# jzlianglu/pykaldi2

Measured on AMD Instinct MI355X. Metric: iRTF (hrs audio/hr) 3x512 BLSTM LF-MMI, LibriSpeech-shaped synthetic utterances, higher is better.
Workload: dtype f32 (GEMMs: bf16x3 split, f32 accumulate)

## Files before the change

pykaldi2_amd/_lib.py:

```python
import ctypes as C
import os

import torch

_HERE = os.path.dirname(os.path.abspath(__file__))
LIB_PATH = os.environ.get("PK2_LIB") or os.path.join(_HERE, "libpk2hip.so")


class Pk2Error(RuntimeError):
    pass


class NumBatch(C.Structure):
    _fields_ = [("arc_src", C.c_void_p), ("arc_dst", C.c_void_p), ("arc_pdf", C.c_void_p),
                ("arc_weight", C.c_void_p), ("frame_off", C.c_void_p), ("state_off", C.c_void_p),
                ("final_state", C.c_void_p), ("final_weight", C.c_void_p), ("final_off", C.c_void_p),
                ("total_arcs", C.c_int64), ("max_seq_arcs", C.c_int64)]


class DecoderOpts(C.Structure):
    _fields_ = [("beam", C.c_float), ("lattice_beam", C.c_float), ("beam_delta", C.c_float),
                ("acoustic_scale", C.c_float), ("max_active", C.c_int32), ("min_active", C.c_int32),
                ("tokens_per_frame", C.c_int32), ("links_per_frame", C.c_int32)]


class SimRirJob(C.Structure):
    _fields_ = [("wav", C.c_void_p), ("rir", C.c_void_p), ("out", C.c_void_p), ("early", C.c_void_p),
                ("delay_dev", C.c_void_p), ("n", C.c_int64), ("k", C.c_int32), ("delay", C.c_int32)]


class SimSeg(C.Structure):
    _fields_ = [("x", C.c_void_p), ("count", C.c_int64)]


class SimMixSrc(C.Structure):
    _fields_ = [("sig", C.c_void_p), ("sig2", C.c_void_p), ("pos", C.c_void_p), ("pos2", C.c_void_p),
                ("n", C.c_int64), ("start", C.c_int64), ("spr_db", C.c_double)]


class ResampleJob(C.Structure):
    _fields_ = [("plan", C.c_void_p), ("inp", C.c_void_p), ("n_in", C.c_int64), ("out", C.c_void_p), ("n_out", C.c_int64),
                ("gain", C.c_float)]


SIM_MAX_SEGS = 16
RESAMPLE_MAX_JOBS = 32
SPEC_MAX_FREQ_MASKS = 4
SPEC_MAX_TIME_MASKS = 16
SPEC_PLAN_STRIDE = 2 + 2 * SPEC_MAX_FREQ_MASKS + 2 * SPEC_MAX_TIME_MASKS
BF_MAX_CHANNELS = 8
BF_MAX_MASKS = 4
BF_FRAMES_PER_PART = 32
BF_REF_SNR = -1
WPE_MAX_CHANNELS = 8
WPE_MAX_ORDER = 80
WPE_MAX_DELAY = 8
WPE_MAX_ITERS = 8
WPE_FRAMES_PER_PART = 1024

_vp, _i32, _i64, _f32, _sz = C.c_void_p, C.c_int32, C.c_int64, C.c_float, C.c_size_t

SIGNATURES = {
    "pk2_last_error": (C.c_char_p, []),
    "pk2_version": (C.c_int, []),
    "pk2_den_graph_create": (C.c_int, [_i32, _i32, _i64, _vp, _vp, _vp, _vp, _i32, C.POINTER(_vp)]),
    "pk2_den_graph_from_openfst": (C.c_int, [C.c_char_p, _i32, C.POINTER(_vp)]),
    "pk2_den_graph_destroy": (C.c_int, [_vp]),
    "pk2_den_graph_info": (C.c_int, [_vp, C.POINTER(_i32), C.POINTER(_i32), C.POINTER(_i64)]),
    "pk2_den_graph_initial_probs": (C.c_int, [_vp, _vp]),
    "pk2_den_graph_arcs_per_lane": (_i32, []),
    "pk2_den_graph_path": (_i32, [_vp, _i32]),
    "pk2_den_graph_persist_form": (_i32, [_vp, _i32]),
    "pk2_den_graph_plan": (C.c_int, [_vp, _i32, _i32, _vp]),
    "pk2_den_graph_debug_ordering": (C.c_int, [_vp, C.c_int, C.POINTER(_i64), C.POINTER(_i32), _vp, _vp,
                                               _vp, _vp, _vp, _vp]),
    "pk2_den_graph_debug_virtual": (C.c_int, [_vp, C.c_int, C.POINTER(_i32), _vp, _vp, _vp, _vp, _vp,
                                              C.POINTER(_i64), _vp, _vp, _vp, C.POINTER(_i32), _vp, _vp]),
    "pk2_den_graph_debug_persist2": (C.c_int, [_vp, C.c_int] + [_vp] * 18),
    "pk2_chain_workspace_bytes": (_sz, [_vp, _i32, _i32, _i64]),
    "pk2_chain_objf_and_deriv": (C.c_int, [_vp, _vp, _i64, _i64, _vp, _i32, C.POINTER(NumBatch), _f32,
                                           _f32, _f32, _f32, _vp, _i64, _i64, _vp, _vp, _sz, _vp]),
    "pk2_chain_objf_and_deriv_op": (C.c_int, [_vp, _vp, _i64, _i64, _vp, _i32, C.POINTER(NumBatch), _f32,
                                              _f32, _f32, _f32, _vp, _i64, _i64, _vp, _vp, _sz, _f32, _vp, _vp]),
    "pk2_chain_den_fwd_bwd": (C.c_int, [_vp, _vp, _i64, _i64, _vp, _i32, _f32, _vp, _vp, _i64, _i64,
                                        _vp, _sz, _vp]),
    "pk2_chain_debug_flags": (C.c_int, [_vp, _vp, _vp, _vp, _i32, _f32, _vp, _vp, _vp]),
    "pk2_chain_debug_num_route": (C.c_int, [_vp]),
    "pk2_split_to_phones": (C.c_int, [_vp, _vp, _vp, _i32, _vp, _i32, _vp, _vp, C.POINTER(_i32), C.POINTER(_i32)]),
    "pk2_sup_model_create": (_vp, [_i32, _vp, _i32, _vp, _vp, _vp, _vp, _vp, _i32, _vp, _i32, _i32, _i32, _vp, _vp,
                                   _vp, _vp, _i32, _vp]),
    "pk2_sup_model_destroy": (None, [_vp]),
    "pk2_sup_model_pdf": (C.c_int, [_vp, _vp, _i32, C.POINTER(_i32)]),
    "pk2_supervision_create": (_vp, [_vp, _vp, _vp, _i32, _i32, _i32, _i32]),
    "pk2_supervision_destroy": (None, [_vp]),
    "pk2_supervision_sizes": (None, [_vp, C.POINTER(_i32), C.POINTER(_i32), C.POINTER(_i32), C.POINTER(_i32),
                                     C.POINTER(_i32)]),
    "pk2_supervision_copy": (C.c_int, [_vp, _vp, _vp, _vp, _vp, _vp, _vp, _vp, _vp, _vp, _vp]),
    "pk2_lexicon_create": (_vp, [_i32, _i32, _i64, _vp, _vp, _vp, _vp, _vp, _vp, _vp, _i32]),
    "pk2_lexicon_from_openfst": (_vp, [C.c_char_p, _vp, _i32]),
    "pk2_lexicon_destroy": (None, [_vp]),
    "pk2_align_model_create": (_vp, [_vp, _i32, _vp, _i32, _vp, C.c_double, C.c_double]),
    "pk2_align_model_destroy": (None, [_vp]),
    "pk2_align_compile": (_vp, [_vp, _vp, _i32, _vp, _vp, _vp]),
    "pk2_align_graphs_destroy": (None, [_vp]),
    "pk2_align_graphs_info": (C.c_int, [_vp, _i32, C.POINTER(_i32), C.POINTER(_i32), C.POINTER(_i32)]),
    "pk2_align_graphs_error": (C.c_char_p, [_vp, _i32]),
    "pk2_align_graphs_copy": (C.c_int, [_vp, _i32, _vp, _vp, _vp, _vp, _vp, _vp]),
    "pk2_align_graphs_packed_words": (_i64, [_vp]),
    "pk2_align_graphs_pack": (C.c_int, [_vp, _vp]),
    "pk2_align_workspace_bytes": (_sz, [_vp]),
    "pk2_align_use_lds": (C.c_int, [_vp]),
    "pk2_align_viterbi": (C.c_int, [_vp, _vp, _vp, _i64, _i64, _i32, _i32, _f32, _f32, _vp, _vp, _vp, _vp, _sz, _vp]),
    "pk2_num_graph_workspace_bytes": (_sz, [_vp]),
    "pk2_num_graph_use_lds": (C.c_int, [_vp]),
    "pk2_num_graph_fwd_bwd": (C.c_int, [_vp, _vp, _vp, _i64, _i64, _i32, _i32, _f32, _vp, _i64, _i64, _vp, _vp, _vp, _sz, _vp]),
    "pk2_chain_graph_workspace_bytes": (_sz, [_vp, _vp]),
    "pk2_chain_objf_and_deriv_graph": (C.c_int, [_vp, _vp, _i64, _i64, _vp, _vp, _f32, _f32, _f32, _f32, _vp, _i64, _i64, _vp,
                                                 _vp, _sz, _vp]),
    "pk2_chain_objf_and_deriv_graph_op": (C.c_int, [_vp, _vp, _i64, _i64, _vp, _vp, _f32, _f32, _f32, _f32, _vp, _i64, _i64,
                                                    _vp, _vp, _sz, _f32, _vp, _vp]),
    "pk2_decode_graph_create": (C.c_int, [_i32, _i32, _i64, _vp, _vp, _vp, _vp, _vp, C.POINTER(_vp)]),
    "pk2_decode_graph_create_words": (C.c_int, [_i32, _i32, _i64, _vp, _vp, _vp, _vp, _vp, _vp, C.POINTER(_vp)]),
    "pk2_decode_graph_link_words": (C.c_int, [_vp, _i64, _vp, _vp, _vp, _vp, _vp]),
    "pk2_decode_graph_from_openfst": (C.c_int, [C.c_char_p, C.POINTER(_vp)]),
    "pk2_decode_graph_destroy": (C.c_int, [_vp]),
    "pk2_decode_graph_info": (C.c_int, [_vp, C.POINTER(_i32), C.POINTER(_i64), C.POINTER(_i32)]),
    "pk2_lattice_batch_create": (C.c_int, [_vp, _vp, _i32, C.POINTER(DecoderOpts), C.POINTER(_vp)]),
    "pk2_lattice_batch_bytes": (_sz, [_vp]),
    "pk2_lattice_batch_destroy": (C.c_int, [_vp]),
    "pk2_lattice_decode": (C.c_int, [_vp, _vp, _i64, _i64, _i32, _vp, _i32, _vp, _vp]),
    "pk2_lattice_summary": (C.c_int, [_vp, _vp, _vp, _vp, _vp, _vp, _vp]),
    "pk2_lattice_persist_status": (C.c_int, [C.POINTER(C.c_int32), C.POINTER(C.c_uint32)]),
    "pk2_lattice_mmi": (C.c_int, [_vp, _vp, _vp, _i64, _vp, C.c_double, C.c_double, _i32, _vp, _i64, _i64, _vp, _vp]),
    "pk2_lattice_mpe": (C.c_int, [_vp, _vp, _vp, _i64, _vp, _vp, _vp, _i32, _i32, C.c_double, C.c_double, _vp, _i64, _i64,
                                  _vp, _vp]),
    "pk2_lattice_nbest_bytes": (_sz, [_vp, _i32, _i64, _i64, _i32, _i32]),
    "pk2_lattice_nbest": (C.c_int, [_vp, _vp, _vp, _i64, _i64, _i32, _i32, _i32, _vp, _i32, C.c_double, C.c_double, _i32,
                                    _vp, _vp, _vp, _vp, _vp, _vp, _vp]),
    "pk2_lattice_mwe": (C.c_int, [_vp, _vp, _vp, _i64, _i64, _i32, _i32, _i32, _vp, _i32, C.c_double, C.c_double, _i32, _i32,
                                  _vp, _i64, _vp, _vp, _i32, _vp, _i64, _i64, _vp, _vp]),
    "pk2_lattice_rescore": (C.c_int, [_vp, _vp, _vp, _i64, _i64, _i32, _vp, _i32, _f32, _vp]),
    "pk2_lattice_fb_rerun": (C.c_int, [_vp, _vp, _vp, _vp]),
    "pk2_lattice_posteriors": (C.c_int, [_vp, _vp, _vp, C.c_double, C.c_double, _f32, _vp, _i64, _i64, _vp, _vp]),
    "pk2_lattice_ts": (C.c_int, [_vp, _vp, _vp, _i64, _i64, _i32, _vp, _i32, _f32, C.c_double, C.c_double, _vp, _i64, _i64,
                                 _vp, _vp, _vp, _vp]),
    "pk2_lattice_export": (C.c_int, [_vp, _vp, _i32, C.POINTER(_i32), C.POINTER(_i32), _vp, _vp, _vp, _vp, _vp,
                                     _vp, _vp, _vp, _vp, _vp]),
    "pk2_comm_unique_id_bytes": (_i32, []),
    "pk2_comm_unique_id": (C.c_int, [_vp]),
    "pk2_comm_init": (C.c_int, [_i32, _i32, _vp, C.POINTER(_vp)]),
    "pk2_allreduce_bucket": (C.c_int, [_vp, _vp, _i64, _vp]),
    "pk2_allreduce_guarded": (C.c_int, [_vp, _vp, _i64, _vp, _vp]),
    "pk2_comm_info": (C.c_int, [_vp, C.POINTER(_i32), C.POINTER(_i32), C.c_char_p, _i32]),
    "pk2_comm_destroy": (C.c_int, [_vp]),
    "pk2_sim_apply_rir": (C.c_int, [_vp, _i64, _vp, _i32, _i32, _vp, _vp]),
    "pk2_sim_apply_rir_dev": (C.c_int, [_vp, _i64, _vp, _i32, _vp, _vp, _vp]),
    "pk2_sim_power": (C.c_int, [_vp, _i64, _vp, _vp]),
    "pk2_rirgen_segment_samples": (_i32, []),
    "pk2_rirgen": (C.c_int, [_vp, _vp, _vp, _vp, _i32, _vp, _i32, _i64, _vp, _vp, _vp, _vp]),
    "pk2_sim_add_noise": (C.c_int, [_vp, _i64, _vp, _i64, _i64, _f32, _vp, _vp, _vp]),
    "pk2_sim_gain_norm": (C.c_int, [_vp, _i64, _vp, _vp]),
    "pk2_sim_apply_rir_mc": (C.c_int, [C.POINTER(SimRirJob), _i32, _i32, _i32, _vp]),
    "pk2_sim_power_seg": (C.c_int, [C.POINTER(SimSeg), _i32, _vp, _vp]),
    "pk2_sim_gain_norm_seg": (C.c_int, [C.POINTER(SimSeg), _i32, _vp, _vp, _vp]),
    "pk2_sim_mix": (C.c_int, [C.POINTER(SimMixSrc), _i32, _i32, _i64, _vp, _vp, _vp, _vp]),
    "pk2_sim_add_noise_mc": (C.c_int, [_vp, _i64, _vp, _i64, _i32, _i64, _f32, _i32, _vp, _vp, _vp]),
    "pk2_resample_plan_create": (C.c_int, [_i32, _i32, C.c_double, _i32, C.POINTER(_vp)]),
    "pk2_resample_plan_destroy": (C.c_int, [_vp]),
    "pk2_resample_plan_info": (C.c_int, [_vp, C.POINTER(_i32), C.POINTER(_i32), C.POINTER(_i32), C.POINTER(_i32),
                                         C.POINTER(_i64)]),
    "pk2_resample_plan_export": (C.c_int, [_vp, _vp, _vp, _vp]),
    "pk2_resample_num_output": (_i64, [_vp, _i64]),
    "pk2_resample_batch": (C.c_int, [C.POINTER(ResampleJob), _i32, _vp]),
    "pk2_resample_last_path": (C.c_int, [C.POINTER(_i32)]),
    "pk2_iso_spectra": (C.c_int, [_vp, _vp, _vp, C.c_uint64, _i32, _i32, _i32, _vp, _vp]),
    "pk2_iso_gauss": (C.c_int, [C.c_uint64, _i32, _i32, _vp, _vp]),
    "pk2_irfft_pow2_f32": (C.c_int, [_vp, _i32, _i32, _vp, _vp]),
    "pk2_stft_num_frames": (_i64, [_i64, _i32, _i32]),
    "pk2_stft_f32": (C.c_int, [C.POINTER(_vp), _i32, _i64, _i32, _i32, _i32, _vp, _vp, _i32, C.c_uint64, _vp, _vp]),
    "pk2_istft_f32": (C.c_int, [_vp, _i32, _i32, _i32, _i32, _i32, _vp, _vp, _vp, _vp]),
    "pk2_mask_power": (C.c_int, [_vp, _i64, _vp, _vp]),
    "pk2_mask_count_workspace_bytes": (_sz, [_i32]),
    "pk2_mask_count_threshold": (C.c_int, [_vp, _i32, _i64, C.c_double, _vp, _sz, _vp, _vp]),
    "pk2_mask_ibm": (C.c_int, [_vp, _vp, _i32, _i32, _i32, _f32, _i32, _vp, _vp, _vp, _vp]),
    "pk2_fbank_create": (C.c_int, [_vp, C.POINTER(_vp)]),
    "pk2_fbank_destroy": (C.c_int, [_vp]),
    "pk2_fbank_num_frames": (_i32, [_i64]),
    "pk2_fbank_compute": (C.c_int, [_vp, _vp, _vp, _i32, _vp, _vp, _i32, _vp]),
    "pk2_pad_roll_subsample": (C.c_int, [_vp, _vp, _i32, _i32, _i32, _i32, _vp, _i32, _i32, _vp]),
    "pk2_mvn_apply": (C.c_int, [_vp, _vp, _vp, _i64, _i32, _vp, _vp]),
    "pk2_spec_augment": (C.c_int, [_vp, _vp, _vp, _i32, _i64, _vp, _i32, _f32, _vp]),
    "pk2_bf_workspace_bytes": (_sz, [_vp, _i32, _i32, _i32, _i32, _i32]),
    "pk2_bf_cov": (C.c_int, [C.POINTER(_vp), C.POINTER(_vp), C.POINTER(_i32), _i32, _i32, _i32, _i32, _i32, _vp, _sz, _vp, _vp]),
    "pk2_bf_mvdr_weights": (C.c_int, [C.POINTER(_vp), C.POINTER(_vp), _i32, _i32, _i32, _i32, C.c_double, _vp, _sz, _vp, _vp,
                                      _vp, _vp]),
    "pk2_bf_apply": (C.c_int, [C.POINTER(_vp), C.POINTER(_vp), C.POINTER(_i32), _i32, _i32, _i32, C.POINTER(_vp), _vp]),
    "pk2_wpe_workspace_bytes": (_sz, [_vp, _i32, _i32, _i32, _i32, _i32]),
    "pk2_wpe_power": (C.c_int, [C.POINTER(_vp), C.POINTER(_i32), _i32, _i32, _i32, C.POINTER(_vp), _vp]),
    "pk2_wpe_corr": (C.c_int, [C.POINTER(_vp), C.POINTER(_vp), C.POINTER(_i32), _i32, _i32, _i32, _i32, _i32, _vp, _sz, _vp, _vp,
                               _vp]),
    "pk2_wpe_solve": (C.c_int, [_vp, _vp, _i32, _i32, _i32, _i32, C.c_double, _vp, _sz, _vp, _vp, _vp]),
    "pk2_wpe_filter": (C.c_int, [C.POINTER(_vp), _vp, C.POINTER(_i32), _i32, _i32, _i32, _i32, _i32, C.POINTER(_vp),
                                 C.POINTER(_vp), _vp]),
    "pk2_wpe": (C.c_int, [C.POINTER(_vp), C.POINTER(_i32), _i32, _i32, _i32, _i32, _i32, _i32, C.c_double, _vp, _sz,
                          C.POINTER(_vp), _vp, _vp]),
    "pk2_softmax_ce_fwd_bwd": (C.c_int, [_vp, _i64, _vp, _i64, _i64, _i32, _vp, _vp, _vp, _i64, _vp, _vp]),
    "pk2_softmax_ce_fwd_bwd_mean": (C.c_int, [_vp, _i64, _vp, _i64, _i64, _i32, _vp, _vp, _vp, _i64, _vp]),
    "pk2_scale_inplace_ratio": (C.c_int, [_vp, _i64, _vp, _vp, _vp]),
    "pk2_scale_by_count": (C.c_int, [_vp, _i64, _f32, _vp, _vp]),
    "pk2_scale_by_scalars": (C.c_int, [_vp, _vp, _i64, _vp, _vp, _vp]),
    "pk2_gemm_f32": (C.c_int, [_i32, _i32, _i32, _i32, _i32, _f32, _vp, _i64, _vp, _i64, _f32, _vp, _i64,
                               _vp, _vp]),
    "pk2_gemm_f32_act": (C.c_int, [_i32, _i32, _i32, _i32, _i32, _f32, _vp, _i64, _vp, _i64, _f32, _vp, _i64, _vp, _i32, _vp, _i64,
                                   _vp]),
    "pk2_gemm_f32_seg": (C.c_int, [_i32, _i32, _i32, _i32, _i32, _i32, _f32, _vp, _i64, _i64, _vp, _i64, _i64, _f32, _vp, _i64, _vp,
                                   _i32, _vp, _i64, _vp]),
    "pk2_gemm_f32_batched": (C.c_int, [_i32, _i32, _i32, _i32, _i32, _f32, _vp, _i64, _i64, _i64, _vp, _i64, _i64, _i64,
                                       _f32, _vp, _i64, _i64, _i64, _i32, _i32, _vp]),
    "pk2_gemm_f32_tn_colsum": (C.c_int, [_i32, _i32, _i32, _f32, _vp, _i64, _vp, _i64, _f32, _vp, _i64, _vp, _vp]),
    "pk2_gemm_set_arith": (C.c_int, [_i32]),
    "pk2_gemm_get_arith": (C.c_int, []),
    "pk2_layernorm_fwd": (C.c_int, [_vp, _vp, _vp, _vp, _i64, _i32, _f32, _vp, _vp, _vp, _vp, _vp]),
    "pk2_layernorm_bwd": (C.c_int, [_vp, _vp, _vp, _vp, _vp, _i64, _i32, _vp, _vp, _vp, _vp]),
    "pk2_softmax_mask_fwd": (C.c_int, [_vp, _vp, _vp, _i32, _i32, _i32, _vp]),
    "pk2_softmax_bwd": (C.c_int, [_vp, _vp, _i32, _i32, _vp]),
    "pk2_attention_fwd": (C.c_int, [_vp, _i32, _i32, _i32, _i32, _f32, _vp, _vp, _f32, C.c_uint64, _vp, _vp, _vp]),
    "pk2_attention_bwd": (C.c_int, [_vp, _vp, _vp, _vp, _i32, _i32, _i32, _i32, _f32, _vp, _vp, _f32, C.c_uint64, _vp,
                                    _vp, _vp]),
    "pk2_attention_bwd_part": (C.c_int, [_i32, _vp, _vp, _vp, _vp, _i32, _i32, _i32, _i32, _f32, _vp, _vp, _f32, C.c_uint64,
                                         _vp, _vp, _vp]),
    "pk2_relu_fwd": (C.c_int, [_vp, _i64, _vp]),
    "pk2_relu_bwd": (C.c_int, [_vp, _vp, _i64, _vp]),
    "pk2_add_inplace": (C.c_int, [_vp, _vp, _i64, _vp]),
    "pk2_colsum_f32": (C.c_int, [_vp, _i64, _i32, _i32, _f32, _vp, _vp]),
    "pk2_lstm_fwd_workspace_floats": (_sz, [_i32, _i32, _i32]),
    "pk2_lstm_layer_fwd": (C.c_int, [_vp, _vp, _vp, _i32, _i32, _i32, _i32, _vp, _vp, _vp, _vp, _vp]),
    "pk2_lstm_layer_fwd_xproj": (C.c_int, [_vp, _vp, _vp, _i32, _i32, _i32, _i32, _vp, _vp, _vp, _vp, _vp, _i32, _vp, _vp,
                                           C.POINTER(_i32), _vp]),
    "pk2_lstm_persist_status": (C.c_int, [C.POINTER(C.c_uint32)]),
    "pk2_lstm_last_path": (C.c_int, [C.POINTER(_i32), C.POINTER(_i32)]),
    "pk2_lattice_determinize": (C.c_int, [_i32, _i32, _i64, _vp, _vp, _vp, _vp, _vp, _vp, _vp, C.c_double, _i64, C.POINTER(_vp)]),
    "pk2_det_lattice_sizes": (C.c_int, [_vp, C.POINTER(_i32), C.POINTER(_i32), C.POINTER(_i64), C.POINTER(_i64), C.POINTER(_i64)]),
    "pk2_det_lattice_export": (C.c_int, [_vp] * 12),
    "pk2_det_lattice_destroy": (None, [_vp]),
    "pk2_persist_guard_status": (C.c_int, [C.POINTER(C.c_uint32)]),
    "pk2_persist_guard_clear": (C.c_int, []),
    "pk2_persist_guard_raise": (C.c_int, [_vp]),
    "pk2_persist_guard_export": (C.c_int, [_vp, _vp]),
    "pk2_persist_guard_import": (C.c_int, [_vp, C.c_uint32, _vp]),
    "pk2_persist_guard_verdict": (C.c_int, [C.c_uint32, C.POINTER(C.c_uint32), C.POINTER(C.c_uint32)]),
    "pk2_lstm_bwd_scratch_floats": (_sz, [_i32, _i32, _i32]),
    "pk2_lstm_layer_bwd_bias": (C.c_int, [_vp, _vp, _vp, _vp, _i32, _i32, _i32, _i32, _vp, _vp, _vp, _vp, C.POINTER(_i32), _vp]),
    "pk2_lstm_layer_bwd": (C.c_int, [_vp, _vp, _vp, _vp, _i32, _i32, _i32, _i32, _vp, _vp, _vp]),
    "pk2_lstm_bwd_wgrad_workspace_floats": (_sz, [_i32, _i32, _i32]),
    "pk2_lstm_layer_bwd_wgrad": (C.c_int, [_vp, _vp, _vp, _vp, _vp, _i32, _i32, _i32, _i32, _vp, _vp, _vp, _vp, _vp, _vp,
                                           C.POINTER(_i32), C.POINTER(_i32), _vp]),
    "pk2_dropout_f32": (C.c_int, [_vp, _vp, _i64, _f32, C.c_uint64, _vp]),
    "pk2_grad_norm": (C.c_int, [_vp, _i64, _vp, _vp, _sz, _vp]),
    "pk2_grad_norm_workspace_bytes": (_sz, [_i64]),
    "pk2_adam_step": (C.c_int, [_vp, _vp, _vp, _vp, _vp, _i64, _f32, _f32, _f32, _f32, _f32, _i64, _f32,
                                _vp, _f32, _vp]),
    "pk2_sgd_step": (C.c_int, [_vp, _vp, _vp, _i64, _f32, _f32, _f32, _i32, _f32, _vp, _f32, _vp]),
    "pk2_stream_create_cu_mask": (C.c_int, [_i32, C.POINTER(_vp)]),
    "pk2_stream_destroy": (C.c_int, [_vp]),
    "pk2_debug_where": (C.c_int, [_vp, _i32, _vp]),
    "pk2_debug_peer_reduce": (C.c_int, [_vp, _vp, _i64, _i32, _i32, _vp]),
}

_lib = None


def lib():
    global _lib
    if _lib is None:
        if not os.path.exists(LIB_PATH):
            raise Pk2Error("%s is missing: run `python -c 'import __graft_entry__ as g; g.build()'` "
                           "(hipcc --offload-arch=gfx950).  There is no CPU fallback." % LIB_PATH)
        handle = C.CDLL(LIB_PATH)
        for name, (res, args) in SIGNATURES.items():
            fn = getattr(handle, name)
            fn.restype = res
            fn.argtypes = args
        _lib = handle
    return _lib


def h2d(host, device):
    import numpy as np
    t = torch.from_numpy(host) if isinstance(host, np.ndarray) else host
    if torch.device(device).type != "cuda" or t.is_cuda or t.numel() == 0:
        return t.to(device)
    return t.contiguous().pin_memory().to(device, non_blocking=True)


def check(status):
    if status != 0:
        msg = lib().pk2_last_error()
        raise Pk2Error("libpk2hip status %d: %s" % (status, msg.decode() if msg else ""))


def persist_guard_raised():
    flag = C.c_uint32(0)
    check(lib().pk2_persist_guard_status(C.byref(flag)))
    return flag.value != 0


def check_persist_guard(where, raised=None):
    if persist_guard_raised() if raised is None else raised:
        raise Pk2Error("%s: a persistent kernel (one-launch LSTM recurrence / denominator / lattice decoder) timed out on "
                       "this device; its output was poisoned with NaN and the optimiser kernels have been leaving the "
                       "weights untouched since.  Typical causes: the GPU is shared with another process, or fewer than "
                       "256 CUs are available to the launch.  PK2_LSTM_SEQ=0 PK2_LSTM_BIG_PERSIST=0 PK2_DEN_PERSIST=0 "
                       "PK2_LAT_DECODER=frames select the launch-per-step kernels." % where)


def ptr(t):
    if t is None:
        return None
    if isinstance(t, torch.Tensor):
        return C.c_void_p(t.data_ptr())
    return C.c_void_p(t.ctypes.data)


def stream_ptr(device=None):
    return C.c_void_p(torch.cuda.current_stream(device).cuda_stream)


def require_gpu():
    if not torch.cuda.is_available():
        raise Pk2Error("pykaldi2_amd needs an MI355X (torch.cuda.is_available() is False); "
                       "there is no CPU fallback")
```

pykaldi2_amd/chain.py:

```python
import ctypes as C

import numpy as np
import torch

from . import _lib


class ChainTrainingOptions:

    def __init__(self, leaky_hmm_coefficient=1.0e-05, xent_regularize=0.0, l2_regularize=0.0):
        self.leaky_hmm_coefficient = leaky_hmm_coefficient
        self.xent_regularize = xent_regularize
        self.l2_regularize = l2_regularize


class SupervisionOptions:

    def __init__(self):
        self.convert_to_pdfs = True
        self.frame_subsampling_factor = 3
        self.left_tolerance = 5
        self.right_tolerance = 5


class DenominatorGraph:
    def __init__(self, den_fst, num_pdfs):
        L = _lib.lib()
        h = C.c_void_p()
        if isinstance(den_fst, (str, bytes)):
            path = den_fst.encode() if isinstance(den_fst, str) else den_fst
            _lib.check(L.pk2_den_graph_from_openfst(path, int(num_pdfs), C.byref(h)))
        else:
            src = np.ascontiguousarray(den_fst["src"], dtype=np.int32)
            dst = np.ascontiguousarray(den_fst["dst"], dtype=np.int32)
            pdf = np.ascontiguousarray(den_fst["pdf"], dtype=np.int32)
            prob = np.ascontiguousarray(den_fst["prob"], dtype=np.float32)
            _lib.check(L.pk2_den_graph_create(int(den_fst["num_states"]), int(num_pdfs), src.shape[0],
                                              _lib.ptr(src), _lib.ptr(dst), _lib.ptr(pdf), _lib.ptr(prob),
                                              int(den_fst.get("start", 0)), C.byref(h)))
        self._h = h
        s, p, a = C.c_int32(), C.c_int32(), C.c_int64()
        _lib.check(L.pk2_den_graph_info(h, C.byref(s), C.byref(p), C.byref(a)))
        self._num_states, self._num_pdfs, self._num_arcs = s.value, p.value, a.value

    def num_states(self):
        return self._num_states

    def num_pdfs(self):
        return self._num_pdfs

    def num_arcs(self):
        return self._num_arcs

    def initial_probs(self):
        out = np.empty(self._num_states, dtype=np.float32)
        _lib.check(_lib.lib().pk2_den_graph_initial_probs(self._h, _lib.ptr(out)))
        return out

    def kernel_path(self, num_seqs):
        return int(_lib.lib().pk2_den_graph_path(self._h, int(num_seqs)))

    def persist_form(self, num_seqs):
        return int(_lib.lib().pk2_den_graph_persist_form(self._h, int(num_seqs)))

    PLAN_FIELDS = ("family", "form", "NG", "need_fill", "xgather", "prep_merged", "tail_mergeable", "gamma_kernel")

    def plan(self, num_seqs, max_frames):
        out = np.zeros(8, dtype=np.int32)
        _lib.check(_lib.lib().pk2_den_graph_plan(self._h, int(num_seqs), int(max_frames), _lib.ptr(out)))
        return dict(zip(self.PLAN_FIELDS, (int(v) for v in out)))

    def debug_persist2(self, which):
        L = _lib.lib()
        info = np.zeros(32, dtype=np.int32)
        _lib.check(L.pk2_den_graph_debug_persist2(self._h, which, _lib.ptr(info), *([None] * 17)))
        if not info[0]:
            return None
        R, T, K, W, SP, SEG = (int(v) for v in info[26:32])
        MC = SEG - 2
        pieces, rows = int(info[7]), int(info[9])
        out = dict(prob=np.empty((R, K, T), np.float32), idx2=np.empty((R, K // 2, T), np.uint32),
                   ends=np.empty((R, 2, T), np.uint32), first_row=np.empty((R, 2, T), np.int32),
                   uncovered=np.empty((R, 2), np.int32), ncomp=np.empty((R, 2), np.int32), rmap=np.empty((2, rows), np.int16),
                   pbeg=np.empty((R, MC + 1), np.int32),
                   sprob=np.empty((pieces, T, SP), np.float32), sidx2=np.empty((pieces, T, SP // 2), np.uint32),
                   sends=np.empty((pieces, T), np.uint32), sfirst_row=np.empty((R, MC, T), np.int32),
                   wcrow=np.empty((R, SEG, W), np.int32), row_begin=np.empty(R + 1, np.int32),
                   grp_begin=np.empty(R + 1, np.int32), row_leak=np.empty(rows, np.float32), row_psum=np.empty(rows, np.float32))
        order = ("prob", "idx2", "ends", "first_row", "uncovered", "ncomp", "rmap", "pbeg", "sprob", "sidx2", "sends", "sfirst_row", "wcrow",
                 "row_begin", "grp_begin", "row_leak", "row_psum")
        _lib.check(L.pk2_den_graph_debug_persist2(self._h, which, _lib.ptr(info), *[_lib.ptr(out[k]) for k in order]))
        out.update(estep=int(info[1]), K=int(info[2]), R=int(info[3]), tfloats=int(info[4]), max_rows=int(info[5]),
                   max_groups=int(info[6]), pieces=pieces, cap=int(info[8]), cbeg=[int(v) for v in info[10:10 + MC + 1]],
                   lds_off=[int(v) for v in info[20:20 + MC]], SP=SP, W=W, T=T, slots=K, row_arrays=int(info[19]))
        return out

    def debug_ordering(self, which):
        L = _lib.lib()
        na, nc = C.c_int64(), C.c_int32()
        _lib.check(L.pk2_den_graph_debug_ordering(self._h, which, C.byref(na), C.byref(nc), None, None,
                                                  None, None, None, None))
        arcs = np.empty((na.value, 4), dtype=np.int32)
        k = int(L.pk2_den_graph_arcs_per_lane())
        meta = np.empty((na.value // k, 2), dtype=np.uint32)
        wb_off = np.empty(nc.value + 1, dtype=np.int32)
        row0 = np.empty(nc.value, dtype=np.int32)
        nrows = np.empty(nc.value, dtype=np.int32)
        atomic = np.empty(nc.value, dtype=np.int32)
        _lib.check(L.pk2_den_graph_debug_ordering(self._h, which, None, None, _lib.ptr(arcs), _lib.ptr(meta),
                                                  _lib.ptr(wb_off), _lib.ptr(row0), _lib.ptr(nrows),
                                                  _lib.ptr(atomic)))
        out = dict(arcs=arcs, meta=meta, wb_off=wb_off, row0=row0, nrows=nrows, atomic=atomic, arcs_per_lane=k)
        if which >= 3:
            nv, nl, no = C.c_int32(), C.c_int64(), C.c_int32()
            _lib.check(L.pk2_den_graph_debug_virtual(self._h, which, C.byref(nv), None, None, None, None, None,
                                                     C.byref(nl), None, None, None, C.byref(no), None, None))
            S = self._num_states
            voff, ooff = np.empty(S + 1, dtype=np.int32), np.empty(S + 1, dtype=np.int32)
            vpdf, opdf = np.empty(nv.value, dtype=np.int32), np.empty(no.value, dtype=np.int32)
            real0, nreal, slot0 = (np.empty(nc.value, dtype=np.int32) for _ in range(3))
            leak = np.empty(nl.value, dtype=np.float32)
            loop_pdf, loop_prob = np.empty(S, dtype=np.int32), np.empty(S, dtype=np.float32)
            _lib.check(L.pk2_den_graph_debug_virtual(self._h, which, None, _lib.ptr(voff), _lib.ptr(vpdf),
                                                     _lib.ptr(real0), _lib.ptr(nreal), _lib.ptr(slot0), None,
                                                     _lib.ptr(leak), _lib.ptr(loop_pdf), _lib.ptr(loop_prob), None,
                                                     _lib.ptr(ooff), _lib.ptr(opdf)))
            out.update(voff=voff, vpdf=vpdf, real0=real0, nreal=nreal, slot0=slot0, row_leak=leak,
                       loop_pdf=loop_pdf, loop_prob=loop_prob, ooff=ooff, opdf=opdf)
        return out

    def __del__(self):
        try:
            if getattr(self, "_h", None):
                _lib.lib().pk2_den_graph_destroy(self._h)
                self._h = None
        except Exception:
            pass


class Supervision:

    def __init__(self, fst, weight=1.0, label_dim=None):
        self.weight = float(weight)
        self.num_sequences = 1
        self.frames_per_sequence = int(fst["frames"])
        self.label_dim = label_dim
        self.num_states = int(fst["num_states"])
        self.src = np.ascontiguousarray(fst["src"], dtype=np.int32)
        self.dst = np.ascontiguousarray(fst["dst"], dtype=np.int32)
        self.pdf = np.ascontiguousarray(fst["pdf"], dtype=np.int32)
        self.arc_weight = np.ascontiguousarray(fst["weight"], dtype=np.float32)
        self.frame_offsets = np.ascontiguousarray(fst["frame_offsets"], dtype=np.int32)
        self.final_states = np.ascontiguousarray(fst["final_states"], dtype=np.int32)
        self.final_weights = np.ascontiguousarray(fst["final_weights"], dtype=np.float32)
        self.state_time = fst.get("state_time")
        assert self.frame_offsets.shape[0] == self.frames_per_sequence + 1


class ProtoSupervision:

    def __init__(self, opts, phones, durations):
        self.phones = np.ascontiguousarray(phones, dtype=np.int32)
        self.durations = np.ascontiguousarray(durations, dtype=np.int32)
        if self.phones.ndim != 1 or self.phones.shape != self.durations.shape or self.phones.shape[0] == 0:
            raise ValueError("phones and durations must be non-empty lists of equal length")
        self.frame_subsampling_factor = int(opts.frame_subsampling_factor)
        self.left_tolerance, self.right_tolerance = int(opts.left_tolerance), int(opts.right_tolerance)


def alignment_to_proto_supervision(opts, phones, durations):
    return ProtoSupervision(opts, phones, durations)


class _SupModel:

    def __init__(self, tree, trans_model):
        if trans_model.entries is None:
            raise ValueError("the transition model carries no topology (read it from 0.trans_mdl / final.mdl)")
        max_phone = max(trans_model.phone2entry)
        p2e = np.full(max_phone + 1, -1, np.int32)
        for ph, e in trans_model.phone2entry.items():
            p2e[ph] = e
        e_off, fwd, loop, t_off, t_dst = [0], [], [], [0], []
        for states in trans_model.entries:
            for f, l, dsts in states:
                fwd.append(f); loop.append(l); t_dst.extend(dsts); t_off.append(len(t_dst))
            e_off.append(len(fwd))
        arr = lambda v: np.ascontiguousarray(v, dtype=np.int32)
        e_off, fwd, loop, t_off, t_dst = arr(e_off), arr(fwd), arr(loop), arr(t_off), arr(t_dst)
        tuples = arr(trans_model.tuples)
        L = _lib.lib()
        self._h = L.pk2_sup_model_create(max_phone, _lib.ptr(p2e), len(trans_model.entries), _lib.ptr(e_off),
                                         _lib.ptr(fwd), _lib.ptr(loop), _lib.ptr(t_off), _lib.ptr(t_dst),
                                         tuples.shape[0], _lib.ptr(tuples), tree.N, tree.P, tree.kind.shape[0],
                                         _lib.ptr(tree.kind), _lib.ptr(tree.key), _lib.ptr(tree.a), _lib.ptr(tree.b),
                                         tree.pool.shape[0], _lib.ptr(tree.pool))
        if not self._h:
            raise _lib.Pk2Error(L.pk2_last_error().decode())
        self.label_dim = trans_model.num_pdfs()

    def pdf(self, window, pdf_class):
        w = np.ascontiguousarray(window, dtype=np.int32)
        out = C.c_int32()
        _lib.check(_lib.lib().pk2_sup_model_pdf(self._h, _lib.ptr(w), int(pdf_class), C.byref(out)))
        return out.value

    def __del__(self):
        try:
            if self._h:
                _lib.lib().pk2_sup_model_destroy(self._h)
                self._h = None
        except Exception:
            pass


_sup_models = {}


def supervision_model(tree, trans_model):
    key = (id(tree), id(trans_model))
    hit = _sup_models.get(key)
    if hit is None or hit[0] is not tree or hit[1] is not trans_model:
        hit = _sup_models[key] = (tree, trans_model, _SupModel(tree, trans_model))
    return hit[2]


def proto_supervision_to_supervision(tree, trans_model, proto, convert_to_pdfs=True, with_allowed=False):
    if not convert_to_pdfs:
        raise NotImplementedError("only convert_to_pdfs=True (reference bin/train_chain.py:185) is built")
    m = supervision_model(tree, trans_model)
    L = _lib.lib()
    h = L.pk2_supervision_create(m._h, _lib.ptr(proto.phones), _lib.ptr(proto.durations), proto.phones.shape[0],
                                 proto.frame_subsampling_factor, proto.left_tolerance, proto.right_tolerance)
    if not h:
        raise _lib.Pk2Error(L.pk2_last_error().decode())
    try:
        n = [C.c_int32() for _ in range(5)]
        L.pk2_supervision_sizes(h, *[C.byref(v) for v in n])
        frames, ns, na, nf, nal = (v.value for v in n)
        src, dst, pdf = (np.empty(na, np.int32) for _ in range(3))
        w, foff, stime = np.empty(na, np.float32), np.empty(frames + 1, np.int32), np.empty(ns, np.int32)
        fin, finw = np.empty(nf, np.int32), np.empty(nf, np.float32)
        aoff = np.empty(frames + 1, np.int32) if with_allowed else None
        aph = np.empty(nal, np.int32) if with_allowed else None
        _lib.check(L.pk2_supervision_copy(h, _lib.ptr(src), _lib.ptr(dst), _lib.ptr(pdf), _lib.ptr(w), _lib.ptr(foff),
                                          _lib.ptr(stime), _lib.ptr(fin), _lib.ptr(finw), _lib.ptr(aoff), _lib.ptr(aph)))
    finally:
        L.pk2_supervision_destroy(h)
    sup = Supervision(dict(num_states=ns, frames=frames, src=src, dst=dst, pdf=pdf, weight=w, frame_offsets=foff,
                           state_time=stime, final_states=fin, final_weights=finw), label_dim=m.label_dim)
    if with_allowed:
        sup.allowed_phones = [aph[aoff[t]:aoff[t + 1]].tolist() for t in range(frames)]
    return sup


def split_to_phones(trans_model, alignment):
    if trans_model.tid2tstate is None:
        raise ValueError("the transition model carries no topology (read it from final.mdl)")
    ali = np.ascontiguousarray(alignment, dtype=np.int32)
    T = ali.shape[0]
    phones, durs = np.empty(max(T, 1), np.int32), np.empty(max(T, 1), np.int32)
    n, ok = C.c_int32(), C.c_int32()
    _lib.check(_lib.lib().pk2_split_to_phones(_lib.ptr(trans_model.tid2tstate), _lib.ptr(trans_model.tid2phone),
                                              _lib.ptr(trans_model.tid_flags), trans_model.num_transition_ids(),
                                              _lib.ptr(ali), T, _lib.ptr(phones), _lib.ptr(durs), C.byref(n),
                                              C.byref(ok)))
    starts = np.concatenate([[0], np.cumsum(durs[:n.value])[:-1]]) if n.value else []
    return bool(ok.value), [(int(p), int(s), int(d)) for p, s, d in zip(phones[:n.value], starts, durs[:n.value])]


def supervision_from_alignment(aligner, tree, trans_model, opts, trans_ids):
    phone_ali = aligner.to_phone_alignment(trans_ids)
    proto = alignment_to_proto_supervision(opts, [item[0] for item in phone_ali], [item[2] for item in phone_ali])
    return proto_supervision_to_supervision(tree, trans_model, proto, opts.convert_to_pdfs)


def read_disambig(path):
    if not path:
        return []
    with open(path) as f:
        return [int(tok) for line in f for tok in line.split()[:1]]


def read_symbols(path):
    with open(path) as f:
        return {p[0]: int(p[1]) for p in (line.split() for line in f) if len(p) >= 2}


class Lexicon:

    def __init__(self, fst, disambig=()):
        L = _lib.lib()
        dis = np.ascontiguousarray(list(disambig), np.int32)
        if isinstance(fst, (str, bytes)):
            h = L.pk2_lexicon_from_openfst(fst.encode() if isinstance(fst, str) else fst, _lib.ptr(dis), dis.shape[0])
        else:
            a = {k: np.ascontiguousarray(fst[k], np.int32) for k in ("src", "dst", "ilabel", "olabel")}
            w = np.ascontiguousarray(fst["weight"], np.float32)
            fin = np.ascontiguousarray(fst["final"], np.float32)
            assert fin.shape[0] == int(fst["num_states"])
            h = L.pk2_lexicon_create(int(fst["num_states"]), int(fst.get("start", 0)), a["src"].shape[0], _lib.ptr(a["src"]),
                                     _lib.ptr(a["dst"]), _lib.ptr(a["ilabel"]), _lib.ptr(a["olabel"]), _lib.ptr(w), _lib.ptr(fin),
                                     _lib.ptr(dis), dis.shape[0])
        if not h:
            raise _lib.Pk2Error(L.pk2_last_error().decode())
        self._h = h

    def __del__(self):
        try:
            if self._h:
                _lib.lib().pk2_lexicon_destroy(self._h)
                self._h = None
        except Exception:
            pass


class AlignModel:

    def __init__(self, tree, trans_model, transition_scale=1.0, self_loop_scale=1.0):
        lp = getattr(trans_model, "log_probs", None)
        if lp is None:
            raise ValueError("the transition model has no <LogProbs> (read it from final.mdl): the aligner needs them")
        if lp.shape[0] != trans_model.num_transition_ids() + 1:
            raise ValueError("<LogProbs> holds %d values for %d transition-ids" % (lp.shape[0], trans_model.num_transition_ids()))
        self._sup = _SupModel(tree, trans_model)
        tuples = np.ascontiguousarray(trans_model.tuples, np.int32)
        lp = np.ascontiguousarray(lp, np.float64)
        L = _lib.lib()
        self._h = L.pk2_align_model_create(self._sup._h, tuples.shape[0], _lib.ptr(tuples), trans_model.num_transition_ids(),
                                           _lib.ptr(lp), float(transition_scale), float(self_loop_scale))
        if not self._h:
            raise _lib.Pk2Error(L.pk2_last_error().decode())

    def __del__(self):
        try:
            if self._h:
                _lib.lib().pk2_align_model_destroy(self._h)
                self._h = None
        except Exception:
            pass


ALIGN_OK, ALIGN_BEAM, ALIGN_NO_PATH, ALIGN_ERROR = 0, 1, 2, 3


class AlignmentGraphs:

    def __init__(self, model, lexicon, texts, frames):
        word_off = np.cumsum([0] + [len(t) for t in texts]).astype(np.int32)
        words = np.ascontiguousarray([int(w) for t in texts for w in t] or [0], np.int32)
        self.frames = np.ascontiguousarray(frames, np.int32)
        assert self.frames.shape[0] == len(texts)
        L = _lib.lib()
        self._h = L.pk2_align_compile(model._h, lexicon._h, len(texts), _lib.ptr(word_off), _lib.ptr(words), _lib.ptr(self.frames))
        if not self._h:
            raise _lib.Pk2Error(L.pk2_last_error().decode())
        self._keep = (model, lexicon)
        self.n = len(texts)
        self.status, self.num_states, self.num_arcs, self.errors = [], [], [], []
        for i in range(self.n):
            v = [C.c_int32() for _ in range(3)]
            _lib.check(L.pk2_align_graphs_info(self._h, i, *[C.byref(x) for x in v]))
            self.status.append(v[0].value); self.num_states.append(v[1].value); self.num_arcs.append(v[2].value)
            self.errors.append(L.pk2_align_graphs_error(self._h, i).decode())

    def export(self, i):
        S, A = self.num_states[i], self.num_arcs[i]
        out = dict(in_off=np.empty(S + 1, np.int32), src=np.empty(A, np.int32), tid=np.empty(A, np.int32),
                   pdf=np.empty(A, np.int32), weight=np.empty(A, np.float32), final=np.empty(S, np.float32))
        _lib.check(_lib.lib().pk2_align_graphs_copy(self._h, i, *[_lib.ptr(out[k]) for k in
                                                                 ("in_off", "src", "tid", "pdf", "weight", "final")]))
        out["dst"] = np.repeat(np.arange(S, dtype=np.int32), np.diff(out["in_off"]))
        return out
# ... 379 lines not shown
```

pykaldi2_amd/csrc/chain_den_persist2.hip:

```cpp
#include <algorithm>
#include <cstdlib>
#include <cstring>
#include <map>
#include <type_traits>
#include <vector>

#include "chain_num.h"
#include "den_persist_dev.h"

namespace pk2 {

struct DenPersist2Params {
  DenParams d;
  DevPersist2 fwd, bwd;
  const float* xv;
  const int32_t* vpdf;
  const int32_t* loop_pdf;
  int xgather;
  int rowarrays;
  float* ring;
  float* pring;
  int rpad;
  int tfloats;
  int cap;
  int ntasks;
  NumParams np;
  int fwd_stream, bwd_stream;
  int pspt;
  short task_seq[kMaxTasks];
  unsigned char task_dir[kMaxTasks];
};
typedef __attribute__((address_space(4))) const DenPersist2Params CParams2;
typedef __attribute__((address_space(4))) const DevPersist2 CDev2;
__device__ __forceinline__ CParams2* uni(CParams2* p) {
  const unsigned long long v = (unsigned long long)p;
  const unsigned lo = (unsigned)__builtin_amdgcn_readfirstlane((int)(unsigned)v);
  const unsigned hi = (unsigned)__builtin_amdgcn_readfirstlane((int)(unsigned)(v >> 32));
  return (CParams2*)(((unsigned long long)hi << 32) | lo);
}

extern __shared__ __attribute__((aligned(16))) float den_persist2_smem[];
struct Lds2 {
  float* table;
  float* accA;
  float* accB;
  float* accS;
  float* xown;
  float* leak;
  float* aux;
  short* mapA;
  short* mapB;
  short* pdfv;
  short* pdfl;
  float* red;
  float* tot;
  float* wcarry;
  int* wcrow;
  int* abort;
};
__device__ __forceinline__ Lds2 carve_lds2(int tfloats, int cap, int arrays) {
  Lds2 L;
  L.table = den_persist2_smem; L.accA = L.table + tfloats; L.accB = L.accA + cap; L.accS = L.accB + cap; L.xown = L.accS + cap;
  L.leak = L.xown + cap; L.aux = L.leak + cap;
  L.mapA = reinterpret_cast<short*>(L.aux + cap); L.mapB = L.mapA + cap;
  L.pdfv = L.mapB + cap; L.pdfl = L.pdfv + cap;
  L.red = L.aux + (arrays - 5) * cap; L.tot = L.red + 2 * kPW; L.wcarry = L.tot + 4;
  L.wcrow = reinterpret_cast<int*>(L.wcarry + kSegs * kPW); L.abort = L.wcrow + kSegs * kPW;
  return L;
}

__device__ __forceinline__ void lds_only_barrier() { asm volatile("s_waitcnt lgkmcnt(0)\n\ts_barrier" ::: "memory"); }

#ifndef PK2_DP2_LATE_HISTORY
#define PK2_DP2_LATE_HISTORY 0
#endif
#ifndef PK2_DP2_LATE_STREAM
#define PK2_DP2_LATE_STREAM 1
#endif
template <bool STREAM> constexpr bool kLateHistory = PK2_DP2_LATE_HISTORY && (!STREAM || PK2_DP2_LATE_STREAM);
template <bool NT>
__device__ __forceinline__ float once_load(cgfloat* p) {
  if constexpr (NT) return __builtin_nontemporal_load(p);
  else return *p;
}
template <bool NT>
__device__ __forceinline__ void once_store(gfloat* p, float v) {
  if constexpr (NT) __builtin_nontemporal_store(v, p);
  else *p = v;
}

template <bool ON>
__device__ __forceinline__ int per_frame(int r) {
  if constexpr (ON) asm volatile("" : "+v"(r));
  return r;
}
__device__ __forceinline__ float ld_uniform_base(cgfloat* ubase, int idx) {
  typedef __attribute__((address_space(1))) const char gchar;
  return *(cgfloat*)((gchar*)ubase + (uint32_t)idx * 4u);
}

__device__ __forceinline__ constexpr int vmcnt_imm(int k) { return (k & 15) | ((k >> 4) << 14) | 0x70 | 0xF00; }
__device__ __forceinline__ void wait_vm(int n) {
  asm volatile("" ::: "memory");
  switch (__builtin_amdgcn_readfirstlane(n)) {
#define PK2_VM_CASE(k) case k: __builtin_amdgcn_s_waitcnt(vmcnt_imm(k)); break;
    PK2_VM_CASE(1) PK2_VM_CASE(2) PK2_VM_CASE(3) PK2_VM_CASE(4) PK2_VM_CASE(5) PK2_VM_CASE(6) PK2_VM_CASE(7) PK2_VM_CASE(8)
    PK2_VM_CASE(9) PK2_VM_CASE(10) PK2_VM_CASE(11) PK2_VM_CASE(12) PK2_VM_CASE(13) PK2_VM_CASE(14) PK2_VM_CASE(15) PK2_VM_CASE(16)
    PK2_VM_CASE(17) PK2_VM_CASE(18) PK2_VM_CASE(19) PK2_VM_CASE(20)
#undef PK2_VM_CASE
    default: __builtin_amdgcn_s_waitcnt(vmcnt_imm(0)); break;
  }
  asm volatile("" ::: "memory");
}

__device__ __forceinline__ int dma_chunk(cgfloat* src, CDev2& o, int c, float* table) {
  const int lane = threadIdx.x & 63, w = threadIdx.x >> 6;
  const int b = o.cbeg[c], e = o.cbeg[c + 1];
  const int rows = (e - b + 255) >> 8;
  const int n = (rows + kPW - 1) / kPW;
  const int e4 = (e + 3) & ~3;
  float* dst = table + o.lds_off[c];
  for (int k = 0; k < n; ++k) {
    int row = w + k * kPW;
    row = row < rows ? row : rows - 1;
    const int off = row << 8;
    if (b + off + lane * 4 < e4) dma256(src + b + off + lane * 4, dst + off);
  }
  return n;
}
typedef __attribute__((address_space(3))) float lfloat;
__device__ __forceinline__ uint32_t lds_addr(const float* p) { return (uint32_t)(uintptr_t)(const lfloat*)p; }
__device__ __forceinline__ float lds_load(uint32_t a) { return *(const lfloat*)(uintptr_t)a; }
__device__ __forceinline__ void lds_store(uint32_t a, float v) { *(lfloat*)(uintptr_t)a = v; }

struct DmaPlan {
  uint64_t mask[8];
  uint32_t off4[8];
  uint32_t dst;
  int rows, efl, w;
  uint32_t lane16;
  __device__ __forceinline__ void place(int j, uint64_t* mask_out, uint32_t* off4_out) const {
    int row = w + j * kPW;
    row = row < rows ? row : rows - 1;
    const int off = row << 8;
    int n = (efl - off + 3) >> 2;
    n = j * kPW < rows ? n : 0;
    n = n < 0 ? 0 : n;
    *mask_out = n >= 64 ? ~0ull : ((1ull << n) - 1ull);
    *off4_out = (uint32_t)off * 4u;
  }
  __device__ __forceinline__ void init(CDev2& o, const float* table) {
    const int b1 = o.cbeg[1], e1 = o.cbeg[2];
    dst = (uint32_t)__builtin_amdgcn_readfirstlane((int)lds_addr(table + o.lds_off[1]));
    rows = (e1 - b1 + 255) >> 8; efl = ((e1 + 3) & ~3) - b1; w = __builtin_amdgcn_readfirstlane((int)(threadIdx.x >> 6));
    lane16 = (threadIdx.x & 63u) * 16u;
#pragma unroll
    for (int j = 0; j < 8; ++j) {
      place(j, &mask[j], &off4[j]);
      asm volatile("" : "+s"(mask[j]), "+s"(off4[j]));
    }
  }
};
__device__ __forceinline__ void dma_issue(uint64_t mask, uint32_t m0v, uint32_t lane16, uint64_t g) {
  uint64_t saved;
  asm volatile("s_mov_b64 %0, exec\n\ts_mov_b64 exec, %1\n\ts_mov_b32 m0, %2\n\ts_nop 0\n\t"
               "global_load_lds_dwordx4 %3, %4 sc1\n\ts_mov_b64 exec, %0"
               : "=&s"(saved) : "s"(mask), "s"(m0v), "v"(lane16), "s"(g) : "memory");
}
struct Chunk1Dma {
  uint64_t src;
  const DmaPlan* pl;
  __device__ __forceinline__ void operator()(int j) const {
    if (j < 8) { dma_issue(pl->mask[j], pl->dst + pl->off4[j], pl->lane16, src + pl->off4[j]); return; }
    uint64_t mask; uint32_t off4;
    pl->place(j, &mask, &off4);
    dma_issue(mask, pl->dst + off4, pl->lane16, src + off4);
  }
};

struct NoDma { __device__ __forceinline__ void operator()(int) const {} };

#ifndef PK2_DP2_PASS_ASM
#define PK2_DP2_PASS_ASM 1
#endif
__device__ __forceinline__ void lds_gather8(const uint32_t* ad, float (&a)[8]) {
  asm volatile("ds_read_b32 %0, %8\n\tds_read_b32 %1, %9\n\tds_read_b32 %2, %10\n\tds_read_b32 %3, %11\n\t"
               "ds_read_b32 %4, %12\n\tds_read_b32 %5, %13\n\tds_read_b32 %6, %14\n\tds_read_b32 %7, %15"
               : "=&v"(a[0]), "=&v"(a[1]), "=&v"(a[2]), "=&v"(a[3]), "=&v"(a[4]), "=&v"(a[5]), "=&v"(a[6]), "=&v"(a[7])
               : "v"(ad[0]), "v"(ad[1]), "v"(ad[2]), "v"(ad[3]), "v"(ad[4]), "v"(ad[5]), "v"(ad[6]), "v"(ad[7]) : "memory");
}
template <int N>
__device__ __forceinline__ void lds_wait8(float (&a)[8]) {
  asm volatile("s_waitcnt lgkmcnt(%8)" : "+v"(a[0]), "+v"(a[1]), "+v"(a[2]), "+v"(a[3]), "+v"(a[4]), "+v"(a[5]), "+v"(a[6]), "+v"(a[7])
               : "n"(N) : "memory");
}
template <int N>
__device__ __forceinline__ void lds_wait4(float& a0, float& a1, float& a2, float& a3) {
  asm volatile("s_waitcnt lgkmcnt(%4)" : "+v"(a0), "+v"(a1), "+v"(a2), "+v"(a3) : "n"(N) : "memory");
}
__device__ __forceinline__ void row_end_place(unsigned& m, uint32_t& cb, float& sum) {
  uint64_t save;
  asm volatile("v_add_co_u32 %0, vcc, %0, %0\n\ts_and_saveexec_b64 %3, vcc\n\tds_write_b32 %1, %2\n\t"
               "v_add_u32 %1, 4, %1\n\tv_mov_b32 %2, 0\n\ts_or_b64 exec, exec, %3"
               : "+v"(m), "+v"(cb), "+v"(sum), "=&s"(save) : : "vcc", "scc", "memory");
}

template <bool PACKED, int J0>
__device__ __forceinline__ void slot_addresses(const uint32_t (&addr)[kPK], uint32_t base, int j0, uint32_t (&out)[8]) {
#pragma unroll
  for (int j = 0; j < 8; ++j) {
    const int s = J0 + j0 + j;
    if (PACKED) {
      uint32_t pk = addr[s >> 1];
      if ((s & 1) == 0) asm volatile("" : "+v"(pk));
      out[j] = base + ((s & 1) ? (pk >> 16) << 2 : (pk & 0xffffu) << 2);
    } else {
      out[j] = addr[s];
    }
  }
}
template <int ESTEP, int J0, int NS, bool PACKED, typename DMA>
__device__ __forceinline__ void pass_rows(const float (&prob)[kPK], const uint32_t (&addr)[kPK], uint32_t base, uint32_t ends, int frow,
                                          float* acc, float* wcarry, const DMA& dma) {
  const int lane = threadIdx.x & 63, w = threadIdx.x >> 6;
  float sum = 0.f;
  uint32_t cb = lds_addr(acc) + 4u * (uint32_t)frow;
  uint32_t packed = 0;
#pragma unroll
  for (int k = 0; k < NS / ESTEP; ++k) packed |= ((ends >> (k * ESTEP + ESTEP - 1)) & 1u) << k;
  unsigned m = __builtin_bitreverse32(packed);
  asm volatile("" : "+v"(m));
  float a[2][8];
#if PK2_DP2_PASS_ASM
  constexpr int NG = NS / 8;
  constexpr int kStores = 8 / ESTEP;
  uint32_t ad[8];
  slot_addresses<PACKED, J0>(addr, base, 0, ad);
  lds_gather8(ad, a[0]);
  dma(0);
#pragma unroll
  for (int g = 0; g < NG; ++g) {
    if (g + 1 < NG) { slot_addresses<PACKED, J0>(addr, base, 8 * (g + 1), ad); lds_gather8(ad, a[(g + 1) & 1]); dma(2 * g + 2); }
    constexpr int kMost = 15;
    if (g == 0) lds_wait8<(NG > 1 ? 8 : 0)>(a[0]);
    else if (g + 1 < NG) lds_wait8<(8 + kStores < kMost ? 8 + kStores : kMost)>(a[g & 1]);
    else lds_wait8<kStores>(a[g & 1]);
#pragma unroll
    for (int j = 0; j < 8; ++j) {
      const int jj = 8 * g + j;
      sum = fmaf(a[g & 1][j], prob[J0 + jj], sum);
      if ((jj + 1) % ESTEP == 0) row_end_place(m, cb, sum);
    }
    dma(2 * g + 1);
  }
#else
  auto gather = [&](int j0, float (&a)[8]) {
    uint32_t ad2[8];
    slot_addresses<PACKED, J0>(addr, base, j0, ad2);
#pragma unroll
    for (int j = 0; j < 8; ++j) a[j] = lds_load(ad2[j]);
  };
  gather(0, a[0]);
  dma(0);
#pragma unroll
  for (int g = 0; g < NS / 8; ++g) {
    if (g + 1 < NS / 8) { gather(8 * (g + 1), a[(g + 1) & 1]); dma(2 * g + 2); }
#pragma unroll
    for (int j = 0; j < 8; ++j) {
      const int jj = 8 * g + j;
      sum = fmaf(a[g & 1][j], prob[J0 + jj], sum);
      if ((jj + 1) % ESTEP == 0) {
        if (__builtin_add_overflow(m, m, &m)) { lds_store(cb, sum); cb += 4u; sum = 0.f; }
      }
    }
    dma(2 * g + 1);
  }
#endif
  float x[1] = {sum};
  int fl = ends != 0u ? 1 : 0;
  seg_scan_step<1, 0x111, 0xf>(x, fl);
  seg_scan_step<1, 0x112, 0xf>(x, fl);
  seg_scan_step<1, 0x114, 0xf>(x, fl);
  seg_scan_step<1, 0x118, 0xf>(x, fl);
  seg_scan_step<1, 0x142, 0xa>(x, fl);
  seg_scan_step<1, 0x143, 0xc>(x, fl);
  const float cin = dpp_f<0x138, 0xf>(x[0]);
  if (ends != 0u) acc[frow] += cin;
  if (lane == 63) wcarry[w] = x[0];
}
template <int J0, bool PACKED, typename DMA>
__device__ __forceinline__ void pass_rows_any(int estep, const float (&prob)[kPK], const uint32_t (&addr)[kPK], uint32_t base,
                                              uint32_t ends, int frow, float* acc, float* wcarry, const DMA& dma) {
  switch (estep) {
    case 8: pass_rows<8, J0, kQ, PACKED>(prob, addr, base, ends, frow, acc, wcarry, dma); break;
    case 4: pass_rows<4, J0, kQ, PACKED>(prob, addr, base, ends, frow, acc, wcarry, dma); break;
    case 2: pass_rows<2, J0, kQ, PACKED>(prob, addr, base, ends, frow, acc, wcarry, dma); break;
    default: pass_rows<1, J0, kQ, PACKED>(prob, addr, base, ends, frow, acc, wcarry, dma); break;
  }
}

typedef float __attribute__((ext_vector_type(4))) f32x4;
typedef uint32_t __attribute__((ext_vector_type(4))) u32x4v;
struct Piece { f32x4 p0, p1; u32x4v ix; uint32_t ends; };
__device__ __forceinline__ void piece_load(CDev2& o, int piece, Piece& q) {
  static_assert(kSP == 8, "a piece is two float4 of probabilities and one uint4 of packed offsets per thread");
  const size_t at = (size_t)piece * kPT + threadIdx.x;
  const __attribute__((address_space(1))) f32x4* sp = (const __attribute__((address_space(1))) f32x4*)o.sprob + at * (kSP / 4);
  const __attribute__((address_space(1))) u32x4v* si = (const __attribute__((address_space(1))) u32x4v*)o.sidx2 + at;
  const __attribute__((address_space(1))) uint32_t* se = (const __attribute__((address_space(1))) uint32_t*)o.sends;
  q.p0 = sp[0]; q.p1 = sp[1];
  q.ix = si[0];
  q.ends = se[at];
}
__device__ __forceinline__ void row_end_add(unsigned& m, uint32_t& cb, float& sum) {
  uint64_t save;
  asm volatile("v_add_co_u32 %0, vcc, %0, %0\n\ts_and_saveexec_b64 %3, vcc\n\tds_add_f32 %1, %2\n\t"
               "v_add_u32 %1, 4, %1\n\tv_mov_b32 %2, 0\n\ts_or_b64 exec, exec, %3"
               : "+v"(m), "+v"(cb), "+v"(sum), "=&s"(save) : : "vcc", "scc", "memory");
}
template <int ESTEP>
__device__ __forceinline__ void piece_rows(const Piece q, uint32_t base, uint32_t& cb, float& sum) {
  uint32_t packed = 0;
#pragma unroll
  for (int k = 0; k < kSP / ESTEP; ++k) packed |= ((q.ends >> (k * ESTEP + ESTEP - 1)) & 1u) << k;
  unsigned m = __builtin_bitreverse32(packed);
  uint32_t ad[8];
#pragma unroll
  for (int j = 0; j < kSP; ++j) {
    const uint32_t pk = q.ix[j >> 1];
    ad[j] = base + ((j & 1) ? (pk >> 16) << 2 : (pk & 0xffffu) << 2);
  }
  float a[8];
  lds_gather8(ad, a);
  lds_wait4<4>(a[0], a[1], a[2], a[3]);
#pragma unroll
  for (int j = 0; j < 4; ++j) {
    sum = fmaf(a[j], q.p0[j], sum);
    if ((j + 1) % ESTEP == 0) row_end_add(m, cb, sum);
  }
  lds_wait4<(ESTEP <= 4 ? 4 / ESTEP : 0)>(a[4], a[5], a[6], a[7]);
#pragma unroll
  for (int j = 4; j < 8; ++j) {
    sum = fmaf(a[j], q.p1[j & 3], sum);
    if ((j + 1) % ESTEP == 0) row_end_add(m, cb, sum);
  }
}
__device__ __forceinline__ void piece_rows_any(int estep, const Piece q, uint32_t base, uint32_t& cb, float& sum) {
  switch (estep) {
    case 8: piece_rows<8>(q, base, cb, sum); break;
    case 4: piece_rows<4>(q, base, cb, sum); break;
    case 2: piece_rows<2>(q, base, cb, sum); break;
    default: piece_rows<1>(q, base, cb, sum); break;
  }
}

constexpr int kPieceDepth = 2;
constexpr int kPieceLoads = 4;
struct StreamState { Piece r0, r1; int pb[kMaxChunks + 1]; int frow[2]; int pend; };
static_assert(kPieceDepth == 2, "StreamState holds two pieces");
__device__ __forceinline__ void stream_init(CDev2& o, int rank, StreamState& st) {
#pragma unroll
  for (int c = 0; c <= kMaxChunks; ++c) st.pb[c] = __builtin_amdgcn_readfirstlane(o.pbeg[rank * (kMaxChunks + 1) + c]);
  const __attribute__((address_space(1))) int32_t* sfr = (const __attribute__((address_space(1))) int32_t*)o.sfirst_row;
#pragma unroll
  for (int c = 0; c < 2; ++c) st.frow[c] = st.pb[c + 1] > st.pb[c] ? sfr[((size_t)rank * kMaxChunks + c) * kPT + threadIdx.x] : 0;
  st.pend = st.pb[0];
#pragma unroll
  for (int c = 1; c <= kMaxChunks; ++c) st.pend = c == o.K ? st.pb[c] : st.pend;
}
__device__ __forceinline__ void stream_prime(CDev2& o, StreamState& st) {
  const int pfirst = st.pb[0], pend = st.pend;
  if (pfirst < pend) piece_load(o, pfirst, st.r0);
  if (pfirst + 1 < pend) piece_load(o, pfirst + 1, st.r1);
}
__device__ __forceinline__ int streamed_segment(CDev2& o, int rank, int c, int p0, int p1, StreamState& st, const Lds2& L) {
  const int tid = threadIdx.x, lane = tid & 63, w = tid >> 6;
  const int pend = st.pend;
  const int frow = c < 2 ? st.frow[c < 2 ? c : 0]
                         : ((const __attribute__((address_space(1))) int32_t*)o.sfirst_row)[((size_t)rank * kMaxChunks + c) * kPT + tid];
  float sum = 0.f;
  int issued = 0;
  uint32_t had = 0;
  uint32_t cb = lds_addr(L.accS) + 4u * (uint32_t)frow;
  const uint32_t base = lds_addr(L.table);
  for (int p = p0; p < p1; ++p) {
    had |= st.r0.ends;
    piece_rows_any(o.estep, st.r0, base, cb, sum);
    st.r0 = st.r1;
    if (p + kPieceDepth < pend) { piece_load(o, p + kPieceDepth, st.r1); ++issued; }
  }
  float x[1] = {sum};
  int fl = had != 0u ? 1 : 0;
  seg_scan_step<1, 0x111, 0xf>(x, fl);
  seg_scan_step<1, 0x112, 0xf>(x, fl);
  seg_scan_step<1, 0x114, 0xf>(x, fl);
  seg_scan_step<1, 0x118, 0xf>(x, fl);
  seg_scan_step<1, 0x142, 0xa>(x, fl);
  seg_scan_step<1, 0x143, 0xc>(x, fl);
  const float cin = dpp_f<0x138, 0xf>(x[0]);
  if (had != 0u) L.accS[frow] += cin;
  if (lane == 63) L.wcarry[(2 + c) * kPW + w] = x[0];
  return issued;
}

struct FrameRegs {
  float prob[kPK]; uint32_t addr[kPK]; uint32_t base; uint32_t endsA, endsB; int frowA, frowB;
};
struct NoStream { };
struct RowSpan { int nrows, uncA, ncA, uncB, ncB; };
template <bool STREAM, typename ST, typename STAGE>
__device__ __forceinline__ void frame_rows(CDev2& o, cgfloat* src, int rank, const RowSpan& rs, const FrameRegs& r,
                                           const DmaPlan& plan, ST& st, const Lds2& L, DpTimers& dp_, STAGE stage,
                                           bool prime_next = false) {
  const int tid = threadIdx.x;
  if constexpr (STREAM) {
    for (int q = tid; q < rs.nrows; q += kPT) L.accS[q] = 0.f;
    for (int q = rs.uncA + tid; q < rs.ncA; q += kPT) L.accA[q] = 0.f;
    for (int q = rs.uncB + tid; q < rs.ncB; q += kPT) L.accB[q] = 0.f;
  }
  dma_chunk(src, o, 0, L.table);
  DP_T(0);
  wait_vm(0);
  lds_only_barrier();
  DP_T(1);
  DP_TLF(2);
  Chunk1Dma c1;
  {
    const uint64_t sb = (uint64_t)(src + o.cbeg[1]);
    c1.src = ((uint64_t)(uint32_t)__builtin_amdgcn_readfirstlane((int)(uint32_t)(sb >> 32)) << 32) |
             (uint32_t)__builtin_amdgcn_readfirstlane((int)(uint32_t)sb);
    c1.pl = &plan;
  }
  const bool shared = o.K == 2 && o.lds_off[1] == o.lds_off[0] && o.cbeg[2] > o.cbeg[1];
  if (shared) {
    pass_rows_any<0, STREAM>(o.estep, r.prob, r.addr, r.base, r.endsA, r.frowA, L.accA, L.wcarry, NoDma());
  } else {
    pass_rows_any<0, STREAM>(o.estep, r.prob, r.addr, r.base, r.endsA, r.frowA, L.accA, L.wcarry, c1);
    for (int j = 8; j * kPW < plan.rows; ++j) c1(j);
  }
  DP_T(2);
  DP_TLF(3);
  if constexpr (STREAM) {
    const int (&pb)[kMaxChunks + 1] = st.pb;
    const int K = o.K;
    int young = 0;
    if (pb[1] > pb[0]) young = streamed_segment(o, rank, 0, pb[0], pb[1], st, L);
    DP_T(8);
    if (shared) { lds_only_barrier(); dma_chunk(src, o, 1, L.table); young = 0; }
    wait_vm(kPieceLoads * (young < kPieceDepth ? young : kPieceDepth));
    stage();
    lds_only_barrier();
    DP_T(3);
    if (K > 2) dma_chunk(src, o, 2, L.table);
    pass_rows_any<kQ, STREAM>(o.estep, r.prob, r.addr, r.base, r.endsB, r.frowB, L.accB, L.wcarry + kPW, NoDma());
    DP_T(4);
    if (pb[2] > pb[1]) streamed_segment(o, rank, 1, pb[1], pb[2], st, L);
#pragma unroll
    for (int c = 2; c < kMaxChunks; ++c) {
      if (c >= K) break;
      wait_vm(0);
      __syncthreads();
      if (c + 1 < K) dma_chunk(src, o, c + 1, L.table);
      if (pb[c + 1] > pb[c]) streamed_segment(o, rank, c, pb[c], pb[c + 1], st, L);
    }
    if (prime_next) stream_prime(o, st);
  } else {
    if (shared) { lds_only_barrier(); dma_chunk(src, o, 1, L.table); }
    wait_vm(0);
    stage();
    __syncthreads();
    DP_T(3);
    pass_rows_any<kQ, STREAM>(o.estep, r.prob, r.addr, r.base, r.endsB, r.frowB, L.accB, L.wcarry + kPW, NoDma());
  }
  if constexpr (STREAM) DP_T(9); else DP_T(4);
}

template <bool STREAM>
__device__ __forceinline__ float row_val(const Lds2& L, uint64_t cmask, int q) {
  const int a = L.mapA[q], b = L.mapB[q];
  float v = (a >= 0 ? L.accA[a] : 0.f) + (b >= 0 ? L.accB[b] : 0.f);
  if constexpr (STREAM) v += L.accS[q];
  uint64_t m = cmask;
  while (m) {
    const int k = __builtin_ctzll(m);
    m &= m - 1;
    if (L.wcrow[k] == q) v += L.wcarry[k];
  }
  return v;
}

template <int NW>
__device__ __forceinline__ void block_sum2(float& u, float& v, float* red) {
  const int lane = threadIdx.x & 63, w = threadIdx.x >> 6;
  u = wave_sum_dpp(u); v = wave_sum_dpp(v);
  __syncthreads();
  if (lane == 0) { red[w] = u; red[NW + w] = v; }
  __syncthreads();
  float a = 0.f, b = 0.f;
  for (int k = 0; k < NW; ++k) { a += red[k]; b += red[NW + k]; }
  u = a; v = b;
}

template <bool PACKED>
__device__ __forceinline__ void load_frame_regs(CDev2& o, int rank, FrameRegs& r, const float* table) {
  const int tid = threadIdx.x;
  const uint32_t base = lds_addr(table);
  r.base = (uint32_t)__builtin_amdgcn_readfirstlane((int)base);
#pragma unroll
  for (int j = 0; j < kPK; ++j) r.prob[j] = o.prob[((size_t)rank * kPK + j) * kPT + tid];
#pragma unroll
  for (int j = 0; j < kPK / 2; ++j) {
    const uint32_t pk = o.idx2[((size_t)rank * (kPK / 2) + j) * kPT + tid];
    if (PACKED) { r.addr[j] = pk; continue; }
    r.addr[2 * j] = base + ((pk & 0xffffu) << 2); r.addr[2 * j + 1] = base + ((pk >> 16) << 2);
    asm volatile("" : "+v"(r.addr[2 * j]), "+v"(r.addr[2 * j + 1]));
  }
  r.endsA = o.ends[((size_t)rank * 2 + 0) * kPT + tid]; r.endsB = o.ends[((size_t)rank * 2 + 1) * kPT + tid];
  r.frowA = o.first_row[((size_t)rank * 2 + 0) * kPT + tid]; r.frowB = o.first_row[((size_t)rank * 2 + 1) * kPT + tid];
}

template <bool STREAM, int PSPT>
__device__ __noinline__ void run_fwd2(CParams2* pp_, DenPersistCtl* ctl_, DenPersistCtl::Team* team_,
                                      unsigned* nbar, int g_, int T_, int rank_, float* ring_, float* pring_) {
  CParams2* pp = uni(pp_);
  DenPersistCtl* ctl = uni(ctl_); DenPersistCtl::Team* team = uni(team_);
  const int g = uni(g_), T = uni(T_), rank = uni(rank_);
  ring_ = uni(ring_); pring_ = uni(pring_);
  CParams2& p = *pp;
  CDenParams& d = p.d;
  CDev2& o = p.fwd;
  const Lds2 L = carve_lds2(p.tfloats, p.cap, p.rowarrays);
  gfloat* ring = G(ring_); gfloat* pring = G(pring_);
  const int tid = threadIdx.x;
  const int S = d.S, V = d.V, Vo = d.Vo;
  const bool sep = d.alphav != d.alpha;
  FrameRegs fr;
  load_frame_regs<STREAM>(o, rank, fr, L.table);
  DmaPlan plan;
  plan.init(o, L.table);
  const int row0 = o.row_begin[rank], nrows = o.row_begin[rank + 1] - row0;
  const int g0 = o.grp_begin[rank], ngrp = o.grp_begin[rank + 1] - g0;
  RowSpan rs;
  rs.nrows = nrows; rs.uncA = o.uncovered[rank * 2]; rs.uncB = o.uncovered[rank * 2 + 1];
  rs.ncA = o.ncomp[rank * 2]; rs.ncB = o.ncomp[rank * 2 + 1];
  for (int r = tid; r < nrows; r += kPT) { L.mapA[r] = o.rmap[row0 + r]; L.mapB[r] = o.rmap[(size_t)o.num_rows + row0 + r]; }
  typename std::conditional<STREAM, StreamState, NoStream>::type st;
  if constexpr (STREAM) stream_init(o, rank, st);
  for (int r = tid; r < nrows; r += kPT) L.leak[r] = o.row_leak[row0 + r];
  const bool xg = p.xgather != 0;
  if (xg) {
    for (int r = tid; r < nrows; r += kPT) L.pdfv[r] = (short)p.vpdf[row0 + r];
    for (int r = tid; r < ngrp; r += kPT) L.pdfl[r] = (short)p.loop_pdf[g0 + r];
  }
  if (tid < kSegs * kPW) L.wcrow[tid] = o.wcrow[(size_t)rank * kSegs * kPW + tid];
  int st_lo[PSPT], st_hi[PSPT], st_o[PSPT]; float st_pl[PSPT], st_pi[PSPT]; bool st_ok[PSPT];
#pragma unroll
  for (int i = 0; i < PSPT; ++i) {
    const int r = tid + i * kPT;
    st_ok[i] = r < ngrp;
    st_lo[i] = st_hi[i] = st_o[i] = 0; st_pl[i] = st_pi[i] = 0.f;
    if (st_ok[i]) {
      const int dd = g0 + r;
      st_lo[i] = d.voff[dd] - row0; st_hi[i] = d.voff[dd + 1] - row0; st_o[i] = d.ooff[dd];
      st_pl[i] = d.loop_prob[dd]; st_pi[i] = d.pi[dd];
    }
  }
  if (tid < 3 * kPWords) st_agent(pring + ((tid / kPWords) * kPR + rank) * kPWords + tid % kPWords, __uint_as_float(kRingSentinel));
  if (!team_barrier(ctl, team, nbar, L.abort)) return;
  uint64_t cmask = 0;
  for (int k = 0; k < kSegs * kPW; ++k) {
    const int q = L.wcrow[k];
    bool mine = false;
#pragma unroll
    for (int i = 0; i < PSPT; ++i) mine = mine || (st_ok[i] && q >= st_lo[i] && q < st_hi[i]);
    if (q >= 0 && mine) cmask |= 1ull << k;
  }

  const size_t f0 = (size_t)g * (d.Tmax + 1);
  cgfloat* xv_g = G(p.xv) + (size_t)g * d.Tmax * V;
  cgfloat* xl_g = G(d.xl) + (size_t)g * d.Tmax * S;
  cgfloat* xp_g = G(p.xv) + (size_t)g * d.Tmax * d.P;
  float xr[PSPT], xlr[PSPT], xln[PSPT];
  auto prefetch = [&](int t) {
    if (xg) {
      cgfloat* row = xp_g + (size_t)t * d.P;
#pragma unroll
      for (int i = 0; i < PSPT; ++i) {
        const int r = per_frame<STREAM>(tid + i * kPT);
        const int pv = r < nrows ? L.pdfv[r] : -1, pl = st_ok[i] ? L.pdfl[r] : -1;
        xr[i] = r < nrows ? (pv >= 0 ? row[pv] : 1.f) : 0.f;
        xln[i] = st_ok[i] ? (pl >= 0 ? row[pl] : 1.f) : 0.f;
      }
      return;
    }
#pragma unroll
    for (int i = 0; i < PSPT; ++i) {
      const int r = per_frame<STREAM>(tid + i * kPT);
      if constexpr (STREAM) {
        xr[i] = r < nrows ? ld_uniform_base(xv_g + ((size_t)t * V + row0), r) : 0.f;
        xln[i] = st_ok[i] ? ld_uniform_base(xl_g + ((size_t)t * S + g0), r) : 0.f;
      } else {
        xr[i] = r < nrows ? once_load<!STREAM>(&xv_g[(size_t)t * V + row0 + r]) : 0.f;
        xln[i] = st_ok[i] ? once_load<!STREAM>(&xl_g[(size_t)t * S + g0 + r]) : 0.f;
      }
    }
  };
  prefetch(0);
#pragma unroll
  for (int i = 0; i < PSPT; ++i) xlr[i] = xln[i];
  if constexpr (STREAM) stream_prime(o, st);
  float own_a[PSPT];
#pragma unroll
  for (int i = 0; i < PSPT; ++i) own_a[i] = st_pi[i];
  float hist_loop[PSPT], hist_loc = 0.f;
#pragma unroll
  for (int i = 0; i < PSPT; ++i) hist_loop[i] = 0.f;
  auto history = [&](int tt) {
    gfloat* alpha_n = G(d.alpha) + (f0 + tt + 1) * (size_t)S;
    gfloat* alphav_n = G(d.alphav) + (f0 + tt + 1) * (size_t)Vo;
    if (tid == 0) G(d.apart)[(f0 + tt + 1) * kPR + rank] = hist_loc;
#pragma unroll
    for (int i = 0; i < PSPT; ++i) {
      if (!st_ok[i]) continue;
      if (!sep) once_store<!STREAM>(&alpha_n[g0 + tid + i * kPT], own_a[i]);
      if (sep) {
        for (int q = st_lo[i]; q < st_hi[i]; ++q) once_store<!STREAM>(&alphav_n[st_o[i] + q - st_lo[i]], L.aux[q]);
        if (st_pl[i] > 0.f) once_store<!STREAM>(&alphav_n[st_o[i] + st_hi[i] - st_lo[i]], hist_loop[i]);
      }
    }
  };
  Spin spin(ctl);
  DP_T0();
  for (int t = 0; t < T; ++t) {
    float as;
    cgfloat* src;
    DP_TL(0, 0);
    DP_TLSET(0);
    if (t == 0) {
      as = d.pi_sum;
      src = G(d.pi);
    } else {
      src = ring + (size_t)(t & 1) * p.rpad;
      poll_words(pring + (size_t)(t % 3) * kPR * kPWords, 0, 1, spin, L);
      __syncthreads();
      DP_TL(0, 1);
      if (*L.abort) return;
      as = L.tot[0];
      if (tid == 0) L.abort[8] = 0;
    }
    const bool publish = t + 1 < T;
    if (tid == 0 && publish) st_agent(word_of(pring, t + 2, rank, 0), __uint_as_float(kRingSentinel));
    frame_rows<STREAM>(o, src, rank, rs, fr, plan, st, L, dp_, [&]() {
#pragma unroll
      for (int i = 0; i < PSPT; ++i) {
        const int r = tid + i * kPT;
        if (r < nrows) L.xown[r] = xr[i];
      }
      if (kLateHistory<STREAM> && t > 0) history(t - 1);
      if (publish) prefetch(t + 1);
    }, publish);
    DP_TL(0, 4);
    if constexpr (STREAM) lds_only_barrier(); else __syncthreads();
    if (rank == 0 && tid == 0) G(d.asum)[f0 + t] = as;
    const float lk = d.leaky * as, inv_as = 1.0f / as;
    gfloat* ring_n = ring + (size_t)((t + 1) & 1) * p.rpad;
    float outv[PSPT], loopv[PSPT], loc = 0.f, unused = 0.f;
#pragma unroll
    for (int i = 0; i < PSPT; ++i) {
      outv[i] = 0.f; loopv[i] = 0.f;
      if (!st_ok[i]) continue;
      float sum = 0.f;
      for (int q = st_lo[i]; q < st_hi[i]; ++q) {
        const float v = (row_val<STREAM>(L, cmask, q) + lk * L.leak[q]) * L.xown[q] * inv_as;
        L.aux[q] = v;
        sum += v;
      }
      if (st_pl[i] > 0.f) { loopv[i] = (own_a[i] + lk * st_pi[i]) * st_pl[i] * xlr[i] * inv_as; sum += loopv[i]; }
      if (publish) ring_store(ring_n + g0 + tid + i * kPT, sum);
      outv[i] = sum;
      own_a[i] = sum;
      loc += sum;
    }
    DP_T(5);
    DP_TL(0, 5);
    wait_stores();
    block_sum2<kPW>(loc, unused, L.red);
    if (tid == 0 && publish) st_agent(word_of(pring, t + 1, rank, 0), loc);
    DP_T(6);
    DP_TL(0, 6);
    hist_loc = loc;
#pragma unroll
    for (int i = 0; i < PSPT; ++i) hist_loop[i] = loopv[i];
    if (!kLateHistory<STREAM>) history(t);
#pragma unroll
    for (int i = 0; i < PSPT; ++i) xlr[i] = xln[i];
    DP_T(7);
  }
  if (kLateHistory<STREAM> && T > 0) history(T - 1);
  DP_FLUSH(0);
}

template <bool STREAM, int PSPT>
__device__ __noinline__ void run_bwd2(CParams2* pp_, DenPersistCtl* ctl_, DenPersistCtl::Team* team_,
                                      unsigned* nbar, int g_, int T_, int rank_, float* ring_, float* pring_) {
  CParams2* pp = uni(pp_);
  DenPersistCtl* ctl = uni(ctl_); DenPersistCtl::Team* team = uni(team_);
  const int g = uni(g_), T = uni(T_), rank = uni(rank_);
  ring_ = uni(ring_); pring_ = uni(pring_);
  CParams2& p = *pp;
  CDenParams& d = p.d;
  CDev2& o = p.bwd;
  const Lds2 L = carve_lds2(p.tfloats, p.cap, p.rowarrays);
  gfloat* ring = G(ring_); gfloat* pring = G(pring_);
  const int tid = threadIdx.x;
  const int S = d.S, V = d.V;
  FrameRegs fr;
  load_frame_regs<STREAM>(o, rank, fr, L.table);
  DmaPlan plan;
  plan.init(o, L.table);
  const int row0 = o.row_begin[rank], nrows = o.row_begin[rank + 1] - row0;
  const int vfirst = d.voff[row0], nvirt = d.voff[row0 + nrows] - vfirst;
  RowSpan rs;
  rs.nrows = nrows; rs.uncA = o.uncovered[rank * 2]; rs.uncB = o.uncovered[rank * 2 + 1];
  rs.ncA = o.ncomp[rank * 2]; rs.ncB = o.ncomp[rank * 2 + 1];
  for (int r = tid; r < nrows; r += kPT) { L.mapA[r] = o.rmap[row0 + r]; L.mapB[r] = o.rmap[(size_t)o.num_rows + row0 + r]; }
  typename std::conditional<STREAM, StreamState, NoStream>::type st;
  if constexpr (STREAM) stream_init(o, rank, st);
  if (tid < kSegs * kPW) L.wcrow[tid] = o.wcrow[(size_t)rank * kSegs * kPW + tid];
  int st_v0[PSPT], st_v1[PSPT]; float st_pl[PSPT], st_pi[PSPT]; bool st_ok[PSPT];
#pragma unroll
  for (int i = 0; i < PSPT; ++i) {
    const int r = tid + i * kPT;
    st_ok[i] = r < nrows;
    st_v0[i] = st_v1[i] = 0; st_pl[i] = st_pi[i] = 0.f;
    if (st_ok[i]) {
      const int s = row0 + r;
      st_v0[i] = d.voff[s] - vfirst; st_v1[i] = d.voff[s + 1] - vfirst; st_pl[i] = d.loop_prob[s]; st_pi[i] = d.pi[s];
    }
  }
  for (int r = tid; r < nvirt; r += kPT) { L.leak[r] = p.fwd.row_leak[vfirst + r]; L.aux[r] = p.fwd.row_psum[vfirst + r]; }
  const bool xg = p.xgather != 0;
  if (xg) {
    for (int r = tid; r < nvirt; r += kPT) L.pdfv[r] = (short)p.vpdf[vfirst + r];
    for (int r = tid; r < nrows; r += kPT) L.pdfl[r] = (short)p.loop_pdf[row0 + r];
  }
  if (tid < 3 * kPWords) st_agent(pring + ((tid / kPWords) * kPR + rank) * kPWords + tid % kPWords, __uint_as_float(kRingSentinel));
  if (!team_barrier(ctl, team, nbar, L.abort)) return;
  uint64_t cmask = 0;
  for (int k = 0; k < kSegs * kPW; ++k) {
    const int q = L.wcrow[k];
    bool mine = false;
#pragma unroll
    for (int i = 0; i < PSPT; ++i) mine = mine || (st_ok[i] && q == tid + i * kPT);
    if (q >= 0 && mine) cmask |= 1ull << k;
  }

  const size_t f0 = (size_t)g * (d.Tmax + 1);
  cgfloat* xv_g = G(p.xv) + (size_t)g * d.Tmax * V;
  cgfloat* xl_g = G(d.xl) + (size_t)g * d.Tmax * S;
  float xl_cur[PSPT], xl_prev[PSPT], xl_next[PSPT], xw[PSPT], bh[PSPT];
  const float cst_last = 1.0f / d.pi_sum + d.leaky;
#pragma unroll
  for (int i = 0; i < PSPT; ++i) { bh[i] = cst_last; xl_cur[i] = 0.f; }
  cgfloat* xp_g = G(p.xv) + (size_t)g * d.Tmax * d.P;
  auto prefetch = [&](int t) {
    if (xg) {
      cgfloat* row = xp_g + (size_t)t * d.P;
#pragma unroll
      for (int i = 0; i < PSPT; ++i) {
        const int r = per_frame<STREAM>(tid + i * kPT);
        const int pl = st_ok[i] ? L.pdfl[r] : -1, pv = r < nvirt ? L.pdfv[r] : -1;
        xl_next[i] = st_ok[i] ? (pl >= 0 ? row[pl] : 1.f) : 0.f;
        xw[i] = r < nvirt ? (pv >= 0 ? row[pv] : 1.f) : 0.f;
      }
      return;
    }
#pragma unroll
    for (int i = 0; i < PSPT; ++i) {
      const int r = per_frame<STREAM>(tid + i * kPT);
      if constexpr (STREAM) {
        xl_next[i] = st_ok[i] ? ld_uniform_base(xl_g + ((size_t)t * S + row0), r) : 0.f;
        xw[i] = r < nvirt ? ld_uniform_base(xv_g + ((size_t)t * V + vfirst), r) : 0.f;
      } else {
        xl_next[i] = st_ok[i] ? once_load<!STREAM>(&xl_g[(size_t)t * S + row0 + r]) : 0.f;
        xw[i] = r < nvirt ? once_load<!STREAM>(&xv_g[(size_t)t * V + vfirst + r]) : 0.f;
      }
    }
  };
  auto stage_x = [&]() {
#pragma unroll
    for (int i = 0; i < PSPT; ++i) {
      const int r = tid + i * kPT;
      if (r < nvirt) L.xown[r] = xw[i];
    }
  };
  auto emit = [&](int t) {
    gfloat* ring_n = ring + (size_t)(t & 1) * p.rpad + vfirst;
    float pB = 0.f, pU = 0.f;
#pragma unroll
    for (int i = 0; i < PSPT; ++i) {
      if (!st_ok[i]) continue;
      for (int q = st_v0[i]; q < st_v1[i]; ++q) {
        const float w = L.xown[q] * bh[i];
        ring_store(ring_n + q, w);
        pB = fmaf(w, L.leak[q], pB); pU = fmaf(w, L.aux[q], pU);
      }
      if (st_pl[i] > 0.f) { const float lp = st_pl[i] * xl_prev[i] * bh[i]; pB = fmaf(st_pi[i], lp, pB); pU += lp; }
    }
    wait_stores();
    block_sum2<kPW>(pB, pU, L.red);
    if (tid < 2) st_agent(word_of(pring, t, rank, tid), tid == 0 ? pB : pU);
    if (tid == 0) {
      G(d.bpart)[((f0 + t - 1) * kPR + rank) * 2] = pB;
      G(d.bpart)[((f0 + t - 1) * kPR + rank) * 2 + 1] = pU;
    }
  };
  prefetch(T - 1);
#pragma unroll
  for (int i = 0; i < PSPT; ++i) xl_prev[i] = xl_next[i];
  stage_x();
  __syncthreads();
  emit(T);
#pragma unroll
  for (int i = 0; i < PSPT; ++i) xl_cur[i] = xl_prev[i];
  if (T >= 2) prefetch(T - 2);
#pragma unroll
  for (int i = 0; i < PSPT; ++i) xl_prev[i] = xl_next[i];
  float vs_hist[PSPT];
#pragma unroll
  for (int i = 0; i < PSPT; ++i) vs_hist[i] = 0.f;
  auto history = [&](int tt) {
    gfloat* bx_t = G(d.beta) + (f0 + tt) * (size_t)V * d.brec;
#pragma unroll
    for (int i = 0; i < PSPT; ++i)
      if (st_ok[i]) once_store<!STREAM>(&bx_t[(size_t)(vfirst + st_v0[i]) * d.brec], vs_hist[i]);
  };
  if constexpr (STREAM) stream_prime(o, st);
  Spin spin(ctl);
  DP_T0();
  for (int t = T - 1; t >= 0; --t) {
    DP_TL(1, 0);
    DP_TLSET(1);
    cgfloat* src_t = ring + (size_t)((t + 1) & 1) * p.rpad;
    poll_words(pring + (size_t)((t + 1) % 3) * kPR * kPWords, 0, 2, spin, L);
    __syncthreads();
    DP_TL(1, 1);
    if (*L.abort) return;
    const float lB = L.tot[0], lU = L.tot[1];
    if (tid == 0) L.abort[8] = 0;
    const bool publish = t > 0;
    if (tid < 2 && publish) st_agent(word_of(pring, t + 2, rank, tid), __uint_as_float(kRingSentinel));
    frame_rows<STREAM>(o, src_t, rank, rs, fr, plan, st, L, dp_, [&]() {
      if (publish) stage_x();
      if (kLateHistory<STREAM> && t + 1 < T) history(t + 1);
      if (t >= 2) prefetch(t - 2);
    }, publish);
    DP_TL(1, 4);
    if constexpr (STREAM) lds_only_barrier(); else __syncthreads();
    const float cu = lB + d.wu * lU;
    const float inv_c = cu > 0.f ? 1.0f / cu : 0.f;
    const float lkr = d.leaky * lB * inv_c;
    float vs[PSPT];
#pragma unroll
    for (int i = 0; i < PSPT; ++i) {
      vs[i] = 0.f;
      if (!st_ok[i]) continue;
      float v = row_val<STREAM>(L, cmask, tid + i * kPT);
      if (st_pl[i] > 0.f) v += st_pl[i] * xl_cur[i] * bh[i];
      vs[i] = v;
      bh[i] = v * inv_c + lkr;
    }
    DP_T(5);
    DP_TL(1, 5);
    if (publish) emit(t);
    DP_T(6);
    DP_TL(1, 6);
#pragma unroll
    for (int i = 0; i < PSPT; ++i) {
      vs_hist[i] = vs[i];
      xl_cur[i] = xl_prev[i];
      xl_prev[i] = xl_next[i];
    }
    if (!kLateHistory<STREAM>) history(t);
    DP_T(7);
  }
  if (kLateHistory<STREAM> && T > 0) history(0);
  DP_FLUSH(1);
}

__global__ void __launch_bounds__(kPT) den_persist2_kernel(const DenPersist2Params* __restrict__ pp_, DenPersistCtl* ctl) {
  CParams2* pp = (CParams2*)pp_;
  CParams2& p = *pp;
  const Lds2 L = carve_lds2(p.tfloats, p.cap, p.rowarrays);
  int& s_abort = L.abort[0];
  int& s_rank = L.abort[1]; int& s_team = L.abort[2]; int& s_xcd = L.abort[3]; int& s_task = L.abort[4];
  const int tid = threadIdx.x;
  if (tid == 0) {
    s_abort = 0;
    const unsigned xcd = den_xcc_id();
    const unsigned slot = __hip_atomic_fetch_add(&ctl->arrive[xcd], 1u, __ATOMIC_RELAXED, __HIP_MEMORY_SCOPE_AGENT);
    s_rank = (int)(slot % kPR); s_team = (int)(slot / kPR); s_xcd = (int)xcd;
  }
  __syncthreads();
  if (s_team >= kMaxTeams) return;
  const int rank = s_rank;
  DenPersistCtl::Team* team = &ctl->team[s_xcd][s_team];
  const size_t ti = (size_t)s_xcd * kMaxTeams + s_team;
  float* ring = p.ring + ti * 2 * p.rpad;
  float* pring = p.pring + ti * 3 * kPR * kPWords;
  unsigned nbar = 0;
  for (int iter = 0; iter <= kMaxTasks; ++iter) {
    if (tid == 0) {
      unsigned k;
      if (rank == 0) {
        k = __hip_atomic_fetch_add(&ctl->next_task, 1u, __ATOMIC_RELAXED, __HIP_MEMORY_SCOPE_AGENT);
        __hip_atomic_store(&team->task[iter], k + 1u, __ATOMIC_RELAXED, __HIP_MEMORY_SCOPE_AGENT);
      } else {
        Spin spin(ctl);
        unsigned k1;
        while ((k1 = ld_agent_u(G(&team->task[iter]))) == 0u) {
          if (spin.expired()) { s_abort = 1; k1 = 1u << 30; break; }
        }
        k = k1 - 1u;
      }
      s_task = (int)k;
    }
    __syncthreads();
    const int k = s_task;
    if (s_abort || k >= p.ntasks) return;
    const int g = p.task_seq[k], T = p.d.lengths[g];
    if (!team_barrier(ctl, team, &nbar, &s_abort)) return;
    if (p.task_dir[k] == 2) {
      if (rank == 0) {
        if (tid < 128) {
          NumParams np = pp_->np;
          num_fwd_bwd_two_waves(np, g, den_persist2_smem);
        } else {
#pragma unroll
          for (int q = 0; q < kNumTwoWaveBarriers; ++q) __syncthreads();
        }
        __syncthreads();
        if (tid == 0) __hip_atomic_fetch_add(&ctl->done, 1u, __ATOMIC_RELAXED, __HIP_MEMORY_SCOPE_AGENT);
      }
      continue;
    }
    if (p.task_dir[k] == 0) {
      if (p.fwd_stream) { if (p.pspt == 2) run_fwd2<true, 2>(pp, ctl, team, &nbar, g, T, rank, ring, pring); else if (p.pspt == 3) run_fwd2<true, 3>(pp, ctl, team, &nbar, g, T, rank, ring, pring); else run_fwd2<true, kPSPT>(pp, ctl, team, &nbar, g, T, rank, ring, pring); }
      else { if (p.pspt == 2) run_fwd2<false, 2>(pp, ctl, team, &nbar, g, T, rank, ring, pring); else if (p.pspt == 3) run_fwd2<false, 3>(pp, ctl, team, &nbar, g, T, rank, ring, pring); else run_fwd2<false, kPSPT>(pp, ctl, team, &nbar, g, T, rank, ring, pring); }
    } else {
      if (p.bwd_stream) { if (p.pspt == 2) run_bwd2<true, 2>(pp, ctl, team, &nbar, g, T, rank, ring, pring); else if (p.pspt == 3) run_bwd2<true, 3>(pp, ctl, team, &nbar, g, T, rank, ring, pring); else run_bwd2<true, kPSPT>(pp, ctl, team, &nbar, g, T, rank, ring, pring); }
      else { if (p.pspt == 2) run_bwd2<false, 2>(pp, ctl, team, &nbar, g, T, rank, ring, pring); else if (p.pspt == 3) run_bwd2<false, 3>(pp, ctl, team, &nbar, g, T, rank, ring, pring); else run_bwd2<false, kPSPT>(pp, ctl, team, &nbar, g, T, rank, ring, pring); }
    }
    __syncthreads();
    if (s_abort) return;
    if (tid == 0 && rank == 0) __hip_atomic_fetch_add(&ctl->done, 1u, __ATOMIC_RELAXED, __HIP_MEMORY_SCOPE_AGENT);
  }
}

__global__ void den_persist2_check(DenPersistCtl* ctl, int ntasks, float* den_lp, int n, unsigned* guard_dev, unsigned* guard_host) {
  const bool bad = ctl->abort != 0u || ctl->done != (unsigned)ntasks;
  __syncthreads();
  for (unsigned i = threadIdx.x; i < sizeof(DenPersistCtl) / sizeof(unsigned); i += blockDim.x) reinterpret_cast<unsigned*>(ctl)[i] = 0u;
  if (bad) {
    if (threadIdx.x == 0) persist_guard_raise(guard_dev, guard_host);
    for (int i = threadIdx.x; i < n; i += blockDim.x) den_lp[i] = __uint_as_float(0x7fc00000u);
  }
}

static PersistFamily g_den_persist2("den_persist2");
static std::map<DevStream, DenPersistScratch> g_den2_scratch;

static int den2_rpad(const pk2_den_graph* g) { return (std::max(g->S, g->V) + 255) / 256 * 256 + 256; }
static int den2_tfloats(const pk2_den_graph* g) { return std::max(g->h_p2fwd.tfloats, g->h_p2bwd.tfloats); }

bool den_persist2_fits(const pk2_den_graph* g) {
  return g->h_p2fwd.ok && g->h_p2bwd.ok && g->p2_cap > 0 && den_persist2_lds_bytes(den2_tfloats(g), g->p2_cap, g->p2_rowarrays) <= kDenPersist2MaxLds;
}

bool den_persist2_usable(const pk2_den_graph* g) { return g_den_persist2.usable() && den_persist2_fits(g); }

static int den_persist_scratch_alloc(DenPersistScratch& sc, size_t params_bytes, int rpad, size_t* ring_bytes) {
  *ring_bytes = 0;
  if (!sc.ctl) PK2_HIP(hipMalloc(reinterpret_cast<void**>(&sc.ctl), sizeof(DenPersistCtl)));
  if (!sc.params) PK2_HIP(hipMalloc(&sc.params, params_bytes));
  if (!sc.pring) PK2_HIP(hipMalloc(reinterpret_cast<void**>(&sc.pring), (size_t)8 * kMaxTeams * 3 * kPR * kPWords * sizeof(float)));
  if (sc.rpad < rpad) {
    if (sc.ring) PK2_HIP(hipFree(sc.ring));
    sc.ring = nullptr; sc.rpad = 0;
    const size_t bytes = (size_t)8 * kMaxTeams * 2 * rpad * sizeof(float);
    PK2_HIP(hipMalloc(reinterpret_cast<void**>(&sc.ring), bytes));
    sc.rpad = rpad;
    *ring_bytes = bytes;
  }
  return PK2_OK;
}

static int den_persist_tasks(const int32_t* lengths_host, int N, short (&task_seq)[kMaxTasks], unsigned char (&task_dir)[kMaxTasks]) {
  std::vector<std::pair<int, int>> order;
  for (int n = 0; n < N; ++n)
    if (lengths_host[n] > 0) { order.push_back({-lengths_host[n], 2 * n}); order.push_back({-lengths_host[n], 2 * n + 1}); }
  std::sort(order.begin(), order.end());
  const int ntasks = (int)order.size();
  for (int k = 0; k < kMaxTasks; ++k) { task_seq[k] = 0; task_dir[k] = 0; }
  for (int k = 0; k < ntasks; ++k) { task_seq[k] = (short)(order[k].second >> 1); task_dir[k] = (unsigned char)(order[k].second & 1); }
  return ntasks;
}

int den_persist2_launch(pk2_den_graph* g, const DenParams& dp, const float* xv, const int32_t* lengths_host, int N,
                        hipStream_t stream, bool* ran, const NumDeferred* tail, bool* num_ran, bool xgather) {
  *ran = false;
  if (num_ran) *num_ran = false;
  DenPersistScratch& sc = g_den2_scratch[dev_stream(stream)];
  const int rpad = den2_rpad(g);
  size_t ring_bytes;
  int rc = den_persist_scratch_alloc(sc, sizeof(DenPersist2Params), rpad, &ring_bytes);
  if (rc) return rc;
  if (ring_bytes) PK2_HIP(hipMemsetAsync(sc.ring, 0, ring_bytes, stream));
  DenPersist2Params p;
  memset(static_cast<void*>(&p), 0, sizeof(p));
  p.d = dp;
  p.fwd = g->p2fwd; p.bwd = g->p2bwd;
  p.xv = xv; p.ring = sc.ring; p.pring = sc.pring;
  p.vpdf = g->d_vpdf; p.loop_pdf = g->d_loop_pdf; p.xgather = xgather ? 1 : 0; p.rowarrays = g->p2_rowarrays;
  p.rpad = rpad; p.tfloats = den2_tfloats(g); p.cap = g->p2_cap;
  p.pspt = g->p2_cap <= 2 * kPT ? 2 : (g->p2_cap <= 3 * kPT ? 3 : kPSPT);
  p.fwd_stream = (!g->h_p2fwd.sends.empty() || g->h_p2fwd.K > 2) ? 1 : 0;
  p.bwd_stream = (!g->h_p2bwd.sends.empty() || g->h_p2bwd.K > 2) ? 1 : 0;
  p.ntasks = den_persist_tasks(lengths_host, N, p.task_seq, p.task_dir);
  sc.ntasks = 0;
  if (p.ntasks == 0) { *ran = true; return PK2_OK; }
  const bool with_num = tail && tail->valid && tail->stage && num_ran && g_den_persist2.verified() && tail->N == N &&
                        tail->lds <= (size_t)den2_tfloats(g) * sizeof(float) && p.ntasks + N <= kMaxTasks;
  if (with_num) {
    p.np = tail->p;
    for (int n = 0; n < N; ++n) { p.task_seq[p.ntasks] = (short)n; p.task_dir[p.ntasks] = 2; ++p.ntasks; }
  }
  const size_t lds = den_persist2_lds_bytes(p.tfloats, p.cap, p.rowarrays);
  PK2_DYN_LDS_ONCE(den_persist2_kernel, 160 * 1024);
  if (!sc.ctl_clean) PK2_HIP(hipMemsetAsync(sc.ctl, 0, sizeof(DenPersistCtl), stream));
  sc.ctl_clean = false;
  DenPersist2Params* params = static_cast<DenPersist2Params*>(sc.params);
  {
    const unsigned char* pb = reinterpret_cast<const unsigned char*>(&p);
    if (sc.params_host.size() != sizeof(p) || memcmp(sc.params_host.data(), pb, sizeof(p)) != 0) {
      hipLaunchKernelGGL(param_block_store<DenPersist2Params>, dim3(1), dim3(1), 0, stream, p, params);
      sc.params_host.assign(pb, pb + sizeof(p));
    }
  }
  hipLaunchKernelGGL(den_persist2_kernel, dim3(8 * kPR), dim3(kPT), lds, stream, params, sc.ctl);
#ifdef PK2_DP_PROFILE
  { int tot = 0; for (int n = 0; n < N; ++n) tot += lengths_host[n];
    hipLaunchKernelGGL(dp_prof_print, dim3(1), dim3(1), 0, stream, std::max(1, tot / 4)); }
#endif
  PK2_LAUNCH_CHECK();
  bool ok = false;
  rc = g_den_persist2.verify_first_use(&sc.ctl->abort, &sc.ctl->done, (unsigned)p.ntasks, stream, &ok);
  if (rc || !ok) return rc;
  sc.ntasks = p.ntasks;
  *ran = true;
  if (with_num) {
    *num_ran = true;
    num_route().carrier = kNumPersist; num_route().threads = 128;
  }
  return PK2_OK;
}

void den_persist2_check_launch(float* den_lp, int N, hipStream_t stream) {
  DenPersistScratch& sc = g_den2_scratch[dev_stream(stream)];
  const PersistGuard guard = persist_guard_or_null();
  if (sc.ctl && sc.ntasks > 0) {
    hipLaunchKernelGGL(den_persist2_check, dim3(1), dim3(256), 0, stream, sc.ctl, sc.ntasks, den_lp, N, guard.dev, guard.host_dev);
    sc.ctl_clean = true;
  }
}

bool den_persist2_tail_check(hipStream_t stream, DenTailCheck* ck) {
  DenPersistScratch& sc = g_den2_scratch[dev_stream(stream)];
  const PersistGuard guard = persist_guard_or_null();
  if (!sc.ctl || sc.ntasks <= 0) return false;
  ck->ctl = reinterpret_cast<unsigned*>(sc.ctl);
  ck->ctl_words = (int)(sizeof(DenPersistCtl) / sizeof(unsigned));
  ck->ntasks = sc.ntasks;
  ck->abort_word = &sc.ctl->abort; ck->done_word = &sc.ctl->done; ck->count_word = &sc.ctl->pad[0];
  ck->guard_dev = guard.dev; ck->guard_host = guard.host_dev;
  sc.ctl_clean = true;
  return true;
}

}
```

pykaldi2_amd/csrc/chain_graph.hip:

```cpp
#include <algorithm>
#include <cmath>
#include <cstdlib>
#include <cstring>
#include <numeric>

#include "chain_internal.h"
#include "den_persist.h"
#include "openfst_io.h"

namespace pk2 {

static void build_ordering(int64_t A, int num_rows, const int32_t* key, const int32_t* a,
                           const int32_t* b, const float* prob, const float* piprob,
                           HostOrdering* out, const int32_t* group_of_row = nullptr,
                           bool want4 = true, bool want2 = true, bool true_ends = false) {
  std::vector<int64_t> ptr(num_rows + 1, 0);
  for (int64_t i = 0; i < A; ++i) ptr[key[i] + 1]++;
  for (int r = 0; r < num_rows; ++r) ptr[r + 1] += ptr[r];
  std::vector<int64_t> perm(A);
  {
    std::vector<int64_t> cur(ptr.begin(), ptr.end() - 1);
    for (int64_t i = 0; i < A; ++i) perm[cur[key[i]]++] = i;
  }
  out->arcs.clear(); out->meta.clear(); out->wb_off.assign(1, 0);
// ... 178 lines not shown
    b = std::max(1, std::min(b, trows - 1));
    out->K = 2;
    out->cbeg[0] = 0; out->cbeg[1] = std::min(R, b * 256); out->cbeg[2] = R;
    out->lds_off[0] = 0; out->lds_off[1] = 0;
    out->tfloats = std::max(b, trows - b) * 256;
    for (int c = 3; c <= kMaxChunks; ++c) out->cbeg[c] = R;
    return true;
  }
  const int H = tcap / 2 / 256 * 256;
  if (H < 256) return false;
  const int K = (R + H - 1) / H;
  if (K > kMaxChunks) return false;
  out->K = K;
  for (int c = 0; c <= kMaxChunks; ++c) out->cbeg[c] = std::min(R, c * H);
  for (int c = 0; c < K; ++c) out->lds_off[c] = (c & 1) * H;
  out->tfloats = 2 * H;
  return true;
}

static void persist2_deal(int64_t n, int spt, const std::vector<int32_t>& srow, std::vector<int64_t>& sarc, const int32_t* lidx,
                          std::vector<int32_t>& sidx, int null_base, int null_span) {
  sidx.assign(n, null_base);
  std::vector<int32_t> load((size_t)2 * spt * 32);
  std::vector<int64_t> cand;
  for (int64_t wbase = 0; wbase < n; wbase += (int64_t)64 * spt) {
    std::fill(load.begin(), load.end(), 0);
    for (int lane = 0; lane < 64; ++lane) {
      const int half = lane >> 5;
      int64_t s = wbase + (int64_t)lane * spt;
      const int64_t lane_end = std::min<int64_t>(n, s + spt);
      while (s < lane_end) {
        int64_t e = s;
        while (e < lane_end && srow[e] == srow[s]) ++e;
        cand.assign(sarc.begin() + s, sarc.begin() + e);
        for (int64_t pos = s; pos < e; ++pos) {
          const int j = (int)(pos % spt);
          int32_t* ld = &load[((size_t)half * spt + j) * 32];
          size_t best = 0; int best_load = 1 << 30;
          for (size_t c = 0; c < cand.size(); ++c) {
            const int l = cand[c] < 0 ? -1 : ld[lidx[cand[c]] & 31];
            if (l < best_load) { best_load = l; best = c; }
          }
          const int64_t a = cand[best];
          cand[best] = cand.back(); cand.pop_back();
          sarc[pos] = a;
          if (a >= 0) {
            sidx[pos] = lidx[a];
          } else {
            int bank = null_base & 31;
            for (int b2 = 0; b2 < null_span; ++b2)
              if (ld[(null_base + b2) & 31] < ld[bank]) bank = (null_base + b2) & 31;
            int off = 0;
            while (((null_base + off) & 31) != bank) ++off;
            sidx[pos] = null_base + off;
          }
          ld[sidx[pos] & 31]++;
        }
        s = e;
      }
    }
  }
}

static void persist2_deal_rows(int64_t n, int spt, const std::vector<int32_t>& srow, std::vector<int64_t>& sarc, const int32_t* lidx,
                               std::vector<int32_t>& sidx, int null_base, int null_span, int rounds) {
  sidx.assign(n, null_base);
  if (n == 0) return;
  if (rounds < 0) {
    for (int64_t i = 0; i < n; ++i) sidx[i] = sarc[i] >= 0 ? lidx[sarc[i]] : null_base;
    return;
  }
  const int nhw = (int)((n + (int64_t)32 * spt - 1) / ((int64_t)32 * spt));
  struct Cell { int32_t addr[32]; uint8_t refs[32]; uint8_t cnt[32]; int n; };
  std::vector<Cell> cells((size_t)nhw * spt);
  for (Cell& c : cells) { c.n = 0; for (int b = 0; b < 32; ++b) c.cnt[b] = 0; }
  auto cell_of = [&](int64_t pos) -> Cell& { return cells[(size_t)(pos / ((int64_t)32 * spt)) * spt + (size_t)(pos % spt)]; };
  auto put = [&](int64_t pos, int addr) {
    Cell& c = cell_of(pos);
    for (int k = 0; k < c.n; ++k) if (c.addr[k] == addr) { c.refs[k]++; return; }
    c.addr[c.n] = addr; c.refs[c.n] = 1; c.n++; c.cnt[addr & 31]++;
  };
  auto take = [&](int64_t pos, int addr) {
    Cell& c = cell_of(pos);
    for (int k = 0; k < c.n; ++k)
      if (c.addr[k] == addr) {
        if (--c.refs[k] == 0) { c.cnt[addr & 31]--; c.n--; c.addr[k] = c.addr[c.n]; c.refs[k] = c.refs[c.n]; }
        return;
      }
  };
  auto cost = [&](int64_t pos, int addr) {
    const Cell& c = cell_of(pos);
    for (int k = 0; k < c.n; ++k) if (c.addr[k] == addr) return -1;
    return (int)c.cnt[addr & 31];
  };
  auto null_addr = [&](int64_t pos) {
    int best = null_base, best_c = 1 << 30;
    for (int b2 = 0; b2 < null_span; ++b2) { const int c = cost(pos, null_base + b2); if (c < best_c) { best_c = c; best = null_base + b2; } }
    return best;
  };
  std::vector<int64_t> cand;
  auto deal_row = [&](int64_t s, int64_t e) {
    cand.assign(sarc.begin() + s, sarc.begin() + e);
    for (int64_t pos = s; pos < e; ++pos) {
      size_t best = 0; int best_c = 1 << 30;
      const size_t lim = std::min<size_t>(cand.size(), 256);
      for (size_t c = 0; c < lim; ++c) {
        const int cc = cand[c] < 0 ? 1 << 20 : cost(pos, lidx[cand[c]]);
        if (cc < best_c) { best_c = cc; best = c; }
      }
      const int64_t a = cand[best];
      cand[best] = cand.back(); cand.pop_back();
      sarc[pos] = a;
      sidx[pos] = a >= 0 ? lidx[a] : null_addr(pos);
      put(pos, sidx[pos]);
    }
  };
  for (int64_t s = 0; s < n;) {
    int64_t e = s;
    while (e < n && srow[e] == srow[s]) ++e;
    deal_row(s, e);
    s = e;
  }
  for (int r = 0; r < rounds; ++r)
    for (int64_t s = 0; s < n;) {
      int64_t e = s;
      while (e < n && srow[e] == srow[s]) ++e;
      for (int64_t pos = s; pos < e; ++pos) take(pos, sidx[pos]);
      deal_row(s, e);
      s = e;
    }
}

static bool persist2_arc_lists(int64_t A, const int32_t* idx, const HostPersist2& h, int estep, const std::vector<int64_t>& ptr,
                               const std::vector<int64_t>& perm, std::vector<uint8_t>* chunk_out, std::vector<int32_t>* lidx_out) {
  const int K = h.K;
  std::vector<uint8_t>& chunk = *chunk_out; std::vector<int32_t>& lidx = *lidx_out;
  chunk.assign(A, 0); lidx.assign(A, 0);
  for (int64_t i = 0; i < A; ++i) {
    int c = 0;
    while (c + 1 < K && idx[i] >= h.cbeg[c + 1]) ++c;
    chunk[i] = (uint8_t)c;
    lidx[i] = h.lds_off[c] + (idx[i] - h.cbeg[c]);
    if (lidx[i] >= 65536) return false;
  }
  if (!h.flexible) return true;
  auto pad = [&](int64_t x) { return x == 0 ? 0 : (estep - x % estep) % estep; };
  for (int r = 0; r < kPR; ++r) {
    int64_t elig = 0, all = 0;
    for (int q = h.row_begin[r]; q < h.row_begin[r + 1]; ++q)
      for (int64_t k = ptr[q]; k < ptr[q + 1]; ++k) { ++all; if (chunk[perm[k]] == 0) ++elig; }
    if (elig == 0) continue;
    const double keep = std::min(1.0, (double)all / 2.0 / (double)elig);
    double err = 0.0;
    for (int q = h.row_begin[r]; q < h.row_begin[r + 1]; ++q) {
      int64_t e = 0, o = 0;
      for (int64_t k = ptr[q]; k < ptr[q + 1]; ++k) (chunk[perm[k]] == 0 ? e : o)++;
      if (e == 0) continue;
      const double t = keep * (double)e + err;
      int64_t best = -1; double best_cost = 1e30;
      const int64_t lo = std::max<int64_t>(0, (int64_t)std::floor(t) - estep), hi = std::min<int64_t>(e, (int64_t)std::ceil(t) + estep);
      for (int64_t a = lo; a <= hi; ++a) {
        const double cost = (double)(pad(a) + pad(e - a + o)) + 0.01 * std::fabs((double)a - t);
        if (cost < best_cost) { best_cost = cost; best = a; }
      }
      err = t - (double)best;
      int64_t kept = 0;
      for (int64_t k = ptr[q]; k < ptr[q + 1]; ++k) {
        if (chunk[perm[k]] != 0) continue;
        if (kept < best) ++kept; else chunk[perm[k]] = 1;
      }
    }
  }
  return true;
}

static bool persist2_lists(int64_t A, int num_rows, const float* prob, const float* piprob, const std::vector<int64_t>& ptr,
                           const std::vector<int64_t>& perm, const std::vector<uint8_t>& chunk, const std::vector<int32_t>& lidx,
                           int estep, int res, bool deal, HostPersist2* out) {
  out->estep = estep;
  const int K = out->K;
  out->prob.assign((size_t)kPR * kPSlots, 0.f);
  out->idx2.assign((size_t)kPR * kPSlots / 2, 0u);
  out->ends.assign((size_t)kPR * 2 * kPT, 0u);
  out->first_row.assign((size_t)kPR * 2 * kPT, 0);
  out->uncovered.assign((size_t)kPR * 2, 0);
  out->ncomp.assign((size_t)kPR * 2, 0);
  out->rmap.assign((size_t)2 * num_rows, (int16_t)-1);
  out->pbeg.assign((size_t)kPR * (kMaxChunks + 1), 0);
  out->sfirst_row.assign((size_t)kPR * kMaxChunks * kPT, 0);
  out->wcrow.assign((size_t)kPR * kSegs * kPW, -1);
  out->row_leak.assign(num_rows, 0.f);
  out->row_psum.assign(num_rows, 0.f);
  out->sprob.clear(); out->sidx2.clear(); out->sends.clear();
  out->resident_slots = out->streamed_slots = 0;
  out->max_pieces = 0;
  std::vector<int32_t> srow, scomp, sidx; std::vector<int64_t> sarc; std::vector<char> send;
  int npieces = 0;
  int null_base[kMaxChunks], null_span[kMaxChunks];
  for (int c = 0; c < K; ++c) {
    const int cc = out->cbeg[c + 1] > out->cbeg[c] ? c : 0;
    null_base[c] = out->lds_off[cc];
    null_span[c] = std::max(1, std::min(32, out->cbeg[cc + 1] - out->cbeg[cc]));
  }
  for (int r = 0; r < kPR; ++r) {
    const int row0 = out->row_begin[r], row1 = out->row_begin[r + 1];
    for (int q = row0; q < row1; ++q) {
      double leak = 0.0, psum = 0.0;
      for (int64_t k = ptr[q]; k < ptr[q + 1]; ++k) { leak += (double)piprob[perm[k]]; psum += (double)prob[perm[k]]; }
      out->row_leak[q] = (float)leak; out->row_psum[q] = (float)psum;
    }
    int rank_pieces = 0;
    for (int c = 0; c < K; ++c) {
      srow.clear(); scomp.clear(); sarc.clear(); send.clear();
      int ncomp = 0;
      for (int q = row0; q < row1; ++q) {
        const size_t before = srow.size();
        for (int64_t k = ptr[q]; k < ptr[q + 1]; ++k)
          if (chunk[perm[k]] == c) { srow.push_back(q - row0); scomp.push_back(ncomp); sarc.push_back(perm[k]); send.push_back(0); }
        if (srow.size() == before) continue;
        while ((srow.size() - before) % estep) { srow.push_back(q - row0); scomp.push_back(ncomp); sarc.push_back(-1); send.push_back(0); }
        send.back() = 1;
        if (c < 2) out->rmap[(size_t)c * num_rows + q] = (int16_t)ncomp;
        ++ncomp;
      }
      const int64_t n = (int64_t)srow.size();
      const int64_t nres = c < 2 ? std::min<int64_t>(n, (int64_t)res * kPT) : 0;
      if (c < 2) {
        std::vector<int32_t> rrow(scomp.begin(), scomp.begin() + nres);
        std::vector<int64_t> rarc(sarc.begin(), sarc.begin() + nres);
        persist2_deal_rows(nres, res, rrow, rarc, lidx.data(), sidx, null_base[c], null_span[c], deal ? 2 : -1);
        for (int tid = 0; tid < kPT; ++tid) {
          uint32_t e = 0;
          for (int j = 0; j < res; ++j) {
            const int64_t s = (int64_t)tid * res + j;
            if (s >= nres) break;
            const int jj = c * kQ + j;
            out->prob[((size_t)r * kPK + jj) * kPT + tid] = rarc[s] >= 0 ? prob[rarc[s]] : 0.f;
            out->idx2[((size_t)r * (kPK / 2) + jj / 2) * kPT + tid] |= (uint32_t)sidx[s] << (16 * (jj & 1));
            if (send[s]) e |= 1u << j;
          }
          out->ends[((size_t)r * 2 + c) * kPT + tid] = e;
          const int64_t s0 = (int64_t)tid * res;
          out->first_row[((size_t)r * 2 + c) * kPT + tid] = s0 < nres ? scomp[s0] : 0;
        }
        for (int w = 0; w < kPW; ++w) {
          const int64_t last = (int64_t)(w + 1) * 64 * res - 1;
          if (last < nres && !send[last]) out->wcrow[((size_t)r * kSegs + c) * kPW + w] = srow[last];
        }
        out->uncovered[(size_t)r * 2 + c] = nres < n ? scomp[nres] : ncomp;
        out->ncomp[(size_t)r * 2 + c] = ncomp;
        out->resident_slots += nres;
      }
      out->pbeg[(size_t)r * (kMaxChunks + 1) + c] = npieces;
      if (nres == n) continue;
      {
        std::vector<int32_t> rrow; std::vector<int64_t> rarc; std::vector<char> rend;
        int64_t s = nres;
        for (int q = srow[nres]; q < row1 - row0; ++q) {
          const size_t before = rrow.size();
          while (s < n && srow[s] == q) { if (sarc[s] >= 0) { rrow.push_back(q); rarc.push_back(sarc[s]); rend.push_back(0); } ++s; }
          if (rrow.size() == before) { rrow.push_back(q); rarc.push_back(-1); rend.push_back(0); }
          while ((rrow.size() - before) % estep) { rrow.push_back(q); rarc.push_back(-1); rend.push_back(0); }
          rend.back() = 1;
        }
        const int64_t ns = (int64_t)rrow.size();
        const int pieces = (int)((ns + (int64_t)kPT * kSP - 1) / ((int64_t)kPT * kSP));
        const int spt = pieces * kSP;
        if (deal) persist2_deal(ns, spt, rrow, rarc, lidx.data(), sidx, null_base[c], null_span[c]);
        else { sidx.assign(ns, null_base[c]); for (int64_t i = 0; i < ns; ++i) if (rarc[i] >= 0) sidx[i] = lidx[rarc[i]]; }
        out->sprob.resize((size_t)(npieces + pieces) * kSP * kPT, 0.f);
        out->sidx2.resize((size_t)(npieces + pieces) * (kSP / 2) * kPT, 0u);
        out->sends.resize((size_t)(npieces + pieces) * kPT, 0u);
        const uint32_t null_pair = (uint32_t)null_base[c] | ((uint32_t)null_base[c] << 16);
        for (size_t k = (size_t)npieces * (kSP / 2) * kPT; k < out->sidx2.size(); ++k) out->sidx2[k] = null_pair;
        for (int tid = 0; tid < kPT; ++tid) {
          for (int p = 0; p < spt; ++p) {
            const int64_t s2 = (int64_t)tid * spt + p;
            if (s2 >= ns) break;
            const int piece = npieces + p / kSP, j = p % kSP;
            out->sprob[((size_t)piece * kPT + tid) * kSP + j] = rarc[s2] >= 0 ? prob[rarc[s2]] : 0.f;
            uint32_t& w2 = out->sidx2[((size_t)piece * kPT + tid) * (kSP / 2) + j / 2];
            w2 = (w2 & ~(0xffffu << (16 * (j & 1)))) | ((uint32_t)sidx[s2] << (16 * (j & 1)));
            if (rend[s2]) out->sends[(size_t)piece * kPT + tid] |= 1u << j;
          }
          const int64_t s0 = (int64_t)tid * spt;
          out->sfirst_row[((size_t)r * kMaxChunks + c) * kPT + tid] = s0 < ns ? rrow[s0] : 0;
        }
        for (int w = 0; w < kPW; ++w) {
          const int64_t last = (int64_t)(w + 1) * 64 * spt - 1;
          if (last < ns && !rend[last]) out->wcrow[((size_t)r * kSegs + 2 + c) * kPW + w] = rrow[last];
        }
        npieces += pieces;
        rank_pieces += pieces;
        out->streamed_slots += ns;
      }
    }
    for (int c = K; c <= kMaxChunks; ++c) out->pbeg[(size_t)r * (kMaxChunks + 1) + c] = npieces;
    out->max_pieces = std::max(out->max_pieces, rank_pieces);
  }
  out->ok = true;
  return true;
}

static void build_persist2(pk2_den_graph* g, int64_t A2, const int32_t* arc_v, const int32_t* src2, const float* prob2,
                           const float* piprob2, const int32_t* vstate) {
  HostPersist2& f = g->h_p2fwd; HostPersist2& b = g->h_p2bwd;
  f = HostPersist2(); b = HostPersist2();
  g->p2_cap = 0;
  const int S = g->S, V = g->V;
  if (V >= 65536 || S >= 65536) { if (getenv("PK2_DP2_DEBUG")) fprintf(stderr, "persist2: bail at line %d\n", __LINE__); return; }
  bool assigned = false;
  for (int lim : {2 * kPT, 3 * kPT, kPMaxRows}) {
    if (!persist2_assign(A2, V, arc_v, vstate, S, lim, &f) || !persist2_assign(A2, S, src2, nullptr, S, lim, &b)) continue;
    b.max_groups = 0;
    for (int r = 0; r < kPR; ++r) b.max_groups = std::max(b.max_groups, g->voff[b.row_begin[r + 1]] - g->voff[b.row_begin[r]]);
    if (b.max_groups > lim) continue;
    assigned = true;
    break;
  }
  if (!assigned && persist2_assign(A2, V, arc_v, vstate, S, kPMaxRows, &f, true) && persist2_assign(A2, S, src2, nullptr, S, kPMaxRows, &b, true)) {
    b.max_groups = 0;
    for (int r = 0; r < kPR; ++r) b.max_groups = std::max(b.max_groups, g->voff[b.row_begin[r + 1]] - g->voff[b.row_begin[r]]);
    assigned = b.max_groups <= kPMaxRows;
    if (assigned && getenv("PK2_DP2_DEBUG")) fprintf(stderr, "persist2: ranks dealt by rows (%d / %d rows on the largest)\n", f.max_rows, b.max_rows);
  }
  if (!assigned) { if (getenv("PK2_DP2_DEBUG")) fprintf(stderr, "persist2: bail at line %d\n", __LINE__); return; }
  const int cap = (std::max({f.max_rows, f.max_groups, b.max_rows, b.max_groups, 1}) + 3) / 4 * 4;
  auto tcap_for = [&](int arrays) { return ((int64_t)kDenPersist2MaxLds / 4 - arrays * (int64_t)cap - kP2FixedFloats) / 512 * 512; };
  g->p2_rowarrays = kP2RowArrays;
  if (tcap_for(kP2RowArrays) >= 512) {
    for (int which = 0; which < 2; ++which) {
      HostPersist2 with = which == 0 ? f : b, without = with;
      const int rows = which == 0 ? V : S, R = which == 0 ? S : V;
      const int32_t* idx = which == 0 ? src2 : arc_v;
      const bool ok8 = persist2_chunks(A2, idx, R, rows, (int)tcap_for(kP2RowArrays), &with);
      const bool ok7 = persist2_chunks(A2, idx, R, rows, (int)tcap_for(kP2RowArrays - 1), &without);
      if (ok7 && (!ok8 || without.K < with.K)) g->p2_rowarrays = kP2RowArrays - 1;
    }
  } else {
    g->p2_rowarrays = kP2RowArrays - 1;
  }
  if (const char* env = getenv("PK2_DP2_ROWARRAYS")) g->p2_rowarrays = atoi(env) == 7 ? 7 : 8;
  int64_t tcap = tcap_for(g->p2_rowarrays);
  if (const char* env = getenv("PK2_DP2_TCAP")) tcap = std::min<int64_t>(tcap, std::max(512, atoi(env) / 512 * 512));
  if (tcap < 512) { if (getenv("PK2_DP2_DEBUG")) fprintf(stderr, "persist2: bail at line %d\n", __LINE__); return; }
  int res = kQ;
  if (const char* env = getenv("PK2_DP2_RES")) res = std::max(1, std::min(kQ, atoi(env)));
  const char* env_e = getenv("PK2_DEN_ESTEP");
  const int forced = env_e ? atoi(env_e) : 0;
  auto arcs_us = [](int e) { return e == 1 ? 3.1 : e == 2 ? 1.8 : e == 4 ? 1.55 : 1.45; };
  for (int which = 0; which < 2; ++which) {
    HostPersist2& h = which == 0 ? f : b;
    const int rows = which == 0 ? V : S, R = which == 0 ? S : V;
    const int32_t* key = which == 0 ? arc_v : src2;
    const int32_t* idx = which == 0 ? src2 : arc_v;
    if (!persist2_chunks(A2, idx, R, rows, (int)tcap, &h)) { if (getenv("PK2_DP2_DEBUG")) fprintf(stderr, "persist2: bail at line %d\n", __LINE__); f.ok = b.ok = false; return; }
    std::vector<int64_t> ptr(rows + 1, 0);
    for (int64_t i = 0; i < A2; ++i) ptr[key[i] + 1]++;
    for (int r = 0; r < rows; ++r) ptr[r + 1] += ptr[r];
    std::vector<int64_t> perm(A2);
    {
      std::vector<int64_t> cur(ptr.begin(), ptr.end() - 1);
      for (int64_t i = 0; i < A2; ++i) perm[cur[key[i]]++] = i;
    }
    int best_estep = 0; double best_cost = 1e30;
    std::vector<uint8_t> list_of; std::vector<int32_t> lidx;
    for (int estep : {8, 4, 2, 1}) {
      if ((forced > 0 && estep != forced) || res % estep != 0) continue;
      HostPersist2 cand = h;
      if (!persist2_arc_lists(A2, idx, cand, estep, ptr, perm, &list_of, &lidx) ||
          !persist2_lists(A2, rows, prob2, piprob2, ptr, perm, list_of, lidx, estep, res, false, &cand)) { if (getenv("PK2_DP2_DEBUG")) fprintf(stderr, "persist2: bail at line %d\n", __LINE__); f.ok = b.ok = false; return; }
      const double cost = arcs_us(estep) + (cand.max_pieces ? 4.5 + 0.9 * cand.max_pieces : 0.0);
      if (cost < best_cost) { best_cost = cost; best_estep = estep; }
      if (cand.max_pieces == 0 && cand.K == 2) break;
    }
    if (best_estep == 0) { if (getenv("PK2_DP2_DEBUG")) fprintf(stderr, "persist2: bail at line %d\n", __LINE__); f.ok = b.ok = false; return; }
    if (!persist2_arc_lists(A2, idx, h, best_estep, ptr, perm, &list_of, &lidx) ||
        !persist2_lists(A2, rows, prob2, piprob2, ptr, perm, list_of, lidx, best_estep, res, true, &h)) { f.ok = b.ok = false; return; }
    if (getenv("PK2_DP2_DEBUG")) fprintf(stderr, "persist2: %s rows padded to %d slots, %d table chunks, at most %d streamed pieces per rank\n", which == 0 ? "fwd" : "bwd", best_estep, h.K, h.max_pieces);
  }
  if (!(f.ok && b.ok)) { if (getenv("PK2_DP2_DEBUG")) fprintf(stderr, "persist2: bail at line %d\n", __LINE__); f.ok = b.ok = false; return; }
  g->p2_cap = cap;
}

static int build_graph_ordered(int32_t S, int32_t P, int64_t A, const int32_t* src_in, const int32_t* dst_in,
                               const int32_t* pdf, const float* prob, int32_t start, const char* order_mode,
                               pk2_den_graph** out) {
  PK2_REQUIRE(S > 0 && P > 0 && A > 0 && start >= 0 && start < S, "den graph: bad sizes");
  PK2_REQUIRE(P <= 65536, "den graph: num_pdfs %d > 65536 unsupported", P);
  for (int64_t i = 0; i < A; ++i) {
    PK2_REQUIRE(src_in[i] >= 0 && src_in[i] < S && dst_in[i] >= 0 && dst_in[i] < S && pdf[i] >= 0 && pdf[i] < P,
                "den graph: arc %lld out of range", (long long)i);
  }
  auto* g = new pk2_den_graph();
  g->S = S; g->P = P; g->A = A;
  std::vector<int32_t> new_of(S), src_v(A), dst_v(A);
  {
    std::vector<int32_t> order(S);
    std::iota(order.begin(), order.end(), 0);
    const char* env = order_mode;
    if (!(env && strcmp(env, "none") == 0)) {
      std::vector<int64_t> deg(S, 0);
      const bool both = env && strcmp(env, "degree") == 0;
      for (int64_t i = 0; i < A; ++i) { deg[dst_in[i]]++; if (both) deg[src_in[i]]++; }
      std::stable_sort(order.begin(), order.end(), [&](int32_t a, int32_t b) { return deg[a] > deg[b]; });
    }
    for (int32_t k = 0; k < S; ++k) new_of[order[k]] = k;
    g->orig_of = order;
    for (int64_t i = 0; i < A; ++i) { src_v[i] = new_of[src_in[i]]; dst_v[i] = new_of[dst_in[i]]; }
    start = new_of[start];
  }
  const int32_t* src = src_v.data();
  const int32_t* dst = dst_v.data();
  g->start = start;
  {
    std::vector<double> cur(S, 0.0), nxt(S), avg(S, 0.0);
    cur[start] = 1.0;
    const int iters = 100;
    for (int it = 0; it < iters; ++it) {
      for (int s = 0; s < S; ++s) avg[s] += cur[s] / iters;
      std::fill(nxt.begin(), nxt.end(), 0.0);
      for (int64_t i = 0; i < A; ++i) nxt[dst[i]] += cur[src[i]] * (double)prob[i];
      double tot = 0.0;
      for (int s = 0; s < S; ++s) tot += nxt[s];
      for (int s = 0; s < S; ++s) cur[s] = nxt[s] / tot;
    }
    g->pi.resize(S);
    double ps = 0.0;
    for (int s = 0; s < S; ++s) { g->pi[s] = (float)avg[s]; ps += (double)g->pi[s]; }
    g->pi_sum = ps;
  }
  std::vector<float> piprob(A);
  for (int64_t i = 0; i < A; ++i) piprob[i] = g->pi[src[i]] * prob[i];
  build_ordering(A, S, dst, src, pdf, prob, piprob.data(), &g->h_fwd, nullptr, true, false);
  build_ordering(A, S, src, dst, pdf, prob, piprob.data(), &g->h_bwd, nullptr, true, false);
  build_ordering(A, P, pdf, src, dst, prob, piprob.data(), &g->h_gam, nullptr, true, false);
  {
    const char* peel_env = getenv("PK2_DEN_PEEL");
    const bool peel = !(peel_env && atoi(peel_env) == 0);
    g->loop_pdf.assign(S, -1);
    g->loop_prob.assign(S, 0.f);
    std::vector<int64_t> keep;
    keep.reserve(A);
    for (int64_t i = 0; i < A; ++i) {
      if (peel && src[i] == dst[i] && g->loop_pdf[src[i]] < 0 && prob[i] > 0.f) {
        g->loop_pdf[src[i]] = pdf[i];
        g->loop_prob[src[i]] = prob[i];
      } else {
        keep.push_back(i);
      }
    }
    const int64_t A2 = (int64_t)keep.size();
    std::vector<int32_t> src2(A2), dst2(A2), pdf2(A2);
    std::vector<float> prob2(A2), piprob2(A2);
    for (int64_t k = 0; k < A2; ++k) {
      const int64_t i = keep[k];
      src2[k] = src[i]; dst2[k] = dst[i]; pdf2[k] = pdf[i]; prob2[k] = prob[i]; piprob2[k] = piprob[i];
    }
    std::vector<int64_t> order(A2);
    std::iota(order.begin(), order.end(), (int64_t)0);
    std::sort(order.begin(), order.end(), [&](int64_t x, int64_t y) {
      return dst2[x] != dst2[y] ? dst2[x] < dst2[y] : pdf2[x] < pdf2[y];
    });
    std::vector<int32_t> arc_v(A2);
    g->voff.assign(S + 1, 0);
    g->vpdf.clear();
    std::vector<int32_t> vstate;
    int64_t k = 0;
    for (int d = 0; d < S; ++d) {
      g->voff[d] = (int32_t)g->vpdf.size();
      if (k == A2 || dst2[order[k]] != d) { g->vpdf.push_back(-1); vstate.push_back(d); continue; }
      while (k < A2 && dst2[order[k]] == d) {
        const int32_t q = pdf2[order[k]];
        g->vpdf.push_back(q); vstate.push_back(d);
        while (k < A2 && dst2[order[k]] == d && pdf2[order[k]] == q) arc_v[order[k++]] = (int32_t)g->vpdf.size() - 1;
      }
    }
    g->V = (int32_t)g->vpdf.size();
    g->voff[S] = g->V;
    g->ooff.assign(S + 1, 0);
    g->opdf.clear(); g->ovirt.clear();
    for (int d = 0; d < S; ++d) {
      g->ooff[d] = (int32_t)g->opdf.size();
      for (int v = g->voff[d]; v < g->voff[d + 1]; ++v) { g->opdf.push_back(g->vpdf[v]); g->ovirt.push_back(g->voff[d]); }
      if (g->loop_pdf[d] >= 0) { g->opdf.push_back(g->loop_pdf[d]); g->ovirt.push_back(g->voff[d]); }
    }
    g->Vo = (int32_t)g->opdf.size();
    g->ooff[S] = g->Vo;
    build_ordering(A2, g->V, arc_v.data(), src2.data(), pdf2.data(), prob2.data(), piprob2.data(), &g->h_fwdv, vstate.data(),
                   false, true, true);
    build_ordering(A2, S, src2.data(), arc_v.data(), pdf2.data(), prob2.data(), piprob2.data(), &g->h_bwdv, nullptr, false,
                   true, true);
    build_persist2(g, A2, arc_v.data(), src2.data(), prob2.data(), piprob2.data(), vstate.data());
    g->po_off.assign(P + 1, 0);
    for (int o = 0; o < g->Vo; ++o) if (g->opdf[o] >= 0) g->po_off[g->opdf[o] + 1]++;
    for (int p = 0; p < P; ++p) g->po_off[p + 1] += g->po_off[p];
    g->po_occ.assign(std::max(1, g->po_off[P]), 0);
    std::vector<int32_t> cur(g->po_off.begin(), g->po_off.end() - 1);
    for (int o = 0; o < g->Vo; ++o) if (g->opdf[o] >= 0) g->po_occ[cur[g->opdf[o]]++] = o;
  }
  *out = g;
  return PK2_OK;
}

static int build_graph(int32_t S, int32_t P, int64_t A, const int32_t* src_in, const int32_t* dst_in,
                       const int32_t* pdf, const float* prob, int32_t start, pk2_den_graph** out) {
  const char* env = getenv("PK2_DEN_ORDER");
  if (env) return build_graph_ordered(S, P, A, src_in, dst_in, pdf, prob, start, env, out);
  int rc = build_graph_ordered(S, P, A, src_in, dst_in, pdf, prob, start, "none", out);
  if (rc) return rc;
  if (den_persist2_fits(*out)) return PK2_OK;
  delete *out;
  *out = nullptr;
  return build_graph_ordered(S, P, A, src_in, dst_in, pdf, prob, start, "indegree", out);
}

template <typename T>
static int upload_vec(pk2_den_graph* g, const std::vector<T>& v, const T** dptr) {
  void* d = nullptr;
  PK2_HIP(hipMalloc(&d, std::max<size_t>(16, v.size() * sizeof(T))));
  g->allocs.push_back(d);
  if (!v.empty()) PK2_HIP(hipMemcpy(d, v.data(), v.size() * sizeof(T), hipMemcpyHostToDevice));
  *dptr = static_cast<const T*>(d);
  return PK2_OK;
}

static int upload_persist2(pk2_den_graph* g, const HostPersist2& h, DevPersist2* d) {
  if (!h.ok) return PK2_OK;
  int rc;
  if ((rc = upload_vec(g, h.prob, &d->prob))) return rc;
  if ((rc = upload_vec(g, h.idx2, &d->idx2))) return rc;
  if ((rc = upload_vec(g, h.ends, &d->ends))) return rc;
  if ((rc = upload_vec(g, h.first_row, &d->first_row))) return rc;
  if ((rc = upload_vec(g, h.uncovered, &d->uncovered))) return rc;
  if ((rc = upload_vec(g, h.ncomp, &d->ncomp))) return rc;
  if ((rc = upload_vec(g, h.rmap, &d->rmap))) return rc;
  d->num_rows = (int)(h.rmap.size() / 2);
  if ((rc = upload_vec(g, h.pbeg, &d->pbeg))) return rc;
  if ((rc = upload_vec(g, h.sprob, &d->sprob))) return rc;
  if ((rc = upload_vec(g, h.sidx2, &d->sidx2))) return rc;
  if ((rc = upload_vec(g, h.sends, &d->sends))) return rc;
  if ((rc = upload_vec(g, h.sfirst_row, &d->sfirst_row))) return rc;
  if ((rc = upload_vec(g, h.wcrow, &d->wcrow))) return rc;
  if ((rc = upload_vec(g, h.row_begin, &d->row_begin))) return rc;
  if ((rc = upload_vec(g, h.grp_begin, &d->grp_begin))) return rc;
  if ((rc = upload_vec(g, h.row_leak, &d->row_leak))) return rc;
  if ((rc = upload_vec(g, h.row_psum, &d->row_psum))) return rc;
  d->estep = h.estep; d->K = h.K; d->R = h.R;
  for (int c = 0; c <= kMaxChunks; ++c) d->cbeg[c] = h.cbeg[c];
  for (int c = 0; c < kMaxChunks; ++c) d->lds_off[c] = h.lds_off[c];
  return PK2_OK;
}

static int upload_ordering(pk2_den_graph* g, const HostOrdering& h, DevOrdering* d) {
  int rc;
  if ((rc = upload_vec(g, h.arcs, &d->arcs))) return rc;
  if ((rc = upload_vec(g, h.arcs2, &d->arcs2))) return rc;
  if ((rc = upload_vec(g, h.row_leak, &d->row_leak))) return rc;
  if ((rc = upload_vec(g, h.slot0, &d->slot0))) return rc;
  if ((rc = upload_vec(g, h.meta, &d->meta))) return rc;
  if ((rc = upload_vec(g, h.wb_off, &d->wb_off))) return rc;
  if ((rc = upload_vec(g, h.row0, &d->row0))) return rc;
  if ((rc = upload_vec(g, h.nrows, &d->nrows))) return rc;
  if ((rc = upload_vec(g, h.atomic, &d->atomic))) return rc;
  if ((rc = upload_vec(g, h.real0, &d->real0))) return rc;
  if ((rc = upload_vec(g, h.nreal, &d->nreal))) return rc;
  if ((rc = upload_vec(g, h.wb_crow, &d->wb_crow))) return rc;
  d->n_chunks = h.n_chunks;
  return PK2_OK;
}

int den_upload(pk2_den_graph* g) {
  if (g->uploaded) return PK2_OK;
  int rc;
  PK2_HIP(hipGetDevice(&g->device));
  if ((rc = upload_ordering(g, g->h_fwd, &g->fwd))) return rc;
  if ((rc = upload_ordering(g, g->h_bwd, &g->bwd))) return rc;
  if ((rc = upload_ordering(g, g->h_gam, &g->gam))) return rc;
  if ((rc = upload_ordering(g, g->h_fwdv, &g->fwdv))) return rc;
  if ((rc = upload_ordering(g, g->h_bwdv, &g->bwdv))) return rc;
  if ((rc = upload_persist2(g, g->h_p2fwd, &g->p2fwd))) return rc;
  if ((rc = upload_persist2(g, g->h_p2bwd, &g->p2bwd))) return rc;
  if ((rc = upload_vec(g, g->voff, &g->d_voff))) return rc;
  if ((rc = upload_vec(g, g->vpdf, &g->d_vpdf))) return rc;
  if ((rc = upload_vec(g, g->loop_pdf, &g->d_loop_pdf))) return rc;
  if ((rc = upload_vec(g, g->loop_prob, &g->d_loop_prob))) return rc;
  if ((rc = upload_vec(g, g->ooff, &g->d_ooff))) return rc;
  if ((rc = upload_vec(g, g->opdf, &g->d_opdf))) return rc;
  if ((rc = upload_vec(g, g->ovirt, &g->d_ovirt))) return rc;
  if ((rc = upload_vec(g, g->po_off, &g->d_po_off))) return rc;
  if ((rc = upload_vec(g, g->po_occ, &g->d_po_occ))) return rc;
  const float* dpi = nullptr;
  {
    std::vector<float> pi_pad(g->pi);
    pi_pad.resize((pi_pad.size() + 255) / 256 * 256 + 256, 0.f);
    if ((rc = upload_vec(g, pi_pad, &dpi))) return rc;
  }
  g->d_pi = const_cast<float*>(dpi);
  g->uploaded = true;
  return PK2_OK;
}

}

using namespace pk2;

extern "C" int pk2_den_graph_create(int32_t num_states, int32_t num_pdfs, int64_t num_arcs,
                                    const int32_t* arc_src, const int32_t* arc_dst,
                                    const int32_t* arc_pdf, const float* arc_prob,
                                    int32_t start_state, pk2_den_graph** out) {
  PK2_REQUIRE(arc_src && arc_dst && arc_pdf && arc_prob && out, "den graph: null pointer");
  return build_graph(num_states, num_pdfs, num_arcs, arc_src, arc_dst, arc_pdf, arc_prob,
                     start_state, out);
}

extern "C" int pk2_den_graph_from_openfst(const char* path, int32_t num_pdfs, pk2_den_graph** out) {
  PK2_REQUIRE(path && out, "den graph: null pointer");
  FstArrays fst;
  const std::string why = read_openfst(path, &fst);
  if (!why.empty()) { set_error("%s: %s", path, why.c_str()); return PK2_ERR_IO; }
  std::vector<int32_t> pdf(fst.ilabel.size());
  std::vector<float> prob(fst.ilabel.size());
  for (size_t a = 0; a < fst.ilabel.size(); ++a) {
    if (fst.ilabel[a] <= 0) { set_error("%s: epsilon / negative ilabel in den.fst", path); return PK2_ERR_IO; }
    pdf[a] = fst.ilabel[a] - 1;
    prob[a] = expf(-fst.weight[a]);
  }
  return build_graph((int32_t)fst.num_states, num_pdfs, (int64_t)pdf.size(), fst.src.data(), fst.dst.data(),
                     pdf.data(), prob.data(), (int32_t)fst.start, out);
}

extern "C" int pk2_den_graph_destroy(pk2_den_graph* g) {
  if (!g) return PK2_OK;
  for (void* p : g->allocs) (void)hipFree(p);
  delete g;
  return PK2_OK;
}

extern "C" int pk2_den_graph_info(const pk2_den_graph* g, int32_t* num_states, int32_t* num_pdfs,
                                  int64_t* num_arcs) {
  PK2_REQUIRE(g, "den graph: null handle");
  if (num_states) *num_states = g->S;
  if (num_pdfs) *num_pdfs = g->P;
  if (num_arcs) *num_arcs = g->A;
  return PK2_OK;
}

extern "C" int pk2_den_graph_initial_probs(const pk2_den_graph* g, float* host_out) {
  PK2_REQUIRE(g && host_out, "den graph: null pointer");
  for (int32_t k = 0; k < g->S; ++k) host_out[g->orig_of[k]] = g->pi[k];
  return PK2_OK;
}

extern "C" int32_t pk2_den_graph_arcs_per_lane(void) { return kK; }

extern "C" int pk2_den_graph_debug_ordering(const pk2_den_graph* g, int which, int64_t* n_arcs_padded,
                                            int32_t* n_chunks, int32_t* arcs_out ,
                                            uint32_t* meta_out, int32_t* wb_off_out,
                                            int32_t* row0_out, int32_t* nrows_out,
                                            int32_t* atomic_out) {
  PK2_REQUIRE(g && which >= 0 && which < 5, "debug ordering: bad args");
  const HostOrdering* hs[5] = {&g->h_fwd, &g->h_bwd, &g->h_gam, &g->h_fwdv, &g->h_bwdv};
  const HostOrdering& h = *hs[which];
  const size_t n = which < 3 ? h.arcs.size() : h.arcs2.size();
  if (n_arcs_padded) *n_arcs_padded = (int64_t)n;
  if (n_chunks) *n_chunks = h.n_chunks;
  if (arcs_out && which < 3) memcpy(arcs_out, h.arcs.data(), n * sizeof(int4));
  if (arcs_out && which >= 3)
    for (size_t i = 0; i < n; ++i) {
      arcs_out[4 * i] = h.arcs2[i].x; arcs_out[4 * i + 1] = 0; arcs_out[4 * i + 2] = h.arcs2[i].y; arcs_out[4 * i + 3] = 0;
    }
  if (meta_out) memcpy(meta_out, h.meta.data(), h.meta.size() * sizeof(uint2));
  if (wb_off_out) memcpy(wb_off_out, h.wb_off.data(), h.wb_off.size() * sizeof(int32_t));
  if (row0_out) memcpy(row0_out, h.row0.data(), h.row0.size() * sizeof(int32_t));
  if (nrows_out) memcpy(nrows_out, h.nrows.data(), h.nrows.size() * sizeof(int32_t));
  if (atomic_out) memcpy(atomic_out, h.atomic.data(), h.atomic.size() * sizeof(int32_t));
  return PK2_OK;
}

extern "C" int pk2_den_graph_debug_virtual(const pk2_den_graph* g, int which, int32_t* num_virtual, int32_t* voff_out,
                                           int32_t* vpdf_out, int32_t* real0_out, int32_t* nreal_out,
                                           int32_t* slot0_out, int64_t* n_row_leak, float* row_leak_out,
                                           int32_t* loop_pdf_out, float* loop_prob_out, int32_t* num_occ,
                                           int32_t* ooff_out, int32_t* opdf_out) {
  PK2_REQUIRE(g && (which == 3 || which == 4), "debug virtual: bad args");
  const HostOrdering& h = which == 3 ? g->h_fwdv : g->h_bwdv;
  if (num_virtual) *num_virtual = g->V;
  if (num_occ) *num_occ = g->Vo;
  if (voff_out) memcpy(voff_out, g->voff.data(), g->voff.size() * sizeof(int32_t));
  if (vpdf_out) memcpy(vpdf_out, g->vpdf.data(), g->vpdf.size() * sizeof(int32_t));
  if (real0_out) memcpy(real0_out, h.real0.data(), h.real0.size() * sizeof(int32_t));
  if (nreal_out) memcpy(nreal_out, h.nreal.data(), h.nreal.size() * sizeof(int32_t));
  if (slot0_out) memcpy(slot0_out, h.slot0.data(), h.slot0.size() * sizeof(int32_t));
  if (n_row_leak) *n_row_leak = (int64_t)h.row_leak.size();
  if (row_leak_out) memcpy(row_leak_out, h.row_leak.data(), h.row_leak.size() * sizeof(float));
  if (loop_pdf_out) memcpy(loop_pdf_out, g->loop_pdf.data(), g->loop_pdf.size() * sizeof(int32_t));
  if (loop_prob_out) memcpy(loop_prob_out, g->loop_prob.data(), g->loop_prob.size() * sizeof(float));
  if (ooff_out) memcpy(ooff_out, g->ooff.data(), g->ooff.size() * sizeof(int32_t));
  if (opdf_out) memcpy(opdf_out, g->opdf.data(), g->opdf.size() * sizeof(int32_t));
  return PK2_OK;
}

extern "C" int pk2_den_graph_debug_persist2(const pk2_den_graph* g, int which, int32_t* info, float* prob, uint32_t* idx2,
                                            uint32_t* ends, int32_t* first_row, int32_t* uncovered, int32_t* ncomp, int16_t* rmap,
                                            int32_t* pbeg, float* sprob,
                                            uint32_t* sidx2, uint32_t* sends, int32_t* sfirst_row, int32_t* wcrow,
                                            int32_t* row_begin, int32_t* grp_begin, float* row_leak, float* row_psum) {
  PK2_REQUIRE(g && (which == 0 || which == 1) && info, "den graph debug: bad arguments");
  const HostPersist2& h = which == 0 ? g->h_p2fwd : g->h_p2bwd;
  for (int k = 0; k < 32; ++k) info[k] = 0;
  info[0] = h.ok ? 1 : 0; info[1] = h.estep; info[2] = h.K; info[3] = h.R; info[4] = h.tfloats; info[5] = h.max_rows;
  info[6] = h.max_groups; info[7] = (int32_t)(h.sends.size() / kPT); info[8] = g->p2_cap; info[9] = (int32_t)h.row_leak.size();
  for (int c = 0; c <= kMaxChunks; ++c) info[10 + c] = h.cbeg[c];
  static_assert(10 + kMaxChunks < 19, "info[19] is free");
  info[19] = g->p2_rowarrays;
  for (int c = 0; c < kMaxChunks; ++c) info[20 + c] = h.lds_off[c];
  info[26] = kPR; info[27] = kPT; info[28] = kPK; info[29] = kPW; info[30] = kSP; info[31] = kSegs;
  if (!h.ok) return PK2_OK;
  auto cp = [](void* dst, const void* src, size_t bytes) { if (dst && bytes) memcpy(dst, src, bytes); };
  cp(prob, h.prob.data(), h.prob.size() * 4); cp(idx2, h.idx2.data(), h.idx2.size() * 4);
  cp(ends, h.ends.data(), h.ends.size() * 4); cp(first_row, h.first_row.data(), h.first_row.size() * 4);
  cp(uncovered, h.uncovered.data(), h.uncovered.size() * 4); cp(pbeg, h.pbeg.data(), h.pbeg.size() * 4);
  cp(ncomp, h.ncomp.data(), h.ncomp.size() * 4); cp(rmap, h.rmap.data(), h.rmap.size() * 2);
  cp(sprob, h.sprob.data(), h.sprob.size() * 4); cp(sidx2, h.sidx2.data(), h.sidx2.size() * 4);
  cp(sends, h.sends.data(), h.sends.size() * 4); cp(sfirst_row, h.sfirst_row.data(), h.sfirst_row.size() * 4);
  cp(wcrow, h.wcrow.data(), h.wcrow.size() * 4); cp(row_begin, h.row_begin.data(), h.row_begin.size() * 4);
  cp(grp_begin, h.grp_begin.data(), h.grp_begin.size() * 4); cp(row_leak, h.row_leak.data(), h.row_leak.size() * 4);
  cp(row_psum, h.row_psum.data(), h.row_psum.size() * 4);
  return PK2_OK;
}
```

pykaldi2_amd/csrc/chain_internal.h:

```cpp
#pragma once
#include <type_traits>
#include <vector>

#include "common.h"

namespace pk2 {

#ifndef PK2_DEN_K
#define PK2_DEN_K 16
#endif
#ifndef PK2_DEN_CHUNK
#define PK2_DEN_CHUNK 4096
#endif
constexpr int kK = PK2_DEN_K;
static_assert(kK >= 1 && kK <= 32, "the flush mask of a lane has 32 bits");
constexpr int kChunkArcs = PK2_DEN_CHUNK;
constexpr int kMaxRows = 1024;
constexpr int kDenWaves = kChunkArcs / (64 * kK);
constexpr int kDenThreads = kDenWaves * 64;
constexpr int kDenBwdThreads = 2 * kDenThreads;

struct HostOrdering {
  std::vector<int4> arcs;
  std::vector<int2> arcs2;
  std::vector<float> row_leak;
  std::vector<int32_t> slot0;
  std::vector<uint2> meta;
  std::vector<int32_t> wb_off;
  std::vector<int32_t> row0;
  std::vector<int32_t> nrows;
  std::vector<int32_t> atomic;
  std::vector<int32_t> real0;
  std::vector<int32_t> nreal;
  std::vector<int32_t> wb_crow;
  int n_chunks = 0;
};

struct DevOrdering {
  const int4* arcs = nullptr;
  const int2* arcs2 = nullptr;
  const float* row_leak = nullptr;
  const int32_t* slot0 = nullptr;
  const uint2* meta = nullptr;
  const int32_t* wb_off = nullptr;
  const int32_t* row0 = nullptr;
  const int32_t* nrows = nullptr;
  const int32_t* atomic = nullptr;
  const int32_t* real0 = nullptr;
  const int32_t* nreal = nullptr;
  const int32_t* wb_crow = nullptr;
  int n_chunks = 0;
};

constexpr int kPR = 32;
constexpr int kPT = 512;
constexpr int kPW = kPT / 64;
constexpr int kPK = 64;
constexpr int kPSlots = kPT * kPK;
constexpr int kPSPT = 4;
constexpr int kPMaxRows = kPSPT * kPT;

constexpr int kQ = kPK / 2;
constexpr int kSP = 8;
constexpr int kMaxChunks = 6;
constexpr int kSegs = 2 + kMaxChunks;
struct HostPersist2 {
  bool ok = false;
  int estep = 1;
  int K = 0;
  int R = 0;
  int cbeg[kMaxChunks + 1] = {0};
  int lds_off[kMaxChunks] = {0};
  int tfloats = 0;
  bool flexible = false;
  int max_rows = 0, max_groups = 0;
  int64_t resident_slots = 0, streamed_slots = 0;
  int max_pieces = 0;
  std::vector<float> prob;
  std::vector<uint32_t> idx2;
  std::vector<uint32_t> ends;
  std::vector<int32_t> first_row;
  std::vector<int32_t> uncovered;
  std::vector<int32_t> ncomp;
  std::vector<int16_t> rmap;
  std::vector<int32_t> pbeg;
  std::vector<float> sprob;
  std::vector<uint32_t> sidx2;
  std::vector<uint32_t> sends;
  std::vector<int32_t> sfirst_row;
  std::vector<int32_t> wcrow;
  std::vector<int32_t> row_begin, grp_begin;
  std::vector<float> row_leak, row_psum;
};
struct DevPersist2 {
  const float* prob = nullptr; const uint32_t* idx2 = nullptr; const uint32_t* ends = nullptr; const int32_t* first_row = nullptr;
  const int32_t* uncovered = nullptr; const int32_t* ncomp = nullptr; const int16_t* rmap = nullptr; const int32_t* pbeg = nullptr;
  int num_rows = 0;
  const float* sprob = nullptr; const uint32_t* sidx2 = nullptr; const uint32_t* sends = nullptr; const int32_t* sfirst_row = nullptr;
  const int32_t* wcrow = nullptr; const int32_t* row_begin = nullptr; const int32_t* grp_begin = nullptr;
  const float* row_leak = nullptr; const float* row_psum = nullptr;
  int estep = 1, K = 0, R = 0;
  int cbeg[kMaxChunks + 1] = {0};
  int lds_off[kMaxChunks] = {0};
};

}

struct pk2_den_graph {
  int32_t S = 0, P = 0, start = 0;
  int64_t A = 0;
  std::vector<float> pi;
  std::vector<int32_t> orig_of;
  double pi_sum = 0.0;
  pk2::HostOrdering h_fwd, h_bwd, h_gam;
  int32_t V = 0, Vo = 0;
  std::vector<int32_t> voff, vpdf;
  std::vector<int32_t> loop_pdf;
  std::vector<float> loop_prob;
  std::vector<int32_t> ooff, opdf, ovirt;
  std::vector<int32_t> po_off, po_occ;
  pk2::HostOrdering h_fwdv, h_bwdv;
  pk2::HostPersist2 h_p2fwd, h_p2bwd;
  pk2::DevPersist2 p2fwd, p2bwd;
  int p2_cap = 0;
  int p2_rowarrays = 8;
  const int32_t* d_voff = nullptr;
  const int32_t* d_vpdf = nullptr;
  const int32_t* d_loop_pdf = nullptr;
  const float* d_loop_prob = nullptr;
  const int32_t* d_ooff = nullptr;
  const int32_t* d_opdf = nullptr;
  const int32_t* d_ovirt = nullptr;
  const int32_t* d_po_off = nullptr;
  const int32_t* d_po_occ = nullptr;
  bool uploaded = false;
  int device = -1;
  pk2::DevOrdering fwd, bwd, gam, fwdv, bwdv;
  float* d_pi = nullptr;
  std::vector<void*> allocs;
};

namespace pk2 {

struct DenEnv {
  int mode = -1;
  int persist = -1;
  bool merge = true;
  bool xgather = true;
  bool num_ride = true;
  bool exp_gather = false, gamma_gather = false;
  bool test_fail = false;
  int debug = 0;
  float beta_seed = 1.0f;
};

enum DenExpKernel { kExpPrep1, kExpRows, kExpStatesLds, kExpStates, kExpTranspose };

struct DenPlan {
  int rc = 0;
  int N, Tmax;
  int NG;
  int NG_frames;
  int G;
  bool sx;
  int form;
  bool need_fill;
  bool xgather;
  bool prep_merged;
  bool tail_mergeable;
  bool gamma_lds;
  DenExpKernel exp_kernel;
  int ncf, ncb;
  DenEnv env;
};
DenPlan den_plan(const pk2_den_graph* g, int N, int Tmax);

struct DenBuffers {
  float* alpha;
  float* alphav;
  float* xl;
  float* beta;
  float* xs;
  float* gamma;
  float* apart;
  float* bpart;
  float* asum;
  float* inv_tot;
  float* den_lp;
  float* check;
  int32_t* lengths;
  float* csum;
  float* kscale;
  float* xv;
};

size_t den_workspace(const pk2_den_graph* g, int N, int Tmax, DenPlan* plan, DenBuffers* buf,
                     void* base);
struct NumDeferred;
int den_upload(pk2_den_graph* g);
struct DenZeroRows { float* grad = nullptr; int64_t gss = 0, gfs = 0; int N = 0; };
int den_compute(pk2_den_graph* g, const float* logits, int64_t seq_stride, int64_t frame_stride,
                const int32_t* lengths_host, const DenPlan& plan, const DenBuffers& buf,
                float leaky, hipStream_t stream, const NumDeferred* tail = nullptr, const DenZeroRows* zero = nullptr);

struct SideStream { hipStream_t stream = nullptr; hipEvent_t fork = nullptr, join = nullptr; };
int get_side_stream(hipStream_t main, SideStream** out);
void den_gamma_out_launch(const DenPlan& plan, const DenBuffers& b, int P, float scale, float* out,
                          int64_t ss, int64_t fs, hipStream_t stream);

template <typename F>
auto dispatch_ng(int ng, F&& fn) {
  switch (ng) {
    case 4: return fn(std::integral_constant<int, 4>{});
    case 2: return fn(std::integral_constant<int, 2>{});
    default: return fn(std::integral_constant<int, 1>{});
  }
}

struct NumParams {
  const int32_t* arc_src; const int32_t* arc_dst; const int32_t* arc_pdf; const float* arc_w;
  const int32_t* frame_off; const int32_t* final_state; const float* final_w;
  const int32_t* seqinfo;
  const float* logits; int64_t seq_stride, frame_stride;
  float* score; float* frame_max; float* num_lp;
  float* grad; int64_t gseq_stride, gframe_stride;
  float scale;
};

enum NumCarrier {
  kNumCarrierNone = 0,
  kNumStandAlone = 1,
  kNumGammaLds = 2,
  kNumGammaGather = 3,
  kNumPersist = 4,
  kNumSideStream = 5,
};
struct NumRoute { int32_t staged = 0, carrier = kNumCarrierNone, threads = 0, lds_bytes = 0; };
NumRoute& num_route();

struct NumDeferred { NumParams p; size_t lds = 0; int N = 0; bool valid = false; bool stage = false; };
int num_launch_deferred(const NumDeferred& d, hipStream_t stream);

struct NumBuffers {
  float* score;
  float* frame_max;
  int32_t* seqinfo;
  float* num_lp;
};
size_t num_workspace(int N, int64_t total_arcs, int64_t total_frames, NumBuffers* buf, void* base);
int num_compute(const pk2_num_batch* nb, const float* logits, int64_t seq_stride,
                int64_t frame_stride, const int32_t* lengths_host, int N, float scale, float* grad,
                int64_t grad_seq_stride, int64_t grad_frame_stride, const NumBuffers& buf,
                hipStream_t stream, NumDeferred* defer = nullptr);

}
```

Baseline: 4682.

## Split persistent denominator arc table into shared prefix plus per-thread direct arcs

Graph setup now separates low-fan-in source entries from the LDS-resident table. It reorders state positions so only high-degree entries form a smaller table prefix. The low-degree arcs (up to two per thread) are handled as direct register-held arcs that read their source values straight from global memory. The persistent forward and backward kernels get a DIRECT template variant that adds these contributions and publishes ring values in the permuted order. The aim is to shrink the table chunk copied into LDS each frame, at the cost of extra per-thread global loads, more registers and more kernel instantiations.

```diff
diff --git a/pykaldi2_amd/_lib.py b/pykaldi2_amd/_lib.py
--- a/pykaldi2_amd/_lib.py
+++ b/pykaldi2_amd/_lib.py
@@ -77,6 +77,7 @@
     "pk2_den_graph_debug_virtual": (C.c_int, [_vp, C.c_int, C.POINTER(_i32), _vp, _vp, _vp, _vp, _vp,
                                               C.POINTER(_i64), _vp, _vp, _vp, C.POINTER(_i32), _vp, _vp]),
     "pk2_den_graph_debug_persist2": (C.c_int, [_vp, C.c_int] + [_vp] * 18),
+    "pk2_den_graph_debug_persist2_table": (C.c_int, [_vp, C.c_int, _vp, _vp, _vp, _vp]),
     "pk2_chain_workspace_bytes": (_sz, [_vp, _i32, _i32, _i64]),
     "pk2_chain_objf_and_deriv": (C.c_int, [_vp, _vp, _i64, _i64, _vp, _i32, C.POINTER(NumBatch), _f32,
                                            _f32, _f32, _f32, _vp, _i64, _i64, _vp, _vp, _sz, _vp]),
diff --git a/pykaldi2_amd/chain.py b/pykaldi2_amd/chain.py
--- a/pykaldi2_amd/chain.py
+++ b/pykaldi2_amd/chain.py
@@ -68,7 +68,28 @@
     def plan(self, num_seqs, max_frames):
         out = np.zeros(8, dtype=np.int32)
         _lib.check(_lib.lib().pk2_den_graph_plan(self._h, int(num_seqs), int(max_frames), _lib.ptr(out)))
-        return dict(zip(self.PLAN_FIELDS, (int(v) for v in out)))
+        pl = dict(zip(self.PLAN_FIELDS, (int(v) for v in out)))
+        for name, which in (("fwd", 0), ("bwd", 1)):
+            info = np.zeros(8, dtype=np.int32)
+            _lib.check(_lib.lib().pk2_den_graph_debug_persist2_table(self._h, which, _lib.ptr(info), None, None, None))
+            pl[name + "_table"] = (int(info[0]), int(info[1]))
+            pl[name + "_direct_arcs"] = int(info[3])
+        return pl
+
+    def debug_persist2_table(self, which):
+        L = _lib.lib()
+        info = np.zeros(8, dtype=np.int32)
+        _lib.check(L.pk2_den_graph_debug_persist2_table(self._h, which, _lib.ptr(info), None, None, None))
+        if not info[1]:
+            return None
+        lay = self.debug_persist2(which)
+        nr, nd, nt = lay["prob"].shape[0], int(info[5]), int(info[7])
+        pos = np.empty(int(info[1]), np.int32)
+        dprob, dpr = np.empty((nr, nd, nt), np.float32), np.empty((nr, nd, nt), np.uint32)
+        _lib.check(L.pk2_den_graph_debug_persist2_table(self._h, which, _lib.ptr(info), _lib.ptr(pos), _lib.ptr(dprob), _lib.ptr(dpr)))
+        return dict(Rt=int(info[0]), R=int(info[1]), table_entries=int(info[2]), direct_arcs=int(info[3]),
+                    max_direct=int(info[4]), kDirect=nd, kDirectDeg=int(info[6]), pos=pos, dprob=dprob,
+                    dpos=(dpr & 0xffff).astype(np.int64), drow=(dpr >> 16).astype(np.int64))
 
     def debug_persist2(self, which):
         L = _lib.lib()
diff --git a/pykaldi2_amd/csrc/chain_den_persist2.hip b/pykaldi2_amd/csrc/chain_den_persist2.hip
--- a/pykaldi2_amd/csrc/chain_den_persist2.hip
+++ b/pykaldi2_amd/csrc/chain_den_persist2.hip
@@ -27,6 +27,8 @@
   NumParams np;
   int fwd_stream, bwd_stream;
   int pspt;
+  int fwd_direct, bwd_direct;
+  const float* pi_pos;
   short task_seq[kMaxTasks];
   unsigned char task_dir[kMaxTasks];
 };
@@ -408,10 +410,32 @@
 };
 struct NoStream { };
 struct RowSpan { int nrows, uncA, ncA, uncB, ncB; };
-template <bool STREAM, typename ST, typename STAGE>
+struct DirectRegs {
+  float prob[kDirect]; uint32_t off[kDirect]; int row[kDirect];
+  float val[kDirect];
+  __device__ __forceinline__ float add_to(int q, float v) const {
+#pragma unroll
+    for (int j = 0; j < kDirect; ++j) v += row[j] == q ? prob[j] * val[j] : 0.f;
+    return v;
+  }
+};
+struct NoDirect { };
+__device__ __forceinline__ void load_direct_regs(CDev2& o, int rank, DirectRegs& d) {
+#pragma unroll
+  for (int j = 0; j < kDirect; ++j) {
+    const size_t at = ((size_t)rank * kDirect + j) * kPT + threadIdx.x;
+    const uint32_t pr = o.dpr[at];
+    d.prob[j] = o.dprob[at];
+    d.off[j] = (pr & 0xffffu) * 4u;
+    d.row[j] = (int)(pr >> 16);
+    d.val[j] = 0.f;
+  }
+}
+template <bool STREAM, bool DIRECT, typename DR, typename ST, typename STAGE>
 __device__ __forceinline__ void frame_rows(CDev2& o, cgfloat* src, int rank, const RowSpan& rs, const FrameRegs& r,
-                                           const DmaPlan& plan, ST& st, const Lds2& L, DpTimers& dp_, STAGE stage,
+                                           const DmaPlan& plan, DR& dr, ST& st, const Lds2& L, DpTimers& dp_, STAGE stage,
                                            bool prime_next = false) {
+  static_assert(!(STREAM && DIRECT), "direct arcs exist in the fully resident form only");
   const int tid = threadIdx.x;
   if constexpr (STREAM) {
     for (int q = tid; q < rs.nrows; q += kPT) L.accS[q] = 0.f;
@@ -424,6 +448,11 @@
   lds_only_barrier();
   DP_T(1);
   DP_TLF(2);
+  if constexpr (DIRECT) {
+    typedef __attribute__((address_space(1))) const char gchar;
+#pragma unroll
+    for (int j = 0; j < kDirect; ++j) dr.val[j] = ld_agent((cgfloat*)((gchar*)src + dr.off[j]));
+  }
   Chunk1Dma c1;
   {
     const uint64_t sb = (uint64_t)(src + o.cbeg[1]);
@@ -467,7 +496,9 @@
   } else {
     if (shared) { lds_only_barrier(); dma_chunk(src, o, 1, L.table); }
     wait_vm(0);
+    DP_T(8);
     stage();
+    DP_T(9);
     __syncthreads();
     DP_T(3);
     pass_rows_any<kQ, STREAM>(o.estep, r.prob, r.addr, r.base, r.endsB, r.frowB, L.accB, L.wcarry + kPW, NoDma());
@@ -519,7 +550,7 @@
   r.frowA = o.first_row[((size_t)rank * 2 + 0) * kPT + tid]; r.frowB = o.first_row[((size_t)rank * 2 + 1) * kPT + tid];
 }
 
-template <bool STREAM, int PSPT>
+template <bool STREAM, int PSPT, bool DIRECT>
 __device__ __noinline__ void run_fwd2(CParams2* pp_, DenPersistCtl* ctl_, DenPersistCtl::Team* team_,
                                       unsigned* nbar, int g_, int T_, int rank_, float* ring_, float* pring_) {
   CParams2* pp = uni(pp_);
@@ -538,6 +569,8 @@
   load_frame_regs<STREAM>(o, rank, fr, L.table);
   DmaPlan plan;
   plan.init(o, L.table);
+  typename std::conditional<DIRECT, DirectRegs, NoDirect>::type dr;
+  if constexpr (DIRECT) load_direct_regs(o, rank, dr);
   const int row0 = o.row_begin[rank], nrows = o.row_begin[rank + 1] - row0;
   const int g0 = o.grp_begin[rank], ngrp = o.grp_begin[rank + 1] - g0;
   RowSpan rs;
@@ -554,15 +587,18 @@
   }
   if (tid < kSegs * kPW) L.wcrow[tid] = o.wcrow[(size_t)rank * kSegs * kPW + tid];
   int st_lo[PSPT], st_hi[PSPT], st_o[PSPT]; float st_pl[PSPT], st_pi[PSPT]; bool st_ok[PSPT];
+  int st_pos[PSPT];
 #pragma unroll
   for (int i = 0; i < PSPT; ++i) {
     const int r = tid + i * kPT;
     st_ok[i] = r < ngrp;
     st_lo[i] = st_hi[i] = st_o[i] = 0; st_pl[i] = st_pi[i] = 0.f;
+    st_pos[i] = 0;
     if (st_ok[i]) {
       const int dd = g0 + r;
       st_lo[i] = d.voff[dd] - row0; st_hi[i] = d.voff[dd + 1] - row0; st_o[i] = d.ooff[dd];
       st_pl[i] = d.loop_prob[dd]; st_pi[i] = d.pi[dd];
+      if constexpr (DIRECT) st_pos[i] = o.pos[dd];
     }
   }
   if (tid < 3 * kPWords) st_agent(pring + ((tid / kPWords) * kPR + rank) * kPWords + tid % kPWords, __uint_as_float(kRingSentinel));
@@ -638,7 +674,7 @@
     DP_TLSET(0);
     if (t == 0) {
       as = d.pi_sum;
-      src = G(d.pi);
+      src = DIRECT ? G(p.pi_pos) : G(d.pi);
     } else {
       src = ring + (size_t)(t & 1) * p.rpad;
       poll_words(pring + (size_t)(t % 3) * kPR * kPWords, 0, 1, spin, L);
@@ -650,7 +686,7 @@
     }
     const bool publish = t + 1 < T;
     if (tid == 0 && publish) st_agent(word_of(pring, t + 2, rank, 0), __uint_as_float(kRingSentinel));
-    frame_rows<STREAM>(o, src, rank, rs, fr, plan, st, L, dp_, [&]() {
+    frame_rows<STREAM, DIRECT>(o, src, rank, rs, fr, plan, dr, st, L, dp_, [&]() {
 #pragma unroll
       for (int i = 0; i < PSPT; ++i) {
         const int r = tid + i * kPT;
@@ -671,12 +707,15 @@
       if (!st_ok[i]) continue;
       float sum = 0.f;
       for (int q = st_lo[i]; q < st_hi[i]; ++q) {
-        const float v = (row_val<STREAM>(L, cmask, q) + lk * L.leak[q]) * L.xown[q] * inv_as;
+        float rv = row_val<STREAM>(L, cmask, q);
+        if constexpr (DIRECT) rv = dr.add_to(q, rv);
+        const float v = (rv + lk * L.leak[q]) * L.xown[q] * inv_as;
         L.aux[q] = v;
         sum += v;
       }
       if (st_pl[i] > 0.f) { loopv[i] = (own_a[i] + lk * st_pi[i]) * st_pl[i] * xlr[i] * inv_as; sum += loopv[i]; }
-      if (publish) ring_store(ring_n + g0 + tid + i * kPT, sum);
+      if constexpr (DIRECT) { if (publish) ring_store(ring_n + st_pos[i], sum); }
+      else { if (publish) ring_store(ring_n + g0 + tid + i * kPT, sum); }
       outv[i] = sum;
       own_a[i] = sum;
       loc += sum;
@@ -700,7 +739,7 @@
   DP_FLUSH(0);
 }
 
-template <bool STREAM, int PSPT>
+template <bool STREAM, int PSPT, bool DIRECT>
 __device__ __noinline__ void run_bwd2(CParams2* pp_, DenPersistCtl* ctl_, DenPersistCtl::Team* team_,
                                       unsigned* nbar, int g_, int T_, int rank_, float* ring_, float* pring_) {
   CParams2* pp = uni(pp_);
@@ -718,6 +757,8 @@
   load_frame_regs<STREAM>(o, rank, fr, L.table);
   DmaPlan plan;
   plan.init(o, L.table);
+  typename std::conditional<DIRECT, DirectRegs, NoDirect>::type dr;
+  if constexpr (DIRECT) load_direct_regs(o, rank, dr);
   const int row0 = o.row_begin[rank], nrows = o.row_begin[rank + 1] - row0;
   const int vfirst = d.voff[row0], nvirt = d.voff[row0 + nrows] - vfirst;
   RowSpan rs;
@@ -728,14 +769,17 @@
   if constexpr (STREAM) stream_init(o, rank, st);
   if (tid < kSegs * kPW) L.wcrow[tid] = o.wcrow[(size_t)rank * kSegs * kPW + tid];
   int st_v0[PSPT], st_v1[PSPT]; float st_pl[PSPT], st_pi[PSPT]; bool st_ok[PSPT];
+  int st_p0[PSPT];
 #pragma unroll
   for (int i = 0; i < PSPT; ++i) {
     const int r = tid + i * kPT;
     st_ok[i] = r < nrows;
     st_v0[i] = st_v1[i] = 0; st_pl[i] = st_pi[i] = 0.f;
+    st_p0[i] = 0;
     if (st_ok[i]) {
       const int s = row0 + r;
       st_v0[i] = d.voff[s] - vfirst; st_v1[i] = d.voff[s + 1] - vfirst; st_pl[i] = d.loop_prob[s]; st_pi[i] = d.pi[s];
+      if constexpr (DIRECT) st_p0[i] = o.pos[vfirst + st_v0[i]];
     }
   }
   for (int r = tid; r < nvirt; r += kPT) { L.leak[r] = p.fwd.row_leak[vfirst + r]; L.aux[r] = p.fwd.row_psum[vfirst + r]; }
@@ -802,7 +846,8 @@
       if (!st_ok[i]) continue;
       for (int q = st_v0[i]; q < st_v1[i]; ++q) {
         const float w = L.xown[q] * bh[i];
-        ring_store(ring_n + q, w);
+        if constexpr (DIRECT) ring_store(ring_n - vfirst + (q == st_v0[i] ? st_p0[i] : o.pos[vfirst + q]), w);
+        else ring_store(ring_n + q, w);
         pB = fmaf(w, L.leak[q], pB); pU = fmaf(w, L.aux[q], pU);
       }
       if (st_pl[i] > 0.f) { const float lp = st_pl[i] * xl_prev[i] * bh[i]; pB = fmaf(st_pi[i], lp, pB); pU += lp; }
@@ -850,7 +895,7 @@
     if (tid == 0) L.abort[8] = 0;
     const bool publish = t > 0;
     if (tid < 2 && publish) st_agent(word_of(pring, t + 2, rank, tid), __uint_as_float(kRingSentinel));
-    frame_rows<STREAM>(o, src_t, rank, rs, fr, plan, st, L, dp_, [&]() {
+    frame_rows<STREAM, DIRECT>(o, src_t, rank, rs, fr, plan, dr, st, L, dp_, [&]() {
       if (publish) stage_x();
       if (kLateHistory<STREAM> && t + 1 < T) history(t + 1);
       if (t >= 2) prefetch(t - 2);
@@ -866,6 +911,7 @@
       vs[i] = 0.f;
       if (!st_ok[i]) continue;
       float v = row_val<STREAM>(L, cmask, tid + i * kPT);
+      if constexpr (DIRECT) v = dr.add_to(tid + i * kPT, v);
       if (st_pl[i] > 0.f) v += st_pl[i] * xl_cur[i] * bh[i];
       vs[i] = v;
       bh[i] = v * inv_c + lkr;
@@ -945,11 +991,13 @@
       continue;
     }
     if (p.task_dir[k] == 0) {
-      if (p.fwd_stream) { if (p.pspt == 2) run_fwd2<true, 2>(pp, ctl, team, &nbar, g, T, rank, ring, pring); else if (p.pspt == 3) run_fwd2<true, 3>(pp, ctl, team, &nbar, g, T, rank, ring, pring); else run_fwd2<true, kPSPT>(pp, ctl, team, &nbar, g, T, rank, ring, pring); }
-      else { if (p.pspt == 2) run_fwd2<false, 2>(pp, ctl, team, &nbar, g, T, rank, ring, pring); else if (p.pspt == 3) run_fwd2<false, 3>(pp, ctl, team, &nbar, g, T, rank, ring, pring); else run_fwd2<false, kPSPT>(pp, ctl, team, &nbar, g, T, rank, ring, pring); }
+      if (p.fwd_stream) { if (p.pspt == 2) run_fwd2<true, 2, false>(pp, ctl, team, &nbar, g, T, rank, ring, pring); else if (p.pspt == 3) run_fwd2<true, 3, false>(pp, ctl, team, &nbar, g, T, rank, ring, pring); else run_fwd2<true, kPSPT, false>(pp, ctl, team, &nbar, g, T, rank, ring, pring); }
+      else if (p.fwd_direct) { if (p.pspt == 2) run_fwd2<false, 2, true>(pp, ctl, team, &nbar, g, T, rank, ring, pring); else if (p.pspt == 3) run_fwd2<false, 3, true>(pp, ctl, team, &nbar, g, T, rank, ring, pring); else run_fwd2<false, kPSPT, true>(pp, ctl, team, &nbar, g, T, rank, ring, pring); }
+      else { if (p.pspt == 2) run_fwd2<false, 2, false>(pp, ctl, team, &nbar, g, T, rank, ring, pring); else if (p.pspt == 3) run_fwd2<false, 3, false>(pp, ctl, team, &nbar, g, T, rank, ring, pring); else run_fwd2<false, kPSPT, false>(pp, ctl, team, &nbar, g, T, rank, ring, pring); }
     } else {
-      if (p.bwd_stream) { if (p.pspt == 2) run_bwd2<true, 2>(pp, ctl, team, &nbar, g, T, rank, ring, pring); else if (p.pspt == 3) run_bwd2<true, 3>(pp, ctl, team, &nbar, g, T, rank, ring, pring); else run_bwd2<true, kPSPT>(pp, ctl, team, &nbar, g, T, rank, ring, pring); }
-      else { if (p.pspt == 2) run_bwd2<false, 2>(pp, ctl, team, &nbar, g, T, rank, ring, pring); else if (p.pspt == 3) run_bwd2<false, 3>(pp, ctl, team, &nbar, g, T, rank, ring, pring); else run_bwd2<false, kPSPT>(pp, ctl, team, &nbar, g, T, rank, ring, pring); }
+      if (p.bwd_stream) { if (p.pspt == 2) run_bwd2<true, 2, false>(pp, ctl, team, &nbar, g, T, rank, ring, pring); else if (p.pspt == 3) run_bwd2<true, 3, false>(pp, ctl, team, &nbar, g, T, rank, ring, pring); else run_bwd2<true, kPSPT, false>(pp, ctl, team, &nbar, g, T, rank, ring, pring); }
+      else if (p.bwd_direct) { if (p.pspt == 2) run_bwd2<false, 2, true>(pp, ctl, team, &nbar, g, T, rank, ring, pring); else if (p.pspt == 3) run_bwd2<false, 3, true>(pp, ctl, team, &nbar, g, T, rank, ring, pring); else run_bwd2<false, kPSPT, true>(pp, ctl, team, &nbar, g, T, rank, ring, pring); }
+      else { if (p.pspt == 2) run_bwd2<false, 2, false>(pp, ctl, team, &nbar, g, T, rank, ring, pring); else if (p.pspt == 3) run_bwd2<false, 3, false>(pp, ctl, team, &nbar, g, T, rank, ring, pring); else run_bwd2<false, kPSPT, false>(pp, ctl, team, &nbar, g, T, rank, ring, pring); }
     }
     __syncthreads();
     if (s_abort) return;
@@ -1026,6 +1074,9 @@
   p.pspt = g->p2_cap <= 2 * kPT ? 2 : (g->p2_cap <= 3 * kPT ? 3 : kPSPT);
   p.fwd_stream = (!g->h_p2fwd.sends.empty() || g->h_p2fwd.K > 2) ? 1 : 0;
   p.bwd_stream = (!g->h_p2bwd.sends.empty() || g->h_p2bwd.K > 2) ? 1 : 0;
+  p.fwd_direct = (!p.fwd_stream && g->h_p2fwd.Rt < g->h_p2fwd.R) ? 1 : 0;
+  p.bwd_direct = (!p.bwd_stream && g->h_p2bwd.Rt < g->h_p2bwd.R) ? 1 : 0;
+  p.pi_pos = g->d_pi_pos;
   p.ntasks = den_persist_tasks(lengths_host, N, p.task_seq, p.task_dir);
   sc.ntasks = 0;
   if (p.ntasks == 0) { *ran = true; return PK2_OK; }
diff --git a/pykaldi2_amd/csrc/chain_graph.hip b/pykaldi2_amd/csrc/chain_graph.hip
--- a/pykaldi2_amd/csrc/chain_graph.hip
+++ b/pykaldi2_amd/csrc/chain_graph.hip
@@ -504,6 +504,80 @@
   return true;
 }
 
+struct P2Split {
+  int Rt = 0, table_entries = 0;
+  std::vector<int32_t> pos, key, idx;
+  std::vector<float> prob, piprob;
+  std::vector<int64_t> direct;
+};
+static inline int persist2_owner(const HostPersist2& h, const int32_t* group_of_row, int rank, int q) {
+  return (group_of_row ? group_of_row[q] - h.grp_begin[rank] : q - h.row_begin[rank]) % kPT;
+}
+static bool persist2_table_split(int64_t A, const int32_t* key, const int32_t* idx, const float* prob, const float* piprob, int R,
+                                 const int32_t* group_of_row, const HostPersist2& h, P2Split* sp) {
+  const int full_rows = (R + 255) / 256;
+  std::vector<int32_t> cnt(R, 0);
+  for (int64_t i = 0; i < A; ++i) cnt[idx[i]]++;
+  std::vector<char> tab(R);
+  for (int e = 0; e < R; ++e) tab[e] = cnt[e] > kDirectDeg;
+  const int num_rows = h.row_begin[kPR];
+  std::vector<int32_t> slot_of(num_rows, 0);
+  for (int r = 0; r < kPR; ++r)
+    for (int q = h.row_begin[r]; q < h.row_begin[r + 1]; ++q) slot_of[q] = r * kPT + persist2_owner(h, group_of_row, r, q);
+  std::vector<int32_t>& pos = sp->pos;
+  pos.assign(R, 0);
+  for (;;) {
+    int nt = 0;
+    for (int e = 0; e < R; ++e) nt += tab[e];
+    const int Rt = std::max(256, (nt + 255) / 256 * 256);
+    if (Rt / 256 >= full_rows) return false;
+    int pt = 0, pn = nt;
+    for (int e = 0; e < R; ++e) pos[e] = tab[e] ? pt++ : pn++;
+    sp->Rt = Rt; sp->table_entries = nt;
+    std::vector<std::pair<int32_t, int32_t>> mine;
+    for (int64_t i = 0; i < A; ++i) if (pos[idx[i]] >= Rt) mine.push_back({slot_of[key[i]], idx[i]});
+    std::stable_sort(mine.begin(), mine.end(), [&](const std::pair<int32_t, int32_t>& x, const std::pair<int32_t, int32_t>& y) {
+      return x.first != y.first ? x.first < y.first : cnt[x.second] > cnt[y.second];
+    });
+    bool fits = true;
+    for (size_t k = 0; k < mine.size();) {
+      size_t e = k;
+      while (e < mine.size() && mine[e].first == mine[k].first) ++e;
+      if (e - k > (size_t)kDirect) {
+        fits = false;
+        for (size_t m = k; m + kDirect < e; ++m) tab[mine[m].second] = 1;
+      }
+      k = e;
+    }
+    if (fits) break;
+  }
+  sp->key.clear(); sp->idx.clear(); sp->prob.clear(); sp->piprob.clear(); sp->direct.clear();
+  for (int64_t i = 0; i < A; ++i) {
+    if (pos[idx[i]] >= sp->Rt) { sp->direct.push_back(i); continue; }
+    sp->key.push_back(key[i]); sp->idx.push_back(pos[idx[i]]); sp->prob.push_back(prob[i]); sp->piprob.push_back(piprob[i]);
+  }
+  return !sp->key.empty();
+}
+
+static void persist2_direct(const P2Split& sp, const int32_t* key, const int32_t* idx, const float* prob, const int32_t* group_of_row,
+                            HostPersist2* h) {
+  h->dprob.assign((size_t)kPR * kDirect * kPT, 0.f);
+  h->dpr.assign((size_t)kPR * kDirect * kPT, 0xffff0000u);
+  h->ndirect = (int64_t)sp.direct.size();
+  h->max_direct = 0;
+  std::vector<int32_t> used((size_t)kPR * kPT, 0), per_rank(kPR, 0);
+  for (int64_t i : sp.direct) {
+    int r = 0;
+    while (key[i] >= h->row_begin[r + 1]) ++r;
+    const int tid = persist2_owner(*h, group_of_row, r, key[i]);
+    const int j = used[(size_t)r * kPT + tid]++;
+    const size_t at = ((size_t)r * kDirect + j) * kPT + tid;
+    h->dprob[at] = prob[i];
+    h->dpr[at] = (uint32_t)sp.pos[idx[i]] | ((uint32_t)(key[i] - h->row_begin[r]) << 16);
+    h->max_direct = std::max(h->max_direct, ++per_rank[r]);
+  }
+}
+
 static void build_persist2(pk2_den_graph* g, int64_t A2, const int32_t* arc_v, const int32_t* src2, const float* prob2,
                            const float* piprob2, const int32_t* vstate) {
   HostPersist2& f = g->h_p2fwd; HostPersist2& b = g->h_p2bwd;
@@ -551,35 +625,79 @@
   const char* env_e = getenv("PK2_DEN_ESTEP");
   const int forced = env_e ? atoi(env_e) : 0;
   auto arcs_us = [](int e) { return e == 1 ? 3.1 : e == 2 ? 1.8 : e == 4 ? 1.55 : 1.45; };
-  for (int which = 0; which < 2; ++which) {
-    HostPersist2& h = which == 0 ? f : b;
-    const int rows = which == 0 ? V : S, R = which == 0 ? S : V;
-    const int32_t* key = which == 0 ? arc_v : src2;
-    const int32_t* idx = which == 0 ? src2 : arc_v;
-    if (!persist2_chunks(A2, idx, R, rows, (int)tcap, &h)) { if (getenv("PK2_DP2_DEBUG")) fprintf(stderr, "persist2: bail at line %d\n", __LINE__); f.ok = b.ok = false; return; }
-    std::vector<int64_t> ptr(rows + 1, 0);
-    for (int64_t i = 0; i < A2; ++i) ptr[key[i] + 1]++;
+  bool prefix_ok = !getenv("PK2_DEN_ORDER") && !getenv("PK2_DP2_RES") && !getenv("PK2_DP2_TCAP") && !getenv("PK2_DP2_SHARED") &&
+                   !getenv("PK2_DP2_ROWARRAYS");
+  if (const char* env = getenv("PK2_DP2_TABLE")) prefix_ok = prefix_ok && strcmp(env, "full") != 0;
+  struct ArcSet { int64_t A; const int32_t* key; const int32_t* idx; const float* prob; const float* piprob; };
+  struct RowIndex { std::vector<int64_t> ptr, perm; };
+  auto index_rows = [](const ArcSet& a, int rows, RowIndex* out) {
+    std::vector<int64_t>& ptr = out->ptr; std::vector<int64_t>& perm = out->perm;
+    ptr.assign(rows + 1, 0);
+    for (int64_t i = 0; i < a.A; ++i) ptr[a.key[i] + 1]++;
     for (int r = 0; r < rows; ++r) ptr[r + 1] += ptr[r];
-    std::vector<int64_t> perm(A2);
-    {
-      std::vector<int64_t> cur(ptr.begin(), ptr.end() - 1);
-      for (int64_t i = 0; i < A2; ++i) perm[cur[key[i]]++] = i;
-    }
+    perm.assign(a.A, 0);
+    std::vector<int64_t> cur(ptr.begin(), ptr.end() - 1);
+    for (int64_t i = 0; i < a.A; ++i) perm[cur[a.key[i]]++] = i;
+  };
+  auto pick_estep = [&](const ArcSet& a, const RowIndex& ri, int rows, const HostPersist2& h, bool* resident) {
     int best_estep = 0; double best_cost = 1e30;
+    *resident = false;
     std::vector<uint8_t> list_of; std::vector<int32_t> lidx;
     for (int estep : {8, 4, 2, 1}) {
       if ((forced > 0 && estep != forced) || res % estep != 0) continue;
       HostPersist2 cand = h;
-      if (!persist2_arc_lists(A2, idx, cand, estep, ptr, perm, &list_of, &lidx) ||
-          !persist2_lists(A2, rows, prob2, piprob2, ptr, perm, list_of, lidx, estep, res, false, &cand)) { if (getenv("PK2_DP2_DEBUG")) fprintf(stderr, "persist2: bail at line %d\n", __LINE__); f.ok = b.ok = false; return; }
+      if (!persist2_arc_lists(a.A, a.idx, cand, estep, ri.ptr, ri.perm, &list_of, &lidx) ||
+          !persist2_lists(a.A, rows, a.prob, a.piprob, ri.ptr, ri.perm, list_of, lidx, estep, res, false, &cand)) return 0;
       const double cost = arcs_us(estep) + (cand.max_pieces ? 4.5 + 0.9 * cand.max_pieces : 0.0);
       if (cost < best_cost) { best_cost = cost; best_estep = estep; }
-      if (cand.max_pieces == 0 && cand.K == 2) break;
-    }
+      if (cand.max_pieces == 0 && cand.K == 2) { *resident = true; break; }
+    }
+    return best_estep;
+  };
+  auto lay_out = [&](const ArcSet& a, const RowIndex& ri, int rows, int estep, HostPersist2* h) {
+    std::vector<uint8_t> list_of; std::vector<int32_t> lidx;
+    return persist2_arc_lists(a.A, a.idx, *h, estep, ri.ptr, ri.perm, &list_of, &lidx) &&
+           persist2_lists(a.A, rows, a.prob, a.piprob, ri.ptr, ri.perm, list_of, lidx, estep, res, true, h);
+  };
+  for (int which = 0; which < 2; ++which) {
+    HostPersist2& h = which == 0 ? f : b;
+    const int rows = which == 0 ? V : S, R = which == 0 ? S : V;
+    const ArcSet full{A2, which == 0 ? arc_v : src2, which == 0 ? src2 : arc_v, prob2, piprob2};
+    if (!persist2_chunks(A2, full.idx, R, rows, (int)tcap, &h)) { if (getenv("PK2_DP2_DEBUG")) fprintf(stderr, "persist2: bail at line %d\n", __LINE__); f.ok = b.ok = false; return; }
+    RowIndex ri;
+    index_rows(full, rows, &ri);
+    bool resident = false;
+    const int best_estep = pick_estep(full, ri, rows, h, &resident);
     if (best_estep == 0) { if (getenv("PK2_DP2_DEBUG")) fprintf(stderr, "persist2: bail at line %d\n", __LINE__); f.ok = b.ok = false; return; }
-    if (!persist2_arc_lists(A2, idx, h, best_estep, ptr, perm, &list_of, &lidx) ||
-        !persist2_lists(A2, rows, prob2, piprob2, ptr, perm, list_of, lidx, best_estep, res, true, &h)) { f.ok = b.ok = false; return; }
-    if (getenv("PK2_DP2_DEBUG")) fprintf(stderr, "persist2: %s rows padded to %d slots, %d table chunks, at most %d streamed pieces per rank\n", which == 0 ? "fwd" : "bwd", best_estep, h.K, h.max_pieces);
+    bool done = false;
+    P2Split sp;
+    if (prefix_ok && resident && h.flexible && persist2_table_split(full.A, full.key, full.idx, full.prob, full.piprob, R, which == 0 ? vstate : nullptr, h, &sp)) {
+      HostPersist2 hp = h;
+      const ArcSet tab{(int64_t)sp.key.size(), sp.key.data(), sp.idx.data(), sp.prob.data(), sp.piprob.data()};
+      RowIndex rt;
+      index_rows(tab, rows, &rt);
+      bool res_p = false;
+      int ep = 0;
+      if (persist2_chunks(tab.A, tab.idx, sp.Rt, rows, (int)tcap, &hp) && hp.flexible && (ep = pick_estep(tab, rt, rows, hp, &res_p)) != 0 &&
+          res_p && lay_out(tab, rt, rows, ep, &hp)) {
+        hp.R = R; hp.tfloats = h.tfloats; hp.Rt = sp.Rt; hp.table_entries = sp.table_entries;
+        hp.pos = sp.pos;
+        for (int q = 0; q < rows; ++q) {
+          double leak = 0.0, psum = 0.0;
+          for (int64_t k = ri.ptr[q]; k < ri.ptr[q + 1]; ++k) { leak += (double)piprob2[ri.perm[k]]; psum += (double)prob2[ri.perm[k]]; }
+          hp.row_leak[q] = (float)leak; hp.row_psum[q] = (float)psum;
+        }
+        persist2_direct(sp, full.key, full.idx, full.prob, which == 0 ? vstate : nullptr, &hp);
+        h = hp;
+        done = true;
+        if (getenv("PK2_DP2_DEBUG")) fprintf(stderr, "persist2: %s table prefix %d of %d entries, %lld direct arcs (at most %d per rank)\n", which == 0 ? "fwd" : "bwd", h.Rt, R, (long long)h.ndirect, h.max_direct);
+      }
+    }
+    if (!done) {
+      if (!lay_out(full, ri, rows, best_estep, &h)) { f.ok = b.ok = false; return; }
+      h.Rt = R; h.table_entries = R;
+    }
+    if (getenv("PK2_DP2_DEBUG")) fprintf(stderr, "persist2: %s rows padded to %d slots, %d table chunks, at most %d streamed pieces per rank\n", which == 0 ? "fwd" : "bwd", h.estep, h.K, h.max_pieces);
   }
   if (!(f.ok && b.ok)) { if (getenv("PK2_DP2_DEBUG")) fprintf(stderr, "persist2: bail at line %d\n", __LINE__); f.ok = b.ok = false; return; }
   g->p2_cap = cap;
@@ -749,6 +867,11 @@
   if ((rc = upload_vec(g, h.row_leak, &d->row_leak))) return rc;
   if ((rc = upload_vec(g, h.row_psum, &d->row_psum))) return rc;
   d->estep = h.estep; d->K = h.K; d->R = h.R;
+  if (h.Rt < h.R) {
+    if ((rc = upload_vec(g, h.pos, &d->pos))) return rc;
+    if ((rc = upload_vec(g, h.dprob, &d->dprob))) return rc;
+    if ((rc = upload_vec(g, h.dpr, &d->dpr))) return rc;
+  }
   for (int c = 0; c <= kMaxChunks; ++c) d->cbeg[c] = h.cbeg[c];
   for (int c = 0; c < kMaxChunks; ++c) d->lds_off[c] = h.lds_off[c];
   return PK2_OK;
@@ -799,6 +922,11 @@
     if ((rc = upload_vec(g, pi_pad, &dpi))) return rc;
   }
   g->d_pi = const_cast<float*>(dpi);
+  if (g->h_p2fwd.ok && g->h_p2fwd.Rt < g->h_p2fwd.R) {
+    std::vector<float> pi_pos((g->pi.size() + 255) / 256 * 256 + 256, 0.f);
+    for (size_t s = 0; s < g->pi.size(); ++s) pi_pos[g->h_p2fwd.pos[s]] = g->pi[s];
+    if ((rc = upload_vec(g, pi_pos, &g->d_pi_pos))) return rc;
+  }
   g->uploaded = true;
   return PK2_OK;
 }
@@ -931,3 +1059,19 @@
   cp(row_psum, h.row_psum.data(), h.row_psum.size() * 4);
   return PK2_OK;
 }
+
+extern "C" int pk2_den_graph_debug_persist2_table(const pk2_den_graph* g, int which, int32_t* info, int32_t* pos, float* dprob,
+                                                  uint32_t* dpr) {
+  PK2_REQUIRE(g && (which == 0 || which == 1) && info, "den graph debug: bad arguments");
+  const HostPersist2& h = which == 0 ? g->h_p2fwd : g->h_p2bwd;
+  const bool prefix = h.ok && h.Rt < h.R;
+  const int32_t v[8] = {h.ok ? h.Rt : 0, h.ok ? h.R : 0, h.ok ? h.table_entries : 0, prefix ? (int32_t)h.ndirect : 0, prefix ? h.max_direct : 0,
+                        kDirect, kDirectDeg, kPT};
+  std::copy(v, v + 8, info);
+  if (!h.ok) return PK2_OK;
+  if (pos) for (int e = 0; e < h.R; ++e) pos[e] = prefix ? h.pos[e] : e;
+  const size_t n = (size_t)kPR * kDirect * kPT;
+  if (dprob) { if (prefix) memcpy(dprob, h.dprob.data(), n * 4); else memset(dprob, 0, n * 4); }
+  if (dpr) { if (prefix) memcpy(dpr, h.dpr.data(), n * 4); else memset(dpr, 0, n * 4); }
+  return PK2_OK;
+}
diff --git a/pykaldi2_amd/csrc/chain_internal.h b/pykaldi2_amd/csrc/chain_internal.h
--- a/pykaldi2_amd/csrc/chain_internal.h
+++ b/pykaldi2_amd/csrc/chain_internal.h
@@ -64,6 +64,8 @@
 constexpr int kSP = 8;
 constexpr int kMaxChunks = 6;
 constexpr int kSegs = 2 + kMaxChunks;
+constexpr int kDirectDeg = 1;
+constexpr int kDirect = 2;
 struct HostPersist2 {
   bool ok = false;
   int estep = 1;
@@ -91,6 +93,13 @@
   std::vector<int32_t> wcrow;
   std::vector<int32_t> row_begin, grp_begin;
   std::vector<float> row_leak, row_psum;
+  int Rt = 0;
+  int table_entries = 0;
+  int max_direct = 0;
+  int64_t ndirect = 0;
+  std::vector<int32_t> pos;
+  std::vector<float> dprob;
+  std::vector<uint32_t> dpr;
 };
 struct DevPersist2 {
   const float* prob = nullptr; const uint32_t* idx2 = nullptr; const uint32_t* ends = nullptr; const int32_t* first_row = nullptr;
@@ -102,6 +111,7 @@
   int estep = 1, K = 0, R = 0;
   int cbeg[kMaxChunks + 1] = {0};
   int lds_off[kMaxChunks] = {0};
+  const int32_t* pos = nullptr; const float* dprob = nullptr; const uint32_t* dpr = nullptr;
 };
 
 }
@@ -137,6 +147,7 @@
   int device = -1;
   pk2::DevOrdering fwd, bwd, gam, fwdv, bwdv;
   float* d_pi = nullptr;
+  const float* d_pi_pos = nullptr;
   std::vector<void*> allocs;
 };
 
```

New measurement: 4841 (median of 6 runs). 1.03x the previous value.
